# NicoNeureiter/sBayes

Hardware: AMD Instinct MI355X
Metric: log-likelihood evals/sec at 1000 sites x 200 feats x 10 states; 1/2/4/8-GPU chains (higher is better)
Workload: dtype f64; 1 GPU; headline synthetic 1000x200x10, K=5, C=2 (BASELINE.json configs[2]); chains_per_gpu=4096, kernel=packed, log_mode=product, parallelism=1 independent engine(s), one per GPU, no collectives

## Files before the change

sbayes_amd/csrc/sbe_engine_internal.hip.h:

```cpp
#pragma once
#include "sbe_kernels.hip.h"
#include "sbe_unit.hip.h"
#include "../../include/sbe_engine.h"
#include "../../include/sbe_engine_steps.h"
#include "../../include/sbe_engine_diag.h"
#include "sbe_host_helpers.h"
#include "sbe_pool.h"

#include <sched.h>
#include <algorithm>
#include <cstdarg>
#include <cstdio>
#include <cstring>
#include <chrono>
#include <atomic>
#include <condition_variable>
#include <functional>
#include <mutex>
#include <string>
#include <thread>
#include <vector>

using namespace sbe;

inline thread_local std::string g_last_error;

namespace {

struct Slot {
    std::vector<uint16_t> h_gid;
    std::vector<uint8_t> h_pid;
    std::vector<uint32_t> patterns;
    int n_tuples = 0;
    std::vector<uint8_t> h_tid;
    std::vector<uint32_t> h_toff;
    std::vector<uint16_t> h_tuple_g;
    std::vector<uint8_t> h_tuple_p;
    bool share_ok = false;
    bool groups_set = false, weights_set = false, source_set = false;
    std::vector<uint8_t> probs_set, counts_set;
    bool patterns_dirty = true;
    uint32_t gid_pending = 0;
    bool tables_follow = false;
    std::vector<int32_t> pat_cnt;
    std::vector<int32_t> tup_cnt;
    bool inc_ok = false;
    uint64_t group_epoch = 0;
    uint32_t overlap_mask = 0;
    int32_t ov_obj = -1, ov_g1 = 0, ov_g2 = 0, ov_comp = 0;
};

}

static int fuse_tables_default() {
    static const int on = [] { const char* v = getenv("SBE_FUSE_TABLES"); return (v && atoi(v) == 0) ? 0 : 1; }();
    return on;
}

struct sbe_engine : sbe::MixShape {
    int device = 0;
    hipStream_t stream = nullptr;
    hipEvent_t ev0 = nullptr, ev1 = nullptr;
    std::vector<hipEvent_t> ev_pool;
    bool ev_timing = false;  int ev_used = 0;
    int Fp = 0, rs_pitch = 0;
    uint64_t rng_seed = 0, rng_draw = 0;
    std::vector<int> G, goff;
    int64_t n_na = 0;
    int64_t hbm_bytes = 0;
    std::string last_error;
    char device_name[64] = {0};
    char last_kernel[128] = "none";

    sbe::MixTuning tune;
    int opt_log = SBE_LOG_PRODUCT;
    int opt_fuse_tables = fuse_tables_default();
    bool ws_lds_allowed[2] = {false, false};

    uint8_t* d_onehot = nullptr;
    uint8_t* d_state = nullptr;
    uint8_t* d_state_q = nullptr;
    float* d_probs_t = nullptr;
    double* d_wpat_t = nullptr;
    uint16_t* d_gid = nullptr;
    uint8_t* d_pid = nullptr;
    uint8_t* d_src = nullptr;
    int32_t* d_counts = nullptr;
    float* d_probs = nullptr;
    float* d_weights = nullptr;
    float* d_wpat = nullptr;
    uint32_t* d_patbits = nullptr;
    uint16_t* d_state_h = nullptr;
    double2* d_logtab = nullptr;
    uint32_t* d_toff = nullptr;
    uint32_t* d_rowoff = nullptr;
    std::vector<uint64_t> rowoff_epoch;
    uint32_t* d_rowoff_s = nullptr;  int rs_nq_max = 0;
    int32_t* d_rs_nq = nullptr;
    uint8_t* d_state_s = nullptr;
    std::vector<uint64_t> rowsort_epoch;
    std::atomic<uint64_t> epoch_counter{0};
    double2* d_logtab_fine = nullptr;
    unsigned* d_arrive = nullptr;
    uint8_t* d_xt = nullptr;
    int xt_NT = 0, xt_KBp = 0;  size_t xt_bytes = 0;
    uint8_t* d_tid = nullptr;
    uint16_t* d_tuple_g = nullptr;
    uint8_t* d_tuple_p = nullptr;
    double* d_conc = nullptr;
    double* d_unif = nullptr;
    double* d_lg_conc = nullptr; double* d_sum_a = nullptr; double* d_lg_sum_a = nullptr;
    double* d_unif_res = nullptr;  bool unif_set = false;
    int32_t* d_comp_of_group = nullptr;
    std::vector<uint8_t> conc_set;
    double* d_partials = nullptr;
    double* d_results = nullptr;
    double* h_results = nullptr;
    int* d_status = nullptr;
    int* h_status = nullptr;
    int* h_flag = nullptr;  int* d_flag = nullptr;
    unsigned long long* h_done = nullptr;  unsigned long long* d_done = nullptr;
    unsigned* d_ticket = nullptr;  unsigned long long done_seq = 0;
    static constexpr int kMaxChunks = 16;
    unsigned long long* h_chunk_flags = nullptr;  unsigned long long* d_chunk_flags = nullptr;
    unsigned* d_chunk_tickets = nullptr;  unsigned long long chunk_seq = 0;
    uint8_t* h_stream = nullptr;  uint8_t* d_stream = nullptr;  size_t stream_bytes = 0;
    uint8_t* d_changed = nullptr;
    uint32_t* d_step_stamp = nullptr;  uint32_t step_id = 0;
    float* d_step_pf = nullptr;
    double* d_step_pg = nullptr;
    struct StepLayout { size_t ids, pid, tid, toff, tuple_g, tuple_p, patbits, weights, row_of, subset, stale, objects, rows, total; } sl{};
    int step_max_rows = 0;
    uint8_t* h_step_payload = nullptr; uint8_t* d_step_payload = nullptr;
    uint8_t* h_io = nullptr; uint8_t* d_io = nullptr; size_t io_bytes = 0;
    uint8_t* h_step = nullptr;     uint8_t* d_step_host = nullptr;
    struct Lane { uint8_t* h_payload; uint8_t* d_payload; uint8_t* h_step; uint8_t* d_step_host; float* d_pf;
                  uint32_t* d_stamp; uint32_t step_id;
                  int* d_status; };
    std::vector<Lane> lanes;
    uint8_t* d_batch_meta = nullptr; size_t batch_meta_bytes = 0;
    uint8_t* h_batch_payload = nullptr; uint8_t* d_batch_payload = nullptr; size_t batch_payload_bytes = 0;
    std::vector<Slot> batch_cands;
    std::vector<std::vector<int32_t>> batch_moved;
    std::vector<int32_t> step_moved;
    struct Pool;
    Pool* pool = nullptr;
    uint8_t* d_scratch = nullptr;  size_t scratch_bytes = 0;
    uint8_t* h_pinned = nullptr;   size_t pinned_bytes = 0;
    uint8_t* h_arena = nullptr;    uint8_t* d_arena = nullptr;   size_t arena_bytes = 0, arena_off = 0;
    SetterJobs* batch = nullptr;
    int opt_step_form = 0;
    int opt_step_derive = 0;
    int opt_deferred = 0;
    bool status_pending = false;
    const char* pending_origin[2] = {nullptr, nullptr};
    int pending_calls = 0;
    std::vector<Slot> slots;
    struct SrcSync { uint64_t version = 1; int peer = -1; uint64_t peer_version = 0, own_version = 0; std::vector<int32_t> diff; };
    std::vector<SrcSync> src_sync;
    std::vector<SrcSync> ids_sync;

    int64_t probs_t_elems() const { return (int64_t)n_ftiles * tile_tab_elems(); }
    int64_t wpat_tile_elems() const { return (int64_t)Pmax * C * ft; }
    int64_t wpat_t_elems() const { return (int64_t)n_ftiles * wpat_tile_elems(); }
};

namespace {
inline void bump_src(sbe_engine* e, int slot) { ++e->src_sync[slot].version; }
inline void bump_ids(sbe_engine* e, int slot) { ++e->ids_sync[slot].version; }
}

struct sbe_engine::Pool : sbe_host::StepPool { using sbe_host::StepPool::StepPool; };

namespace {

int fail(sbe_engine* e, int code, const char* fmt, ...) {
    char buf[512];
    va_list ap;
    va_start(ap, fmt);
    vsnprintf(buf, sizeof buf, fmt, ap);
    va_end(ap);
    g_last_error = buf;
    if (e) e->last_error = buf;
    return code;
}

#define CHECK_ENGINE(e) \
    if (!(e)) return fail(nullptr, SBE_ERR_ARG, "null engine handle")
#define CHECK_SLOT(e, s) \
    if ((s) < 0 || (s) >= (e)->n_slots) return fail(e, SBE_ERR_ARG, "slot %d out of range [0,%d)", (s), (e)->n_slots)
#define CHECK_COMP(e, c) \
    if ((c) < 0 || (c) >= (e)->C) return fail(e, SBE_ERR_ARG, "component %d out of range [0,%d)", (c), (e)->C)
#define CHECK_PTR(e, p) \
    if (!(p)) return fail(e, SBE_ERR_ARG, "null pointer argument: %s", #p)

inline int round_up(int a, int b) { return (a + b - 1) / b * b; }

template <class T>
int dmalloc(sbe_engine* e, T** p, int64_t n) {
    const size_t bytes = std::max<int64_t>(n, 1) * sizeof(T);
    HIPCHK(e, hipMalloc((void**)p, bytes));
    e->hbm_bytes += (int64_t)bytes;
    return SBE_OK;
}

inline size_t al256(size_t v) { return (v + 255) / 256 * 256; }

int ensure_scratch(sbe_engine* e, size_t bytes) {
    if (bytes <= e->scratch_bytes) return SBE_OK;
    if (e->d_scratch) { HIPCHK(e, hipStreamSynchronize(e->stream)); HIPCHK(e, hipFree(e->d_scratch)); }
    e->scratch_bytes = bytes + bytes / 4 + 4096;
    HIPCHK(e, hipMalloc((void**)&e->d_scratch, e->scratch_bytes));
    return SBE_OK;
}

int ensure_io(sbe_engine* e, size_t bytes) {
    if (bytes <= e->io_bytes) return SBE_OK;
    if (e->h_io) { HIPCHK(e, hipStreamSynchronize(e->stream)); HIPCHK(e, hipHostFree(e->h_io)); e->h_io = nullptr; e->io_bytes = 0; }
    const size_t want = bytes + bytes / 4 + 4096;
    HIPCHK(e, hipHostMalloc((void**)&e->h_io, want, hipHostMallocMapped));
    HIPCHK(e, hipHostGetDevicePointer((void**)&e->d_io, e->h_io, 0));
    e->io_bytes = want;
    return SBE_OK;
}

int ensure_pinned(sbe_engine* e, size_t bytes) {
    if (bytes <= e->pinned_bytes) return SBE_OK;
    if (e->h_pinned) { HIPCHK(e, hipStreamSynchronize(e->stream)); HIPCHK(e, hipHostFree(e->h_pinned)); }
    e->pinned_bytes = bytes + bytes / 4 + 4096;
    HIPCHK(e, hipHostMalloc((void**)&e->h_pinned, e->pinned_bytes, hipHostMallocDefault));
    return SBE_OK;
}

int upload(sbe_engine* e, void* dst_dev, const void* src, size_t bytes);
int synced(sbe_engine* e);

int ensure_step_pool(sbe_engine* e);

int ensure_stream(sbe_engine* e, size_t bytes) {
    if (bytes <= e->stream_bytes) return SBE_OK;
    if (e->h_stream) { HIPCHK(e, hipStreamSynchronize(e->stream)); HIPCHK(e, hipHostFree(e->h_stream)); e->h_stream = nullptr; e->stream_bytes = 0; }
    const size_t want = bytes + bytes / 4 + 4096;
    HIPCHK(e, hipHostMalloc((void**)&e->h_stream, want, hipHostMallocMapped));
    HIPCHK(e, hipHostGetDevicePointer((void**)&e->d_stream, e->h_stream, 0));
    e->stream_bytes = want;
    return SBE_OK;
}

struct StreamPlan { ChunkSig sig; int n_chunks; size_t chunk_bytes; size_t bytes; unsigned grid; };

StreamPlan plan_stream(sbe_engine* e, unsigned n_blocks, size_t bytes_per_block, size_t bytes) {
    static const int max_chunks = [] { const char* v = getenv("SBE_STREAM_CHUNKS"); const int n = v ? atoi(v) : 0;
                                       return n >= 1 && n <= sbe_engine::kMaxChunks ? n : 8; }();
    unsigned per = std::max<unsigned>(1, (unsigned)div_up((int64_t)n_blocks, max_chunks));
    per = std::max<unsigned>(per, (unsigned)div_up((int64_t)128 << 10, (int64_t)bytes_per_block));
    const int n_chunks = (int)div_up((int64_t)n_blocks, (int64_t)per);
    static const bool ordered = [] { const char* v = getenv("SBE_STREAM_ORDERED"); return !(v && atoi(v) == 0); }();
    ChunkSig sig{e->d_chunk_tickets, e->d_chunk_flags, ++e->chunk_seq, per, n_blocks, (unsigned)n_chunks, 0};
    unsigned grid = n_blocks;
    if (ordered && n_chunks > 1) {
        sig.chunk_elems = (long long)per * (long long)(bytes_per_block / sizeof(double));
        grid = per;
    }
    return StreamPlan{sig, n_chunks, (size_t)per * bytes_per_block, bytes, grid};
}

template <class JobBegin, class JobEnd, class Work>
int stream_result(sbe_engine* e, const StreamPlan& plan, int n_jobs, JobBegin job_begin, JobEnd job_end, Work work) {
    static const bool single_thread = [] { const char* v = getenv("SBE_D2H_THREADS"); return v && atoi(v) == 1; }();
    if (!single_thread) { int rc = ensure_step_pool(e); if (rc) return rc; }
    std::atomic<bool> all_landed{false};
    hipError_t sync_err = hipSuccess;
    const volatile unsigned long long* flags = e->h_chunk_flags;
    const unsigned long long seq = plan.sig.seq;
    const size_t chunk_bytes = plan.chunk_bytes;
    const auto t_limit = std::chrono::steady_clock::now() + std::chrono::microseconds(2000 + (int64_t)(plan.bytes / 10000));
    unsigned spins = 0;
    sbe_host::run_as_chunks_land(
        single_thread ? nullptr : e->pool, n_jobs,
        [=](int j) { return (int)(job_begin(j) / chunk_bytes); },
        [=](int j) { return (int)((job_end(j) - 1) / chunk_bytes); },
        [&, flags, seq](int k) { return flags[k] == seq || all_landed.load(std::memory_order_acquire); },
        [&] {
            if ((++spins & 1023u) == 0 && !all_landed.load(std::memory_order_relaxed) && std::chrono::steady_clock::now() > t_limit) {
                sync_err = hipStreamSynchronize(e->stream);
                all_landed.store(true, std::memory_order_release);
            }
        },
        work);
    if (sync_err != hipSuccess) return fail(e, SBE_ERR_HIP, "hipStreamSynchronize (streamed result): %s", hipGetErrorString(sync_err));
    return SBE_OK;
}

int d2h(sbe_engine* e, void* dst, const void* src_dev, size_t bytes) {
    int rc = ensure_pinned(e, bytes);
    if (rc) return rc;
    HIPCHK(e, hipMemcpyAsync(e->h_pinned, src_dev, bytes, hipMemcpyDeviceToHost, e->stream));
    HIPCHK(e, hipStreamSynchronize(e->stream));
    static const bool single_copy = [] { const char* v = getenv("SBE_D2H_THREADS"); return v && atoi(v) == 1; }();
    if (bytes >= ((size_t)1 << 20) && !single_copy) {
        rc = ensure_step_pool(e);
        if (rc) return rc;
        constexpr size_t kJob = (size_t)64 << 10;
        uint8_t* out = (uint8_t*)dst;
        const uint8_t* stage = e->h_pinned;
        e->pool->run((int)((bytes + kJob - 1) / kJob),
                     [=](int j) { const size_t o = (size_t)j * kJob; memcpy(out + o, stage + o, std::min(kJob, bytes - o)); });
        return synced(e);
    }
    memcpy(dst, e->h_pinned, bytes);
    return synced(e);
}

constexpr size_t kMappedOutMax = (size_t)1 << 18;
int out_target(sbe_engine* e, size_t bytes, void* dev_fallback, void** target) {
    *target = dev_fallback;
    if (bytes > kMappedOutMax) return SBE_OK;
    int rc = ensure_io(e, bytes);
    if (rc) return rc;
    *target = e->d_io;
    return SBE_OK;
}
int wait_done(sbe_engine* e, const DoneSig& d);
DoneSig next_done(sbe_engine* e, unsigned n_blocks);
DoneSig out_done(sbe_engine* e, const void* target, unsigned n_blocks) {
    return target == (const void*)e->d_io ? next_done(e, n_blocks) : DoneSig{};
}
int out_fetch(sbe_engine* e, void* host_out, const void* target, size_t bytes, const DoneSig& done = DoneSig{}) {
    if (target != (const void*)e->d_io) return d2h(e, host_out, target, bytes);
    int rc = wait_done(e, done);
    if (rc) return rc;
    memcpy(host_out, e->h_io, bytes);
    return synced(e);
}

int h2d(sbe_engine* e, void* dst_dev, const void* src, size_t bytes) { return upload(e, dst_dev, src, bytes); }

int upload(sbe_engine* e, void* dst_dev, const void* src, size_t bytes) {
    if (bytes == 0) return SBE_OK;
    if (e->h_arena && bytes <= e->arena_bytes / 4) {
        const size_t need = (bytes + 63) / 64 * 64;
        if (e->arena_off + need > e->arena_bytes) {
            HIPCHK(e, hipStreamSynchronize(e->stream));
            e->arena_off = 0;
        }
        uint8_t* stage = e->h_arena + e->arena_off;
        e->arena_off += need;
        memcpy(stage, src, bytes);
        HIPCHK(e, hipMemcpyAsync(dst_dev, stage, bytes, hipMemcpyHostToDevice, e->stream));
        return SBE_OK;
    }
    HIPCHK(e, hipMemcpyAsync(dst_dev, src, bytes, hipMemcpyHostToDevice, e->stream));
    HIPCHK(e, hipStreamSynchronize(e->stream));
    return SBE_OK;
}

int stage(sbe_engine* e, const void* src, size_t bytes, void* dev_fallback, const void** out) {
    constexpr size_t kDirect = (size_t)64 << 10;
    *out = dev_fallback;
    if (bytes == 0) return SBE_OK;
    if (!e->d_arena || bytes > kDirect) return upload(e, dev_fallback, src, bytes);
    const size_t need = (bytes + 63) / 64 * 64;
    if (e->arena_off + need > e->arena_bytes) {
        HIPCHK(e, hipStreamSynchronize(e->stream));
        e->arena_off = 0;
    }
    memcpy(e->h_arena + e->arena_off, src, bytes);
    *out = e->d_arena + e->arena_off;
    e->arena_off += need;
    return SBE_OK;
}

struct UploadSeg { void* dst; const void* src; size_t bytes; };
struct FusedWeightPatterns { WeightPatternArgs args; int bits_seg; const float* new_weights; bool done; };
int upload_segments(sbe_engine* e, const UploadSeg* segs, int n, FusedWeightPatterns* wp = nullptr) {
    size_t total = 0, largest = 0;
    for (int i = 0; i < n; ++i) { total += (segs[i].bytes + 63) / 64 * 64; largest = std::max(largest, segs[i].bytes); }
    if (wp) wp->done = false;
    if (total == 0) return SBE_OK;
    if (!e->d_arena || n > 8 || total > ((size_t)64 << 10)) {
        for (int i = 0; i < n; ++i) { int rc = upload(e, segs[i].dst, segs[i].src, segs[i].bytes); if (rc) return rc; }
        return SBE_OK;
    }
    const size_t w_bytes = wp && wp->new_weights ? (size_t)wp->args.F * wp->args.C * sizeof(float) : 0;
    const bool fuse = wp && segs[wp->bits_seg].bytes > 0 && w_bytes <= ((size_t)64 << 10);
    const size_t reserve = total + (fuse ? (w_bytes + 63) / 64 * 64 : 0);
    if (e->arena_off + reserve > e->arena_bytes) {
        HIPCHK(e, hipStreamSynchronize(e->stream));
        e->arena_off = 0;
    }
    ScatterSegs sg{};
    size_t off = 0;
    for (int i = 0; i < n; ++i) {
        if (segs[i].bytes == 0) continue;
        memcpy(e->h_arena + e->arena_off + off, segs[i].src, segs[i].bytes);
        sg.dst[sg.n] = (uint8_t*)segs[i].dst; sg.off[sg.n] = (uint32_t)off; sg.bytes[sg.n] = (uint32_t)segs[i].bytes;
        ++sg.n;
        if (fuse && i == wp->bits_seg) wp->args.pattern_bits = (const uint32_t*)(e->d_arena + e->arena_off + off);
        off += (segs[i].bytes + 63) / 64 * 64;
    }
    const unsigned sx = (unsigned)std::min<size_t>(div_up((int64_t)largest, 1024), 16);
    unsigned wx = 0;
    if (fuse) {
        if (w_bytes) {
            memcpy(e->h_arena + e->arena_off + off, wp->new_weights, w_bytes);
            wp->args.weights = (const float*)(e->d_arena + e->arena_off + off);
        }
        wx = (unsigned)div_up((int64_t)wp->args.P * wp->args.F, 256);
        wp->done = true;
    }
    if (e->batch && e->batch->n_group_blocks == 0 && (fuse || !wp)) {
        SetterJobs& j = *e->batch;
        j.group_base = e->d_arena + e->arena_off; j.sg = sg; j.has_wp = fuse ? 1 : 0;
        if (fuse) j.wp = wp->args;
        j.group_gx = std::max(sx, wx); j.n_group_blocks = j.group_gx * (unsigned)(sg.n + (fuse ? 1 : 0));
    } else if (fuse) {
        k_scatter_weight_patterns<<<dim3(std::max(sx, wx), sg.n + 1), 256, 0, e->stream>>>(e->d_arena + e->arena_off, sg, wp->args);
    } else {
        k_scatter_bytes<<<dim3(sx, sg.n), 256, 0, e->stream>>>(e->d_arena + e->arena_off, sg);
    }
    HIPCHK(e, hipGetLastError());
    e->arena_off += reserve;
    return SBE_OK;
}

bool poll_done_enabled() {
    static const bool on = [] { const char* v = getenv("SBE_POLL_DONE"); return !(v && atoi(v) == 0); }();
    return on;
}
DoneSig next_done(sbe_engine* e, unsigned n_blocks) {
    if (!poll_done_enabled()) return DoneSig{};
    return DoneSig{e->d_ticket, e->d_done, ++e->done_seq, n_blocks};
}
int wait_done(sbe_engine* e, const DoneSig& d) {
    if (d.flag) {
        const volatile unsigned long long* f = e->h_done;
        const auto t0 = std::chrono::steady_clock::now();
        for (unsigned spins = 1;; ++spins) {
            if (*f == d.seq) { std::atomic_thread_fence(std::memory_order_acquire); return SBE_OK; }
            if ((spins & 127u) == 0u) sched_yield(); else __builtin_ia32_pause();
            if ((spins & 255u) == 0 && std::chrono::steady_clock::now() - t0 > std::chrono::microseconds(300)) break;
        }
    }
    HIPCHK(e, hipStreamSynchronize(e->stream));
    return SBE_OK;
}

bool status_raised(const sbe_engine* e) {
    const volatile int* f = e->h_flag;
    return (f[ST_BAD_NORMALIZE] | f[ST_MULTI_SOURCE]) != 0;
}

int fetch_and_clear_status(sbe_engine* e) {
    HIPCHK(e, hipMemcpyAsync(e->h_status, e->d_status, ST_FLAG_PTR * sizeof(int), hipMemcpyDeviceToHost, e->stream));
    HIPCHK(e, hipMemsetAsync(e->d_status + ST_BAD_NORMALIZE, 0, 2 * sizeof(int), e->stream));
    HIPCHK(e, hipStreamSynchronize(e->stream));
    e->h_flag[ST_BAD_NORMALIZE] = e->h_flag[ST_MULTI_SOURCE] = 0;
    return SBE_OK;
}

int report_status(sbe_engine* e, bool deferred = false) {
    const int n_calls = e->pending_calls;
    const char* origin[2] = {e->pending_origin[0], e->pending_origin[1]};
    e->pending_calls = 0;
    e->pending_origin[0] = e->pending_origin[1] = nullptr;
    if (!status_raised(e)) return SBE_OK;
    int rc = fetch_and_clear_status(e);
    if (rc) return rc;
    const int bad_norm = e->h_status[ST_BAD_NORMALIZE], multi_src = e->h_status[ST_MULTI_SOURCE];
    e->h_status[ST_BAD_NORMALIZE] = e->h_status[ST_MULTI_SOURCE] = 0;
    char where[200] = "";
    const char* who = origin[bad_norm ? 0 : 1];
    if (deferred && who)
        snprintf(where, sizeof where, " [deferred data check: raised by %s (%d state-setting call%s queued since the last report), "
                 "reported by the first call that waited for the device]", who, n_calls, n_calls == 1 ? "" : "s");
    if (bad_norm)
        return fail(e, SBE_ERR_DATA, "normalize: %d rows have a non-positive sum (sbayes/util.py:1006 assert)%s", bad_norm, where);
    return fail(e, SBE_ERR_DATA, "source is not one-hot over components in %d observations%s", multi_src, where);
}

int check_after(sbe_engine* e, int word, const char* who = __builtin_FUNCTION()) {
    if (e->opt_deferred) {
        e->status_pending = true;
        e->pending_origin[word == ST_BAD_NORMALIZE ? 0 : 1] = who;
        ++e->pending_calls;
        return SBE_OK;
    }
    HIPCHK(e, hipStreamSynchronize(e->stream));
    e->status_pending = false;
    return report_status(e);
}

int synced(sbe_engine* e) {
    if (!e->status_pending) return SBE_OK;
    e->status_pending = false;
    return report_status(e, true);
}

int read_status(sbe_engine* e) {
    HIPCHK(e, hipStreamSynchronize(e->stream));
    int rc = synced(e);
    if (rc) return rc;
    e->h_status[ST_BAD_NORMALIZE] = e->h_status[ST_MULTI_SOURCE] = 0;
    if (status_raised(e)) return fetch_and_clear_status(e);
    return SBE_OK;
}

int take_status(sbe_engine* e) {
    e->h_status[ST_BAD_NORMALIZE] = e->h_status[ST_MULTI_SOURCE] = 0;
    if (status_raised(e)) return fetch_and_clear_status(e);
    return SBE_OK;
}

int clear_status_word(sbe_engine* e, int word) {
    if (e->status_pending) return SBE_OK;
    if (!e->h_flag[word]) return SBE_OK;
    HIPCHK(e, hipStreamSynchronize(e->stream));
    HIPCHK(e, hipMemsetAsync(e->d_status + word, 0, sizeof(int), e->stream));
    e->h_flag[word] = 0;
    return SBE_OK;
}

void derive_patterns(sbe_engine* e, Slot& s) {
    const int N = e->N, C = e->C;
    static thread_local std::vector<uint8_t> bits;
    bits.resize(N);
    bool seen[256] = {false};
    s.pat_cnt.assign(256, 0);
    for (int n = 0; n < N; ++n) {
        uint32_t b = 0;
        for (int c = 0; c < C; ++c)
            if (s.h_gid[(size_t)c * N + n] != kNoGroup) b |= 1u << c;
        bits[n] = (uint8_t)b;
        seen[b] = true;
        ++s.pat_cnt[b];
    }
    auto key = [C](uint32_t b) {
        uint32_t k = 0;
        for (int c = 0; c < C; ++c) k |= ((b >> c) & 1u) << (C - 1 - c);
        return k;
    };
    std::vector<uint32_t> uniq;
    for (uint32_t b = 0; b < 256; ++b) if (seen[b]) uniq.push_back(b);
    std::sort(uniq.begin(), uniq.end(), [&](uint32_t a, uint32_t b) { return key(a) < key(b); });
    uint8_t index_of[256] = {0};
    for (size_t i = 0; i < uniq.size(); ++i) index_of[uniq[i]] = (uint8_t)i;
    s.patterns = uniq;
    s.h_pid.resize(N);
    for (int n = 0; n < N; ++n) s.h_pid[n] = index_of[bits[n]];
}

bool tuples_share_operands(const sbe_engine* e, const Slot& s) {
    if (e->C != 2 || s.n_tuples == 0 || (int)s.h_tuple_p.size() != kMaxTuples) return false;
    int first = -1, pb = -1;
    for (int t = 0; t < kMaxTuples; ++t) {
        const int pat = s.h_tuple_p[t];
        if (pat == 0xFF) continue;
        if (first < 0) { first = t; continue; }
        if (s.h_tuple_g[(size_t)t * kMaxComponents + 1] != s.h_tuple_g[(size_t)first * kMaxComponents + 1]) return false;
        const int pa = s.h_tuple_p[first];
        if (pat != pa) {
            if (pb < 0) pb = pat;
            else if (pat != pb) return false;
        }
    }
    return first >= 0;
}

void derive_tuples(sbe_engine* e, Slot& s) {
    const int N = e->N, C = e->C;
    s.h_tid.assign(e->Np, 0);
    s.h_toff.assign(e->Np, 0);
    s.h_tuple_g.assign((size_t)kMaxTuples * kMaxComponents, (uint16_t)e->Gtot);
    s.h_tuple_p.assign(kMaxTuples, 0xFF);
    uint16_t tuples[kMaxTuples][kMaxComponents];
    int n_tup = 0;
    bool ok = true;
    s.tup_cnt.assign(kMaxTuples, 0);
    uint64_t packed[kMaxTuples];
    int last = 0;
    for (int n = 0; n < N && ok; ++n) {
        uint16_t key[kMaxComponents];
        for (int c = 0; c < C; ++c) key[c] = s.h_gid[(size_t)c * N + n];
        int t = 0;
        if (C <= 4) {
            uint64_t k64 = 0;
            for (int c = 0; c < C; ++c) k64 |= (uint64_t)key[c] << (16 * c);
            if (n_tup && packed[last] == k64) t = last;
            else for (; t < n_tup; ++t) if (packed[t] == k64) break;
            if (t == n_tup && n_tup < kMaxTuples) packed[n_tup] = k64;
        } else {
            for (; t < n_tup; ++t) if (memcmp(tuples[t], key, (size_t)C * sizeof(uint16_t)) == 0) break;
        }
        last = t;
        if (t == n_tup) {
            if (n_tup == kMaxTuples) { ok = false; break; }
            memcpy(tuples[n_tup++], key, (size_t)C * sizeof(uint16_t));
            for (int c = 0; c < C; ++c) s.h_tuple_g[(size_t)t * kMaxComponents + c] = key[c] == kNoGroup ? (uint16_t)e->Gtot : key[c];
            s.h_tuple_p[t] = s.h_pid[n];
        }
        s.h_tid[n] = (uint8_t)t;
        s.h_toff[n] = (uint32_t)t * (uint32_t)(e->S + 1) * 512u;
        ++s.tup_cnt[t];
    }
    s.n_tuples = ok ? n_tup : 0;
    s.inc_ok = ok;
    s.share_ok = tuples_share_operands(e, s);
}

bool update_patterns_and_tuples(sbe_engine* e, Slot& s, const int32_t* moved, const uint16_t* old_gid0, int n_moved) {
    const int N = e->N, C = e->C;
    if (!s.inc_ok || s.n_tuples == 0 || (int)s.pat_cnt.size() != 256 || (int)s.tup_cnt.size() != kMaxTuples) return false;
    auto bits_rest = [&](int n) { uint32_t b = 0; for (int c = 1; c < C; ++c) if (s.h_gid[(size_t)c * N + n] != kNoGroup) b |= 1u << c; return b; };
    for (int i = 0; i < n_moved; ++i) {
        const int n = moved[i];
        const uint32_t rest = bits_rest(n);
        const uint32_t b0 = rest | (old_gid0[i] != kNoGroup ? 1u : 0u), b1 = rest | (s.h_gid[n] != kNoGroup ? 1u : 0u);
        if (b0 == b1) continue;
        --s.pat_cnt[b0]; ++s.pat_cnt[b1];
    }
    {
        size_t live = 0;
        for (uint32_t b = 0; b < 256; ++b) if (s.pat_cnt[b] > 0) ++live;
        bool same = live == s.patterns.size();
        for (size_t i = 0; same && i < s.patterns.size(); ++i) same = s.pat_cnt[s.patterns[i]] > 0;
        if (!same) return false;
    }
    uint8_t rank_of[256];
    for (size_t i = 0; i < s.patterns.size(); ++i) rank_of[s.patterns[i]] = (uint8_t)i;
    for (int i = 0; i < n_moved; ++i) {
        const int n = moved[i];
        const uint32_t b1 = bits_rest(n) | (s.h_gid[n] != kNoGroup ? 1u : 0u);
        s.h_pid[n] = rank_of[b1];
        uint16_t key[kMaxComponents];
        for (int c = 0; c < C; ++c) { const uint16_t g = s.h_gid[(size_t)c * N + n]; key[c] = g == kNoGroup ? (uint16_t)e->Gtot : g; }
        const int t0 = s.h_tid[n];
        int t1 = -1, free_t = -1;
        for (int t = 0; t < s.n_tuples; ++t) {
            if (s.tup_cnt[t] == 0) { if (free_t < 0 && t != t0) free_t = t; continue; }
            if (memcmp(&s.h_tuple_g[(size_t)t * kMaxComponents], key, (size_t)C * sizeof(uint16_t)) == 0) { t1 = t; break; }
        }
        if (t1 < 0) {
            if (s.tup_cnt[t0] == 1) t1 = t0;
            else if (free_t >= 0) t1 = free_t;
            else if (s.n_tuples < kMaxTuples) t1 = s.n_tuples++;
            else return false;
            for (int c = 0; c < C; ++c) s.h_tuple_g[(size_t)t1 * kMaxComponents + c] = key[c];
        }
        if (t1 != t0) {
            if (--s.tup_cnt[t0] == 0) s.h_tuple_p[t0] = 0xFF;
            ++s.tup_cnt[t1];
        }
        s.h_tuple_p[t1] = s.h_pid[n];
        s.h_tid[n] = (uint8_t)t1;
        s.h_toff[n] = (uint32_t)t1 * (uint32_t)(e->S + 1) * 512u;
    }
    while (s.n_tuples > 0 && s.tup_cnt[s.n_tuples - 1] == 0) --s.n_tuples;
    s.share_ok = tuples_share_operands(e, s);
    for (int t = 0; t < s.n_tuples; ++t)
        if (s.tup_cnt[t] == 0) return false;
    return s.n_tuples > 0;
}

int upload_patterns_and_weights(sbe_engine* e, int slot, const float* new_weights = nullptr, bool eager = false) {
    Slot& s = e->slots[slot];
    float* d_w = e->d_weights + (int64_t)slot * e->F * e->C;
    auto gid_seg = [&](int c) { return UploadSeg{e->d_gid + ((int64_t)slot * e->C + c) * e->Np, s.h_gid.data() + (size_t)c * e->N, (size_t)e->N * sizeof(uint16_t)}; };
    bool patterns_done = false;
    if (s.patterns_dirty) {
        const bool follow = s.tables_follow;
        s.tables_follow = false;
        if (!follow) derive_patterns(e, s);
        if ((int)s.patterns.size() > e->Pmax) {
            if (eager) {
                for (int c = 0; c < e->C; ++c)
                    if (s.gid_pending >> c & 1u) { const UploadSeg g = gid_seg(c); int rc = upload(e, g.dst, g.src, g.bytes); if (rc) return rc; }
                s.gid_pending = 0;
                return SBE_OK;
            }
            return fail(e, SBE_ERR_ARG, "%zu distinct has_components patterns exceed capacity %d",
                        s.patterns.size(), e->Pmax);
        }
        if (!follow) derive_tuples(e, s);
        UploadSeg segs[6 + kMaxComponents] = {{e->d_pid + (int64_t)slot * e->Np, s.h_pid.data(), (size_t)e->N},
                                              {e->d_patbits + (int64_t)slot * e->Pmax, s.patterns.data(), s.patterns.size() * sizeof(uint32_t)}};
        int n_segs = 2;
        if (s.n_tuples) {
            segs[n_segs++] = {e->d_tid + (int64_t)slot * e->Np, s.h_tid.data(), (size_t)e->Np};
            segs[n_segs++] = {e->d_toff + (int64_t)slot * e->Np, s.h_toff.data(), (size_t)e->Np * sizeof(uint32_t)};
            segs[n_segs++] = {e->d_tuple_g + (int64_t)slot * kMaxTuples * kMaxComponents, s.h_tuple_g.data(), s.h_tuple_g.size() * sizeof(uint16_t)};
            segs[n_segs++] = {e->d_tuple_p + (int64_t)slot * kMaxTuples, s.h_tuple_p.data(), s.h_tuple_p.size()};
        }
        for (int c = 0; c < e->C; ++c) if (s.gid_pending >> c & 1u) segs[n_segs++] = gid_seg(c);
        const int P = (int)s.patterns.size();
        FusedWeightPatterns wp{};
        const bool want_wp = (s.weights_set || new_weights) && P > 0;
        if (want_wp) {
            wp.args = WeightPatternArgs{d_w, nullptr, e->d_wpat + (int64_t)slot * e->Pmax * e->F * e->C, new_weights ? d_w : nullptr,
                                        e->d_wpat_t + (int64_t)slot * e->wpat_t_elems(), P, e->F, e->C, e->Pmax, e->ft};
            wp.bits_seg = 1;
            wp.new_weights = new_weights;
        }
        { int _urc = upload_segments(e, segs, n_segs, want_wp ? &wp : nullptr); if (_urc) return _urc; }
        patterns_done = wp.done;
        s.patterns_dirty = false;
        s.gid_pending = 0;
    }
    const int P = (int)s.patterns.size();
    if (new_weights && P == 0) {
        int rc = upload(e, d_w, new_weights, (size_t)e->F * e->C * sizeof(float));
        if (rc) return rc;
    }
    if ((s.weights_set || new_weights) && P > 0 && !patterns_done) {
        const void* w_in = d_w;
        if (new_weights) { int rc = stage(e, new_weights, (size_t)e->F * e->C * sizeof(float), d_w, &w_in); if (rc) return rc; }
        k_weight_patterns<<<div_up((int64_t)P * e->F, 256), 256, 0, e->stream>>>(
            (const float*)w_in, e->d_patbits + (int64_t)slot * e->Pmax, e->d_wpat + (int64_t)slot * e->Pmax * e->F * e->C, P, e->F, e->C,
            w_in != d_w ? d_w : nullptr, e->d_wpat_t + (int64_t)slot * e->wpat_t_elems(), e->Pmax, e->ft);
        HIPCHK(e, hipGetLastError());
    }
    return SBE_OK;
}

int retile_probs(sbe_engine* e, int slot, int component) {
    const int g_lo = e->goff[component], g_hi = g_lo + e->G[component];
    const int64_t n = (int64_t)(g_hi - g_lo) * e->S * e->ft * e->n_ftiles;
    if (n == 0) return SBE_OK;
    k_tile_probs<<<div_up(n, 256), 256, 0, e->stream>>>(
        e->d_probs + (int64_t)slot * e->table_elems(), e->d_probs_t + (int64_t)slot * e->probs_t_elems(),
        g_lo, g_hi, e->Gtot, e->F, e->S, e->ft, e->n_ftiles);
    HIPCHK(e, hipGetLastError());
    return SBE_OK;
}

int check_slot_ready(sbe_engine* e, int slot, bool need_weights) {
    Slot& s = e->slots[slot];
    if (!s.groups_set) return fail(e, SBE_ERR_STATE, "slot %d: groups not set for every component", slot);
    for (int c = 0; c < e->C; ++c)
        if (!s.probs_set[c]) return fail(e, SBE_ERR_STATE, "slot %d: probability tables of component %d not set", slot, c);
    if (need_weights && !s.weights_set) return fail(e, SBE_ERR_STATE, "slot %d: weights not set", slot);
    return SBE_OK;
}

int check_collapsed_ready(sbe_engine* e, int slot, int c_lo, int c_hi) {
    Slot& s = e->slots[slot];
    for (int c = c_lo; c < c_hi; ++c) {
        if (e->G[c] == 0) continue;
        if (!s.counts_set[c]) return fail(e, SBE_ERR_STATE, "slot %d: counts of component %d not set", slot, c);
        if (!e->conc_set[c]) return fail(e, SBE_ERR_STATE, "concentration of component %d not set", c);
    }
    return SBE_OK;
}

constexpr size_t kCollapsedLdsMax = (size_t)96 << 10;
inline size_t collapsed_lds_bytes(const sbe_engine* e) { return (size_t)e->F * e->S * sizeof(double) + (size_t)e->F * sizeof(float); }

template <class TC>
int enqueue_dcl(sbe_engine* e, const TC* counts, const double* conc, int conc_per_group, int g_lo, int G, float* d_pf, double* d_pg) {
    k_dcl<TC><<<div_up((int64_t)G * e->F, 256), 256, 0, e->stream>>>(counts, conc, d_pf, g_lo, g_lo + G, e->F, e->S, conc_per_group);
    HIPCHK(e, hipGetLastError());
    if (!d_pg) return SBE_OK;
    k_group_sum_f32<<<div_up((int64_t)G * 8, 64), 64, 0, e->stream>>>(d_pf, d_pg, G, e->F);
    HIPCHK(e, hipGetLastError());
    return SBE_OK;
}

int ensure_xt(sbe_engine* e) {
    if (e->d_xt) return SBE_OK;
    const int NT = div_up((int64_t)e->F * e->S, 32), KBp = round_up(div_up(e->N, kTupleMfmaKBlockObjects), 4);
    const size_t bytes = ((size_t)(NT + 1) * KBp + 4) * 1024;
    uint8_t* xt = nullptr;
    double2* logtab = nullptr;
    auto build = [&]() -> int {
        HIPCHK(e, hipMalloc((void**)&xt, bytes));
        HIPCHK(e, hipMemsetAsync(xt, 0, bytes, e->stream));
        std::vector<double> tab(2 * kFineLogEntries);
        fine_log_table(tab.data());
        HIPCHK(e, hipMalloc((void**)&logtab, tab.size() * sizeof(double) + column_tables_bytes(NT)));
        HIPCHK(e, hipMemcpy(logtab, tab.data(), tab.size() * sizeof(double), hipMemcpyHostToDevice));
        launch_column_tables(e->d_state, reinterpret_cast<int32_t*>(logtab + kFineLogEntries), e->N, e->F, e->S, e->Fp, NT, e->stream);
        HIPCHK(e, hipGetLastError());
        launch_xt_frags(e->d_state, xt, e->N, e->F, e->S, e->Fp, NT, KBp, e->stream);
        HIPCHK(e, hipGetLastError());
        return SBE_OK;
    };
    const int rc = build();
    if (rc) {
        (void)hipStreamSynchronize(e->stream);
        if (xt) (void)hipFree(xt);
        if (logtab) (void)hipFree(logtab);
        return rc;
    }
    e->d_xt = xt; e->d_logtab_fine = logtab;
    e->hbm_bytes += (int64_t)bytes;
    e->xt_NT = NT; e->xt_KBp = KBp; e->xt_bytes = bytes;
    return SBE_OK;
}

int next_timing_events(sbe_engine* e, hipEvent_t* ev_a, hipEvent_t* ev_b) {
    *ev_a = *ev_b = nullptr;
    if (!e->ev_timing) return SBE_OK;
    while ((int)e->ev_pool.size() < 2 * (e->ev_used + 1)) {
        hipEvent_t ev;
        HIPCHK(e, hipEventCreate(&ev));
        e->ev_pool.push_back(ev);
    }
    *ev_a = e->ev_pool[2 * e->ev_used]; *ev_b = e->ev_pool[2 * e->ev_used + 1];
    ++e->ev_used;
    return SBE_OK;
}

struct MixCall {
    int first_slot = 0, n = 1;
    const int32_t* slots = nullptr;  const int32_t* d_slots = nullptr;
    const StepFinish* fin = nullptr;
    const StepFinish* d_fins = nullptr;
    DoneSig* done_out = nullptr;
    hipEvent_t ev_a = nullptr, ev_b = nullptr;
    int slot_at(int i) const { return slots ? (int)slots[i] : first_slot + i; }
};

MixFacts mixture_facts(const sbe_engine* e, const MixCall& c) {
    MixFacts f;
    f.n = c.n;
    f.share_ok = true;
    bool tuples = true;
    for (int i = 0; i < c.n; ++i) {
        const Slot& s = e->slots[c.slot_at(i)];
        f.P = std::max<int>(f.P, (int)s.patterns.size());
        f.KT = std::max(f.KT, s.n_tuples);
        tuples &= s.n_tuples != 0;
        f.share_ok &= s.share_ok;
    }
    if (!tuples) f.KT = 0;
    f.epilogue = c.fin || c.d_fins;
    f.waits = c.done_out != nullptr;
    return f;
}

MixTuning launch_tuning(const sbe_engine* e, const MixFacts& f) {
    MixTuning t = e->tune;
    if (considers_tuple_mfma(*e, t, f))
        if (const char* env = getenv("SBE_MFMA_SPLIT")) t.mfma_split = atoi(env);
    t.shared_allowed = tuple_mfma_shared();
    static const bool in_kernel_opt = !(getenv("SBE_REDUCE_IN_KERNEL") && atoi(getenv("SBE_REDUCE_IN_KERNEL")) == 0);
    t.in_kernel_allowed = in_kernel_opt;
    return t;
}

int prepare_mixture(sbe_engine* e, const MixPlan& pl, const MixCall& c) {
    if (pl.form == MixForm::TupleMfma) return ensure_xt(e);
    if (pl.form != MixForm::Rows && pl.form != MixForm::RowsSorted) return SBE_OK;
    const bool sorted = pl.form == MixForm::RowsSorted;
    const int rft = pl.ft;
    if (sorted && !e->d_rowoff_s) {
        e->rs_nq_max = pl.rs_nq_max;
        int rc = dmalloc(e, &e->d_rowoff_s, (int64_t)e->n_slots * e->rs_nq_max * (e->C + 1) * 4); if (rc) return rc;
        rc = dmalloc(e, &e->d_rs_nq, e->n_slots); if (rc) return rc;
        rc = dmalloc(e, &e->d_state_s, (int64_t)(e->N + 1) * e->Fq); if (rc) return rc;
        launch_state_s(e->d_state, e->d_state_s, e->N, e->F, e->Fp, e->Fq, e->S, e->stream);
        HIPCHK(e, hipGetLastError());
        e->rowsort_epoch.assign(e->n_slots, ~0ull);
    }
    std::vector<uint64_t>& built = sorted ? e->rowsort_epoch : e->rowoff_epoch;
    bool stale = false;
    for (int i = 0; i < c.n; ++i) stale |= built[c.slot_at(i)] != e->slots[c.slot_at(i)].group_epoch;
    if (!stale) return SBE_OK;
    if (sorted) {
        launch_rowsort(e->d_gid, e->d_pid, e->d_rowoff_s, e->d_rs_nq, (int64_t)e->C * e->Np, e->Np,
                       (int64_t)e->rs_nq_max * (e->C + 1) * 4, c.first_slot, c.d_slots, c.n, e->N, e->Np, e->C, e->Gtot, e->Pmax,
                       (uint32_t)((e->S + 1) * rft * 4), (uint32_t)e->Fq, 4 * (kWave / rft), e->stream);
    } else {
        const int cells = (e->C + 1) * e->Np;
        k_rowoff<<<dim3(div_up(cells, 256), c.n), 256, 0, e->stream>>>(
            e->d_gid, e->d_pid, e->d_rowoff, (int64_t)e->C * e->Np, e->Np, (int64_t)cells, c.first_slot, c.d_slots, e->N, e->Np,
            e->C, e->Gtot, (uint32_t)((e->S + 1) * rft * 4), (uint32_t)(((e->C + 1) / 2) * rft * 16));
    }
    HIPCHK(e, hipGetLastError());
    for (int i = 0; i < c.n; ++i) built[c.slot_at(i)] = e->slots[c.slot_at(i)].group_epoch;
    return SBE_OK;
}

int launch_mfma_form(sbe_engine* e, const MixCall& c, const MixPlan& pl, const DoneSig& done) {
    MfmaMixParams p{};
    p.F = e->F; p.S = e->S; p.FS = e->F * e->S; p.Gtot = e->Gtot; p.Np = e->Np;
    p.NT = e->xt_NT; p.KBp = e->xt_KBp; p.KT = pl.KT; p.SL = pl.SL; p.shared = pl.shared ? 1 : 0;
    p.n_batch = c.n; p.n_split = pl.n_split; p.nt_per_split = pl.nt_per_split;
    p.first_slot = c.first_slot; p.slot_list = c.d_slots;
    p.xt = e->d_xt; p.xt_bytes = (uint32_t)e->xt_bytes;
    p.tid = e->d_tid; p.tid_stride = e->Np;
    p.tuple_g = e->d_tuple_g; p.tuple_g_stride = (int64_t)kMaxTuples * kMaxComponents;
    p.tuple_p = e->d_tuple_p; p.tuple_p_stride = kMaxTuples;
    p.probs = e->d_probs; p.probs_stride = e->table_elems();
    p.probs_ones_off = (uint32_t)((int64_t)e->n_slots * e->table_elems() * 4);
    p.probs_bytes = p.probs_ones_off + (uint32_t)(e->F * e->S * 4);
    p.wpat = e->d_wpat; p.wpat_stride = (int64_t)e->Pmax * e->F * e->C;
    p.wpat_ones_off = (uint32_t)((int64_t)e->n_slots * e->Pmax * e->F * e->C * 4);
    p.wpat_bytes = p.wpat_ones_off + (uint32_t)(e->F * e->C * 4);
    p.logtab = e->d_logtab_fine;
    p.colcount = reinterpret_cast<const int32_t*>(e->d_logtab_fine + kFineLogEntries);
    p.colfeat = p.colcount + (size_t)(e->xt_NT + 1) * 32;
    p.tile_prefix = p.colcount + (size_t)(e->xt_NT + 1) * 64;
    p.partials = e->d_partials; p.partials_stride = e->partials_stride;
    if (pl.in_kernel) { p.results = e->d_results; p.arrive = e->d_arrive; p.done = done; }
    if (!launch_tuple_mfma(e->C, p, dim3(pl.grid_x), pl.lds_bytes, e->stream))
        return fail(e, SBE_ERR_STATE, "k_mixture_tuple_mfma was built with static LDS: its log table must sit at LDS address 0 "
                                      "(toolchain change; rebuild without static __shared__ in sbe_mixture_mfma.hip)");
    return SBE_OK;
}

void launch_tile_form(sbe_engine* e, const MixCall& c, const MixPlan& pl, const DoneSig& done) {
    Mix2Params p{};
    p.N = e->N; p.NQ = e->NQ; p.Np = e->Np; p.F = e->F; p.Fq = e->Fq; p.S = e->S; p.C = e->C;
    p.Gtot = e->Gtot; p.P = pl.P; p.n_ftiles = pl.n_ftiles; p.quads_per_chunk = pl.quads_per_chunk;
    p.state_q = reinterpret_cast<const uint32_t*>(e->d_state_q);
    p.onehot = e->d_onehot; p.rs_pitch = e->rs_pitch;
    p.gid = e->d_gid; p.gid_stride = (int64_t)e->C * e->Np;
    p.pid = e->d_pid; p.pid_stride = e->Np;
    p.probs_t = e->d_probs_t; p.probs_t_stride = e->probs_t_elems();
    p.wpat_t = e->d_wpat_t; p.wpat_t_stride = e->wpat_t_elems(); p.wpat_tile_stride = (int)e->wpat_tile_elems();
    p.partials = e->d_partials; p.partials_stride = e->partials_stride; p.first_slot = c.first_slot;
    if (pl.in_kernel) { p.results = e->d_results; p.arrive = e->d_arrive; p.done = done; }
    p.slot_list = c.d_slots;
    p.n_work = pl.n_partials; p.n_batch = c.n;
    p.slot_groups = pl.slot_groups; p.slots_per_group = pl.slots_per_group;
    p.tid = e->d_tid; p.tid_stride = e->Np;
    p.state_h = reinterpret_cast<const uint2*>(e->d_state_h);
    p.toff = e->d_toff; p.toff_stride = e->Np;
    p.logtab = e->d_logtab;
    p.ragged_w = pl.ragged_w; p.gen_slots = pl.gen_slots;
    p.tuple_g = e->d_tuple_g; p.tuple_g_stride = (int64_t)kMaxTuples * kMaxComponents;
    p.tuple_p = e->d_tuple_p; p.tuple_p_stride = kMaxTuples;
    p.combo_w_off = pl.combo_w_off; p.combo_tab_off = pl.combo_tab_off;
    p.KT = pl.KT;
    p.eft = e->ft;
    p.wpat = e->d_wpat; p.wpat_stride = (int64_t)e->Pmax * e->F * e->C;
    p.rowoff = e->d_rowoff; p.rowoff_stride = (int64_t)(e->C + 1) * e->Np;
    p.rowoff_s = e->d_rowoff_s; p.rowoff_s_stride = (int64_t)e->rs_nq_max * (e->C + 1) * 4;
    p.rs_nq = e->d_rs_nq; p.state_s = e->d_state_s; p.state_s_pitch = e->Fq;
    {
        constexpr int split[4] = {450, 270, 170, 110};
        p.rows_cum[0] = 0;
        for (int i = 0; i < 4; ++i) p.rows_cum[i + 1] = p.rows_cum[i] + split[i];
    }
    const int mode = e->opt_log == SBE_LOG_PRODUCT ? LOG_PRODUCT : LOG_PER_OBS;
    const dim3 grid(pl.grid_x, 1);
    switch (pl.form) {
        case MixForm::Tuple64: launch_tuple64(e->C, p, grid, pl.lds_bytes, e->stream); break;
        case MixForm::Combo: launch_combo(pl.onehot, pl.ft, e->C, p, grid, pl.lds_bytes, e->stream); break;
        case MixForm::Rows: case MixForm::RowsSorted:
            launch_rows(mode, pl.ft, e->C, p, grid, pl.lds_bytes, e->stream, pl.form == MixForm::RowsSorted); break;
        case MixForm::OnehotV2: launch_oh2(mode, pl.ft, e->C, p, grid, pl.lds_bytes, e->stream, e->direct); break;
        default: launch_v2(mode, pl.ft, e->C, p, grid, pl.lds_bytes, e->stream, e->direct); break;
    }
}

int launch_mixture(sbe_engine* e, const MixCall& c) {
    const MixFacts facts = mixture_facts(e, c);
    const MixPlan pl = plan_mixture(*e, launch_tuning(e, facts), facts);
    if (pl.err) return fail(e, pl.err, "%s", pl.msg);
    int rc = prepare_mixture(e, pl, c);
    if (rc) return rc;
    if (c.ev_a) HIPCHK(e, hipEventRecord(c.ev_a, e->stream));
    DoneSig done_k{};
    if (pl.in_kernel && c.done_out) *c.done_out = done_k = next_done(e, pl.done_blocks);
    plan_name(pl, *e, e->last_kernel, sizeof e->last_kernel);
    if (pl.form == MixForm::TupleMfma) { rc = launch_mfma_form(e, c, pl, done_k); if (rc) return rc; }
    else launch_tile_form(e, c, pl, done_k);
    if (c.ev_b) HIPCHK(e, hipEventRecord(c.ev_b, e->stream));
    HIPCHK(e, hipGetLastError());
    if (pl.in_kernel) return SBE_OK;
    const unsigned n_red = (unsigned)(c.n + (c.d_fins ? c.n : (c.fin ? 1 : 0)));
    const DoneSig done = c.done_out ? next_done(e, n_red) : DoneSig{};
    if (c.done_out) *c.done_out = done;
    k_reduce_partials<<<n_red, kBlock, 0, e->stream>>>(e->d_partials, e->partials_stride, pl.n_partials,
                                                       e->d_results, c.first_slot, c.n, c.fin ? *c.fin : StepFinish{},
                                                       c.d_slots, c.d_fins, done);
    HIPCHK(e, hipGetLastError());
    return SBE_OK;
}

int enqueue_mixture(sbe_engine* e, int first_slot, int n, DoneSig* done_out = nullptr) {
    for (int s = first_slot; s < first_slot + n; ++s) {
        int rc = check_slot_ready(e, s, true);
        if (rc) return rc;
        if (e->slots[s].patterns_dirty) { rc = upload_patterns_and_weights(e, s); if (rc) return rc; }
    }
    MixCall c;
    c.first_slot = first_slot; c.n = n; c.done_out = done_out;
    { int rc = next_timing_events(e, &c.ev_a, &c.ev_b); if (rc) return rc; }
    return launch_mixture(e, c);
}

int counts_launch(sbe_engine* e, int slot_a, int sign_a, int slot_b, int sign_b, const int32_t* d_objects,
                  int n_listed, int dst_slot, bool single_chunk, uint8_t* d_changed) {
    CountSide A{e->d_gid + (int64_t)slot_a * e->C * e->Np, e->d_src + (int64_t)slot_a * e->N * e->Fp, sign_a};
    CountSide B{e->d_gid + (int64_t)slot_b * e->C * e->Np, e->d_src + (int64_t)slot_b * e->N * e->Fp, sign_b};
    int32_t* counts = e->d_counts + (int64_t)dst_slot * e->table_elems();
    int ft = 32;
    auto lds_for = [&](int t) { return (size_t)e->Gtot * t * e->S * sizeof(int32_t); };
    while (ft > 4 && lds_for(ft) > 96 * 1024) ft >>= 1;
    if (lds_for(ft) > 150 * 1024) {
        k_counts_global<<<div_up((int64_t)n_listed * e->F, 256), 256, 0, e->stream>>>(
            e->d_state, A, B, d_objects, n_listed, e->Np, e->F, e->S, e->C, e->Fp, counts, d_changed);
        HIPCHK(e, hipGetLastError());
        return SBE_OK;
    }
    const int n_ftiles = div_up(e->F, ft);
    int chunks = 1;
    if (!single_chunk) chunks = std::max(1, std::min(div_up(n_listed, 32), div_up(2 * e->compute_units, n_ftiles)));
    const int opc = div_up(n_listed, chunks);
    chunks = div_up(n_listed, opc);
    k_counts<<<dim3(n_ftiles, chunks), kBlock, lds_for(ft), e->stream>>>(
        e->d_state, A, B, d_objects, n_listed, opc, e->Np, e->F, e->S, e->C, e->Fp, e->Gtot, ft, counts, d_changed);
    HIPCHK(e, hipGetLastError());
    return SBE_OK;
}

}

namespace {

int set_gid_common(sbe_engine* e, int slot, int component, const std::vector<uint16_t>& ids) {
    Slot& s = e->slots[slot];
    s.tables_follow = false;
    static const bool follow_on = [] { const char* v = getenv("SBE_FOLLOW_TABLES"); return !(v && atoi(v) == 0); }();
    if (follow_on && component == 0 && !s.patterns_dirty && s.inc_ok) {
        static thread_local std::vector<int32_t> moved;
        static thread_local std::vector<uint16_t> old_ids;
        moved.clear(); old_ids.clear();
        const int N = e->N;
        for (int n = 0; n < N; ++n)
            if (ids[n] != s.h_gid[n]) { moved.push_back(n); old_ids.push_back(s.h_gid[n]); }
        std::copy(ids.begin(), ids.end(), s.h_gid.begin());
        s.tables_follow = (int)moved.size() * 8 <= N &&
                          update_patterns_and_tuples(e, s, moved.data(), old_ids.data(), (int)moved.size());
    } else {
        std::copy(ids.begin(), ids.end(), s.h_gid.begin() + (size_t)component * e->N);
    }
    s.gid_pending |= 1u << component;
    s.patterns_dirty = true;
    s.group_epoch = ++e->epoch_counter;
    bump_ids(e, slot);
    s.groups_set = true;
    return upload_patterns_and_weights(e, slot, nullptr, true);
}

void overlap_message(char* buf, size_t len, int n, int g1, int g2, int component) {
    snprintf(buf, len, "object %d is in groups %d and %d of component %d: resident slot state keeps one group id per object "
             "and component (counts.py:28-30 would count it in both); counts of overlapping groups come from the caller or "
             "the stateless sbe_effect_counts", n, g1, g2, component);
}

struct OverlapNote { bool found = false; int obj = -1, g1 = 0, g2 = 0; };

bool matrix_to_ids(const uint8_t* groups, int G, int N, int off, int component, uint16_t* ids, char* msg, size_t msg_len,
                   OverlapNote* note = nullptr) {
    std::fill(ids, ids + N, kNoGroup);
    auto hit = [&](int n, int g) -> bool {
        if (ids[n] != kNoGroup) {
            if (!note) { overlap_message(msg, msg_len, n, (int)ids[n] - off, g, component); return false; }
            if (!note->found) { note->found = true; note->obj = n; note->g1 = (int)ids[n] - off; note->g2 = g; }
        }
        ids[n] = (uint16_t)(off + g);
        return true;
    };
    for (int g = 0; g < G; ++g) {
        const uint8_t* row = groups + (size_t)g * N;
        int n = 0;
        for (; n + 8 <= N; n += 8) {
            uint64_t w8;
            memcpy(&w8, row + n, 8);
            if (!w8) continue;
            for (int k = 0; k < 8; ++k) if (row[n + k] && !hit(n + k, g)) return false;
        }
        for (; n < N; ++n) if (row[n] && !hit(n, g)) return false;
    }
    return true;
}

int reject_overlap(sbe_engine* e, int slot, const char* what) {
    const Slot& s = e->slots[slot];
    if (!s.overlap_mask) return SBE_OK;
    char msg[320];
    overlap_message(msg, sizeof msg, s.ov_obj, s.ov_g1, s.ov_g2, s.ov_comp);
    return fail(e, SBE_ERR_DATA, "%s (slot %d, %s)", msg, slot, what);
}


int enqueue_lh_exact(sbe_engine* e, int slot, const char* who) {
    Slot& s = e->slots[slot];
    if (!s.groups_set || !s.source_set || !s.weights_set) return fail(e, SBE_ERR_STATE, "slot %d: groups / source / weights not set", slot);
    { int orc = reject_overlap(e, slot, who); if (orc) return orc; }
    for (int c = 0; c < e->C; ++c)
        if (!s.counts_set[c] || !e->conc_set[c]) return fail(e, SBE_ERR_STATE, "slot %d: counts / concentration of component %d not set", slot, c);
    HIPCHK(e, hipSetDevice(e->device));
    int rc = SBE_OK;
    if (s.patterns_dirty) { rc = upload_patterns_and_weights(e, slot); if (rc) return rc; }
    const int64_t n = (int64_t)e->N * e->F;
    rc = ensure_scratch(e, n * sizeof(double));
    if (rc) return rc;
    rc = clear_status_word(e, ST_BAD_NORMALIZE);
    if (rc) return rc;
    k_lh_exact<<<div_up(n, 256), 256, 0, e->stream>>>(
        e->d_state, e->d_src + (int64_t)slot * e->N * e->Fp, e->d_gid + (int64_t)slot * e->C * e->Np,
        e->d_counts + (int64_t)slot * e->table_elems(), e->d_conc, (double*)e->d_scratch, e->N, e->Np, e->F, e->S, e->C,
        e->Fp, e->d_status, e->d_wpat + (int64_t)slot * e->Pmax * e->F * e->C, e->d_pid + (int64_t)slot * e->Np);
    HIPCHK(e, hipGetLastError());
    return SBE_OK;
}

int lh_exact_report(sbe_engine* e) {
    int rc = read_status(e);
    if (rc) return rc;
    if (e->h_status[ST_BAD_NORMALIZE]) return fail(e, SBE_ERR_DATA, "normalize: non-positive row sum in leave-one-out tables (sbayes/util.py:1006 assert)");
    return SBE_OK;
}

int sync_and_report(sbe_engine* e, const DoneSig& done = DoneSig{}) {
    { int rc = wait_done(e, done); if (rc) return rc; }
    const bool was_pending = e->status_pending;
    e->status_pending = false;
    return report_status(e, was_pending);
}

int check_objects(sbe_engine* e, const int32_t* objects, int n) {
    for (int i = 0; i < n; ++i)
        if (objects[i] < 0 || objects[i] >= e->N) return fail(e, SBE_ERR_ARG, "object index %d out of range", objects[i]);
    return SBE_OK;
}

SrcPostArgs src_post_args(sbe_engine* e, int slot, const int32_t* d_objects, int n_sub, double temperature, double prior_temperature,
                          int from_prior) {
    const double inv_t = 1.0 / temperature, inv_tp = 1.0 / prior_temperature;
    return SrcPostArgs{e->d_state, e->d_gid + (int64_t)slot * e->C * e->Np, e->d_pid + (int64_t)slot * e->Np,
                       e->d_probs + (int64_t)slot * e->table_elems(), e->d_wpat + (int64_t)slot * e->Pmax * e->F * e->C,
                       d_objects, n_sub, e->Np, e->F, e->S, e->C, e->Fp, inv_t, (float)inv_tp, inv_t != 1.0, inv_tp != 1.0,
                       from_prior != 0};
}

ClusterOpArgs cluster_op_args(sbe_engine* e, int slot, double prior_temperature, const int32_t* d_objects, int n, double* d_out) {
    const double inv = 1.0 / prior_temperature;
    return ClusterOpArgs{e->d_state, e->d_gid + (int64_t)slot * e->C * e->Np, e->d_pid + (int64_t)slot * e->Np,
                         e->d_weights + (int64_t)slot * e->F * e->C, e->d_patbits + (int64_t)slot * e->Pmax, (float)inv,
                         inv != 1.0 ? 1 : 0, d_objects, n, d_out, reinterpret_cast<const f64x2_t*>(e->d_logtab),
                         e->Np, e->F, e->S, e->C, e->Fp};
}

constexpr size_t kGuFusedLdsMax = (size_t)96 << 10;

}

namespace {
int ensure_step_pool(sbe_engine* e) {
    if (!e->pool) {
        int nt = 7;
        if (const char* env = getenv("SBE_STEP_THREADS")) nt = std::max(0, atoi(env) - 1);
        int cpus = (int)std::thread::hardware_concurrency();
        cpu_set_t set;
        if (sched_getaffinity(0, sizeof set, &set) == 0) cpus = std::min(cpus > 0 ? cpus : CPU_COUNT(&set), CPU_COUNT(&set));
        if (FILE* f = fopen("/sys/fs/cgroup/cpu.max", "r")) {
            long long quota = 0, period = 0;
            if (fscanf(f, "%lld %lld", &quota, &period) == 2 && quota > 0 && period > 0)
                cpus = std::min<int>(cpus, (int)std::max<long long>(1, quota / period));
            fclose(f);
        }
        int local_world = 1;
        if (const char* env = getenv("LOCAL_WORLD_SIZE")) local_world = std::max(1, atoi(env));
        nt = std::min<int>(nt, std::max(0, cpus / local_world - 1));
        e->pool = new sbe_engine::Pool(nt);
    }
    return SBE_OK;
}
}
```

sbayes_amd/csrc/sbe_engine_steps.hip:

```cpp
#include "sbe_engine_internal.hip.h"

extern "C" {

namespace {
struct CoreInputs {
    const void* ids_new = nullptr;
    const void* pid = nullptr; const void* tid = nullptr; const void* toff = nullptr;
    const void* tuple_g = nullptr; const void* tuple_p = nullptr; const void* patbits = nullptr;
    const void* weights = nullptr;
    const int16_t* row_of = nullptr;
    const uint8_t* rows = nullptr; const int32_t* objects = nullptr; int n_changed = 0;
    const uint8_t* src_new = nullptr;
    const int32_t* subset = nullptr; int n_subset = 0;
    int P = 1;
    bool full_src_copy = true; const int32_t* stale = nullptr; int n_stale = 0;
    const int32_t* patch_n = nullptr; const uint16_t* patch_gid = nullptr; const uint8_t* patch_pid = nullptr;
    const uint8_t* patch_tid = nullptr; int n_patch = -1;
    const int16_t* sub_row = nullptr; const uint16_t* sub_gid0 = nullptr;
};

sbe_engine::Lane lane0(sbe_engine* e) {
    return sbe_engine::Lane{e->h_step_payload, e->d_step_payload, e->h_step, e->d_step_host, e->d_step_pf, e->d_step_stamp, e->step_id,
                            e->d_status};
}
// ... 275 lines not shown
    ++rc.version;
    if (moved.size() == 1 && moved[0] < 0) {
        rc.peer = cu.peer = -1;
        rc.diff.clear(); cu.diff.clear();
        return;
    }
    rc.peer = cur_slot; rc.peer_version = cu.version; rc.own_version = rc.version; rc.diff = moved;
    cu.peer = cand_slot; cu.peer_version = rc.version; cu.own_version = cu.version; cu.diff = moved;
}

static void commit_src_sync(sbe_engine* e, int cur_slot, int cand_slot, const int32_t* changed_objects, int n_changed) {
    sbe_engine::SrcSync& rc = e->src_sync[cand_slot];
    sbe_engine::SrcSync& cu = e->src_sync[cur_slot];
    ++rc.version;
    rc.peer = cur_slot; rc.peer_version = cu.version; rc.own_version = rc.version;
    rc.diff.assign(changed_objects, changed_objects + n_changed);
    cu.peer = cand_slot; cu.peer_version = rc.version; cu.own_version = cu.version;
    cu.diff = rc.diff;
}

static int step_lean(sbe_engine* e, int cur_slot, int cand_slot, const uint8_t* clusters, const int32_t* changed_objects,
                     int n_changed, const uint8_t* source_rows, const float* weights, double* group_logliks_out,
                     double* mixture_out, uint8_t* changed_groups_out) {
    if (e->status_pending) {
        HIPCHK(e, hipStreamSynchronize(e->stream));
        int rc = synced(e);
        if (rc) return rc;
    }
    static const bool timing = getenv("SBE_STEP_TIMING") && atoi(getenv("SBE_STEP_TIMING")) == 1;
    static double t_acc[3] = {0, 0, 0};
    static int t_n = 0;
    const auto t0 = std::chrono::steady_clock::now();
    Slot cd;
    CoreInputs in;
    {
        std::string err;
        int rc = prepare_step(e, lane0(e), cur_slot, cand_slot, clusters, changed_objects, n_changed, source_rows, weights, cd, in, &err,
                              &e->step_moved);
        if (rc) return fail(e, rc, "%s", err.c_str());
    }
    const auto t1 = std::chrono::steady_clock::now();
    int rc = launch_step_core(e, cur_slot, cand_slot, in);
    if (rc) return rc;
    commit_src_sync(e, cur_slot, cand_slot, changed_objects, n_changed);
    commit_ids_sync(e, cur_slot, cand_slot, e->step_moved);
    e->slots[cand_slot] = cd;
    StepFinish fin = make_step_finish(e);
    DoneSig done;
    MixCall mix;
    mix.first_slot = cand_slot; mix.fin = &fin; mix.done_out = &done;
    rc = launch_mixture(e, mix);
    if (rc) return rc;
    const auto t2 = std::chrono::steady_clock::now();
    rc = wait_done(e, done);
    if (rc) return rc;
    if (timing) {
        const auto t3 = std::chrono::steady_clock::now();
        t_acc[0] += std::chrono::duration<double, std::micro>(t1 - t0).count();
        t_acc[1] += std::chrono::duration<double, std::micro>(t2 - t1).count();
        t_acc[2] += std::chrono::duration<double, std::micro>(t3 - t2).count();
        if (++t_n == 2000) {
            fprintf(stderr, "[sbe_step] host prepare %.1f us, enqueue %.1f us, wait %.1f us per step\n", t_acc[0] / t_n, t_acc[1] / t_n, t_acc[2] / t_n);
            t_acc[0] = t_acc[1] = t_acc[2] = 0; t_n = 0;
        }
    }
    return read_step_results(e, cand_slot, group_logliks_out, mixture_out, changed_groups_out, "rows");
}

namespace {
int ensure_lanes(sbe_engine* e, int n) {
    const size_t hb = step_host_lq_offset(e) + 2 * sizeof(double);
    while ((int)e->lanes.size() < n) {
        sbe_engine::Lane ln{};
        HIPCHK(e, hipHostMalloc((void**)&ln.h_step, hb, hipHostMallocMapped));
        memset(ln.h_step, 0, hb);
        HIPCHK(e, hipHostGetDevicePointer((void**)&ln.d_step_host, ln.h_step, 0));
        HIPCHK(e, hipMalloc((void**)&ln.d_pf, (size_t)e->Gtot * e->F * sizeof(float)));
        HIPCHK(e, hipMalloc((void**)&ln.d_stamp, (size_t)e->Gtot * sizeof(uint32_t)));
        HIPCHK(e, hipMemsetAsync(ln.d_stamp, 0, (size_t)e->Gtot * sizeof(uint32_t), e->stream));
        HIPCHK(e, hipMalloc((void**)&ln.d_status, ST_WORDS * sizeof(int)));
        HIPCHK(e, hipMemsetAsync(ln.d_status, 0, ST_WORDS * sizeof(int), e->stream));
        ln.step_id = 0;
        e->lanes.push_back(ln);
    }
    return SBE_OK;
}
}


int sbe_step_batch(sbe_engine* e, int n_chains, const int32_t* cur_slots, const int32_t* cand_slots,
                   const uint8_t* clusters, const uint8_t* clusters_mask, const int32_t* rows_ptr,
                   const int32_t* changed_objects, const uint8_t* source_rows, const float* weights,
                   const uint8_t* weights_mask, double* group_logliks_out, double* mixture_out,
                   uint8_t* changed_groups_out) {
    CHECK_ENGINE(e); CHECK_PTR(e, cur_slots); CHECK_PTR(e, cand_slots); CHECK_PTR(e, rows_ptr);
    CHECK_PTR(e, group_logliks_out); CHECK_PTR(e, mixture_out);
    if (n_chains < 1 || n_chains > e->n_slots / 2) return fail(e, SBE_ERR_ARG, "n_chains=%d (1..%d: two slots per chain)", n_chains, e->n_slots / 2);
    if ((int64_t)e->Gtot * e->S * 28 > 60 * 1024) return fail(e, SBE_ERR_ARG, "sbe_step_batch: tables too large for the one-launch step (G_total=%d, S=%d)", e->Gtot, e->S);
    const int N = e->N, F = e->F, C = e->C, K = e->G[0];
    if (rows_ptr[0] != 0) return fail(e, SBE_ERR_ARG, "rows_ptr[0] must be 0");
    static const bool timing = getenv("SBE_STEP_TIMING") && atoi(getenv("SBE_STEP_TIMING")) != 0;
    using clk = std::chrono::steady_clock;
    clk::time_point tp[12]; int ntp = 0;
    auto mark = [&] { if (timing && ntp < 12) tp[ntp++] = clk::now(); };
    mark();
    {
        std::vector<uint8_t> used(e->n_slots, 0);
        for (int i = 0; i < n_chains; ++i) {
            const int a = cur_slots[i], b = cand_slots[i];
            if (a < 0 || a >= e->n_slots || b < 0 || b >= e->n_slots || a == b) return fail(e, SBE_ERR_ARG, "chain %d: bad slots (%d, %d)", i, a, b);
            if (used[a] || used[b]) return fail(e, SBE_ERR_ARG, "chain %d: slot used by another chain of the batch", i);
            used[a] = used[b] = 1;
            const int nr = rows_ptr[i + 1] - rows_ptr[i];
            if (nr < 0 || nr > e->step_max_rows) return fail(e, SBE_ERR_ARG, "chain %d: %d changed source rows (0..%d per chain in a batched step)", i, nr, e->step_max_rows);
            if (nr > 0 && (!changed_objects || !source_rows)) return fail(e, SBE_ERR_ARG, "changed_objects / source_rows missing");
            for (int k = rows_ptr[i]; k < rows_ptr[i + 1]; ++k)
                if (changed_objects[k] < 0 || changed_objects[k] >= N) return fail(e, SBE_ERR_ARG, "chain %d: object index %d out of range", i, changed_objects[k]);
            const Slot& cur = e->slots[a];
            if (!cur.groups_set || !cur.source_set || !cur.weights_set) return fail(e, SBE_ERR_STATE, "slot %d: groups / source / weights not set", a);
            { int orc = reject_overlap(e, a, "one-call step"); if (orc) return orc; }
            for (int c = 0; c < C; ++c)
                if (!cur.counts_set[c] || !e->conc_set[c]) return fail(e, SBE_ERR_STATE, "slot %d: counts / concentration of component %d not set", a, c);
        }
    }
    HIPCHK(e, hipSetDevice(e->device));
    if (e->status_pending) {
        HIPCHK(e, hipStreamSynchronize(e->stream));
        int rc = synced(e);
        if (rc) return rc;
    }
    for (int i = 0; i < n_chains; ++i)
        if (e->slots[cur_slots[i]].patterns_dirty) { int rc = upload_patterns_and_weights(e, cur_slots[i]); if (rc) return rc; }
    int rc = ensure_lanes(e, n_chains);
    if (rc) return rc;
    rc = ensure_step_pool(e);
    if (rc) return rc;
    mark();
    if ((int)e->batch_cands.size() < n_chains) e->batch_cands.resize(n_chains);
    if ((int)e->batch_moved.size() < n_chains) e->batch_moved.resize(n_chains);
    std::vector<Slot>& cds = e->batch_cands;
    std::vector<CoreInputs> ins(n_chains);
    std::vector<size_t> pay_off(n_chains + 1, 0);
    for (int i = 0; i < n_chains; ++i)
        pay_off[i + 1] = pay_off[i] + (e->sl.rows + (size_t)(rows_ptr[i + 1] - rows_ptr[i]) * F * C + 255) / 256 * 256;
    if (pay_off[n_chains] > e->batch_payload_bytes) {
        HIPCHK(e, hipStreamSynchronize(e->stream));
        if (e->h_batch_payload) { HIPCHK(e, hipHostFree(e->h_batch_payload)); e->h_batch_payload = nullptr; }
        if (e->d_batch_payload) { HIPCHK(e, hipFree(e->d_batch_payload)); e->d_batch_payload = nullptr; }
        e->batch_payload_bytes = pay_off[n_chains] + pay_off[n_chains] / 2;
        HIPCHK(e, hipHostMalloc((void**)&e->h_batch_payload, e->batch_payload_bytes, hipHostMallocDefault));
        HIPCHK(e, hipMalloc((void**)&e->d_batch_payload, e->batch_payload_bytes));
    }
    int n_parts = n_chains >= 128 ? 2 : 1;
    if (const char* env = getenv("SBE_STEP_PARTS")) n_parts = std::max(1, std::min(atoi(env), n_chains));
    const int per_part = div_up(n_chains, n_parts);
    const size_t part_cores = ((size_t)per_part * sizeof(StepCore) + 255) / 256 * 256;
    const size_t part_fins = ((size_t)per_part * sizeof(StepFinish) + 255) / 256 * 256;
    const size_t part_bytes = part_cores + part_fins + ((size_t)per_part * sizeof(int32_t) + 255) / 256 * 256;
    const size_t meta_bytes = part_bytes * n_parts;
    if (meta_bytes > e->batch_meta_bytes) {
        if (e->d_batch_meta) { HIPCHK(e, hipStreamSynchronize(e->stream)); HIPCHK(e, hipFree(e->d_batch_meta)); }
        e->batch_meta_bytes = meta_bytes + meta_bytes / 2;
        HIPCHK(e, hipMalloc((void**)&e->d_batch_meta, e->batch_meta_bytes));
    }
    std::vector<uint8_t> meta(meta_bytes);
    std::vector<int> rcs(n_chains, SBE_OK);
    std::vector<std::string> errs(n_chains);
    DoneSig batch_done{};
    for (int part = 0; part < n_parts; ++part) {
        const int i0 = part * per_part, i1 = std::min(n_chains, i0 + per_part), np = i1 - i0;
        if (np <= 0) break;
        constexpr int kCopyChunk = 16;
        const int n_copy_chunks = div_up(np, kCopyChunk);
        std::vector<std::atomic<int>> chunk_done(n_copy_chunks);
        for (auto& c : chunk_done) c.store(0, std::memory_order_relaxed);
        int next_copy = 0;
        hipError_t copy_err = hipSuccess;
        auto send_ready = [&]() {
            while (next_copy < n_copy_chunks) {
                const int c0 = i0 + next_copy * kCopyChunk, c1 = std::min(i1, c0 + kCopyChunk);
                if (chunk_done[next_copy].load(std::memory_order_acquire) < c1 - c0) break;
                const hipError_t he = hipMemcpyAsync(e->d_batch_payload + pay_off[c0], e->h_batch_payload + pay_off[c0],
                                                     pay_off[c1] - pay_off[c0], hipMemcpyHostToDevice, e->stream);
                if (he != hipSuccess) copy_err = he;
                ++next_copy;
            }
        };
        const std::function<void()> poll = send_ready;
        e->pool->run(np, [&](int j) {
            const int i = i0 + j;
            const bool regroup = clusters && (!clusters_mask || clusters_mask[i]);
            const bool reweight = weights && (!weights_mask || weights_mask[i]);
            const int r0 = rows_ptr[i], nr = rows_ptr[i + 1] - r0;
            sbe_engine::Lane lane = e->lanes[i];
            lane.h_payload = e->h_batch_payload + pay_off[i];
            lane.d_payload = e->d_batch_payload + pay_off[i];
            rcs[i] = prepare_step(e, lane, cur_slots[i], cand_slots[i], regroup ? clusters + (size_t)i * K * N : nullptr,
                                  nr ? changed_objects + r0 : nullptr, nr, nr ? source_rows + (size_t)r0 * F * C : nullptr,
                                  reweight ? weights + (size_t)i * F * C : nullptr, cds[i], ins[i], &errs[i], &e->batch_moved[i]);
            chunk_done[j / kCopyChunk].fetch_add(1, std::memory_order_release);
        }, &poll);
        send_ready();
        HIPCHK(e, copy_err);
        for (int i = i0; i < i1; ++i)
            if (rcs[i]) { (void)hipStreamSynchronize(e->stream); return fail(e, rcs[i], "chain %d: %s", i, errs[i].c_str()); }
        if (part == 0) mark();
        uint8_t* pm = meta.data() + (size_t)part * part_bytes;
        StepCore* cores = reinterpret_cast<StepCore*>(pm);
        StepFinish* fins = reinterpret_cast<StepFinish*>(pm + part_cores);
        int32_t* slot_list = reinterpret_cast<int32_t*>(pm + part_cores + part_fins);
        size_t lds = 0; int max_blocks = 0;
        for (int i = i0; i < i1; ++i) {
            size_t l = 0; int nb = 0;
            rc = build_step_core(e, e->lanes[i], cur_slots[i], cand_slots[i], ins[i], cores[i - i0], l, nb, n_chains);
            if (rc) return rc;
            lds = std::max(lds, l); max_blocks = std::max(max_blocks, nb);
            fins[i - i0] = make_step_finish_lane(e, e->lanes[i]);
            slot_list[i - i0] = cand_slots[i];
        }
        if (part == 0) mark();
        uint8_t* dm = e->d_batch_meta + (size_t)part * part_bytes;
        rc = upload(e, dm, pm, part_bytes);
        if (rc) return rc;
        if (part == 0) mark();
        k_step_core_batch<<<dim3(max_blocks, np), kBlock, lds, e->stream>>>(reinterpret_cast<const StepCore*>(dm));
        HIPCHK(e, hipGetLastError());
        if (part == 0) mark();
        for (int i = i0; i < i1; ++i) {
            commit_src_sync(e, cur_slots[i], cand_slots[i], changed_objects ? changed_objects + rows_ptr[i] : nullptr,
                            rows_ptr[i + 1] - rows_ptr[i]);
            commit_ids_sync(e, cur_slots[i], cand_slots[i], e->batch_moved[i]);
            std::swap(e->slots[cand_slots[i]], cds[i]);
        }
        if (part == 0) mark();
        MixCall mix;
        mix.n = np; mix.slots = cand_slots + i0; mix.d_slots = reinterpret_cast<const int32_t*>(dm + part_cores + part_fins);
        mix.d_fins = reinterpret_cast<const StepFinish*>(dm + part_cores); mix.done_out = part == n_parts - 1 ? &batch_done : nullptr;
        rc = launch_mixture(e, mix);
        if (rc) return rc;
    }
    mark();
    { int wrc = wait_done(e, batch_done); if (wrc) return wrc; }
    mark();
    int first_bad = SBE_OK;
    std::string first_msg;
    for (int i = 0; i < n_chains; ++i) {
        rc = read_step_results_lane(e, e->lanes[i].h_step, cand_slots[i], group_logliks_out + (size_t)i * e->Gtot, mixture_out + i,
                               changed_groups_out ? changed_groups_out + (size_t)i * e->Gtot : nullptr, "rows", e->lanes[i].d_status, i);
        if (rc && !first_bad) { first_bad = rc; first_msg = e->last_error; }
    }
    if (first_bad) return fail(e, first_bad, "%s", first_msg.c_str());
    mark();
    if (timing && ntp == 10) {
        auto us = [&](int a, int b) { return std::chrono::duration<double, std::micro>(tp[b] - tp[a]).count(); };
        fprintf(stderr, "[sbe_step_batch] %d chains (first part): checks %.1f | prepare (pool) %.1f | step cores %.1f | upload %.1f | launch core %.1f | "
                        "slot moves %.1f | mixture + reduce launches and the other parts %.1f | wait for the device %.1f | read results %.1f us\n", n_chains,
                us(0, 1), us(1, 2), us(2, 3), us(3, 4), us(4, 5), us(5, 6), us(6, 7), us(7, 8), us(8, 9));
    }
    return SBE_OK;
}

namespace {

struct DeltaPlan {
    size_t subset, sub_row, sub_gid0, patch_n, patch_gid, patch_pid, patch_tid, stale, objects, tuple_g, tuple_p, patbits, weights, rows, total;
};

inline size_t al16(size_t v) { return (v + 15) / 16 * 16; }

DeltaPlan plan_delta(const sbe_engine* e, int n_mv, int n_changed, int n_last_ids, int n_last_src, bool reweight) {
    DeltaPlan p{};
    const size_t n_sub = (size_t)n_mv + n_changed, n_patch = (size_t)n_mv + n_last_ids;
    size_t o = 0;
    p.subset = o;    o = al16(o + n_sub * 4);
    p.sub_row = o;   o = al16(o + n_sub * 2);
    p.sub_gid0 = o;  o = al16(o + n_sub * 2);
    p.patch_n = o;   o = al16(o + n_patch * 4);
    p.patch_gid = o; o = al16(o + n_patch * 2);
    p.patch_pid = o; o = al16(o + n_patch);
    p.patch_tid = o; o = al16(o + n_patch);
    p.stale = o;     o = al16(o + (size_t)n_last_src * 4);
    p.objects = o;   o = al16(o + (size_t)n_changed * 4);
    p.tuple_g = o;   o = al16(o + (size_t)kMaxTuples * kMaxComponents * 2);
    p.tuple_p = o;   o = al16(o + (size_t)kMaxTuples);
    p.patbits = o;   o = al16(o + (size_t)e->Pmax * 4);
    p.weights = o;   o = al16(o + (reweight ? (size_t)e->F * e->C * 4 : 0));
    p.rows = o;      o = al16(o + (size_t)n_changed * e->F * e->C);
    p.total = (o + 255) / 256 * 256;
    return p;
}

int prepare_step_delta(sbe_engine* e, uint8_t* h_base, const uint8_t* d_base, const DeltaPlan& L, int cur_slot, int cand_slot,
                       const int32_t* mv_objects, const int32_t* mv_cluster, int n_mv, const int32_t* changed_objects, int n_changed,
                       const uint8_t* source_rows, const float* weights, CoreInputs& in, std::vector<int32_t>& moved_out) {
    const int F = e->F, C = e->C;
    const Slot& cur = e->slots[cur_slot];
    Slot& cd = e->slots[cand_slot];
    const sbe_engine::SrcSync& irec = e->ids_sync[cand_slot];
    for (int32_t n : irec.diff) {
        cd.h_gid[n] = cur.h_gid[n]; cd.h_pid[n] = cur.h_pid[n]; cd.h_tid[n] = cur.h_tid[n]; cd.h_toff[n] = cur.h_toff[n];
    }
    cd.patterns = cur.patterns; cd.n_tuples = cur.n_tuples;
    cd.h_tuple_g = cur.h_tuple_g; cd.h_tuple_p = cur.h_tuple_p; cd.pat_cnt = cur.pat_cnt; cd.tup_cnt = cur.tup_cnt;
    cd.share_ok = cur.share_ok;
    cd.inc_ok = cur.inc_ok; cd.patterns_dirty = false;
    cd.groups_set = cur.groups_set; cd.weights_set = true; cd.source_set = cur.source_set;
    cd.counts_set = cur.counts_set;
    static thread_local std::vector<int32_t> mv;
    static thread_local std::vector<uint16_t> mv_old;
    mv.clear(); mv_old.clear();
    for (int i = 0; i < n_mv; ++i) {
        const int n = mv_objects[i];
        const uint16_t g_new = mv_cluster[i] < 0 ? kNoGroup : (uint16_t)mv_cluster[i];
        if (cd.h_gid[n] == g_new) continue;
        mv.push_back(n); mv_old.push_back(cd.h_gid[n]);
        cd.h_gid[n] = g_new;
    }
    if (!mv.empty()) {
        if (e->opt_step_derive == 1 || !update_patterns_and_tuples(e, cd, mv.data(), mv_old.data(), (int)mv.size())) return 1;
        cd.group_epoch = ++e->epoch_counter;
    } else cd.group_epoch = cur.group_epoch;
    std::fill(cd.probs_set.begin(), cd.probs_set.end(), 1);
    moved_out = mv;
    uint8_t* st = h_base;
    in = CoreInputs{};
    int32_t* sub = reinterpret_cast<int32_t*>(st + L.subset);
    int16_t* sub_row = reinterpret_cast<int16_t*>(st + L.sub_row);
    uint16_t* sub_gid0 = reinterpret_cast<uint16_t*>(st + L.sub_gid0);
    int n_subset = 0;
    {
        static thread_local std::vector<std::pair<int32_t, int32_t>> ch;
        ch.clear();
        for (int i = 0; i < n_changed; ++i) ch.emplace_back(changed_objects[i], i);
        std::sort(ch.begin(), ch.end());
        std::sort(mv.begin(), mv.end());
        size_t a = 0, b = 0;
        while (a < mv.size() || b < ch.size()) {
            int32_t n; int r = -1;
            if (b == ch.size() || (a < mv.size() && mv[a] < ch[b].first)) n = mv[a++];
            else { n = ch[b].first; r = ch[b].second; if (a < mv.size() && mv[a] == n) ++a; ++b; }
            sub[n_subset] = n; sub_row[n_subset] = (int16_t)r; sub_gid0[n_subset] = cd.h_gid[n];
            ++n_subset;
        }
    }
    int n_patch = 0;
    {
        int32_t* pn = reinterpret_cast<int32_t*>(st + L.patch_n);
        uint16_t* pg = reinterpret_cast<uint16_t*>(st + L.patch_gid);
        uint8_t* pp = st + L.patch_pid; uint8_t* pt = st + L.patch_tid;
        auto put = [&](int32_t n) { pn[n_patch] = n; pg[n_patch] = cd.h_gid[n]; pp[n_patch] = cd.h_pid[n]; pt[n_patch] = cd.h_tid[n]; ++n_patch; };
        for (int32_t n : irec.diff) put(n);
        for (int32_t n : mv) put(n);
    }
    const bool tables_changed = cd.patterns != cur.patterns || cd.h_tuple_p != cur.h_tuple_p || cd.h_tuple_g != cur.h_tuple_g;
    if (tables_changed) {
        memcpy(st + L.tuple_g, cd.h_tuple_g.data(), (size_t)kMaxTuples * kMaxComponents * 2);
        memcpy(st + L.tuple_p, cd.h_tuple_p.data(), kMaxTuples);
        memset(st + L.patbits, 0, (size_t)e->Pmax * 4);
        memcpy(st + L.patbits, cd.patterns.data(), cd.patterns.size() * 4);
        in.tuple_g = d_base + L.tuple_g; in.tuple_p = d_base + L.tuple_p; in.patbits = d_base + L.patbits;
    }
    if (weights) { memcpy(st + L.weights, weights, (size_t)F * C * 4); in.weights = d_base + L.weights; }
    if (n_changed > 0) {
        memcpy(st + L.objects, changed_objects, (size_t)n_changed * 4);
        memcpy(st + L.rows, source_rows, (size_t)n_changed * F * C);
        in.rows = d_base + L.rows;
        in.objects = reinterpret_cast<const int32_t*>(d_base + L.objects);
        in.n_changed = n_changed;
    }
    in.subset = reinterpret_cast<const int32_t*>(d_base + L.subset); in.n_subset = n_subset;
    in.sub_row = reinterpret_cast<const int16_t*>(d_base + L.sub_row);
    in.sub_gid0 = reinterpret_cast<const uint16_t*>(d_base + L.sub_gid0);
    in.patch_n = reinterpret_cast<const int32_t*>(d_base + L.patch_n);
    in.patch_gid = reinterpret_cast<const uint16_t*>(d_base + L.patch_gid);
    in.patch_pid = d_base + L.patch_pid; in.patch_tid = d_base + L.patch_tid; in.n_patch = n_patch;
    in.P = (int)cd.patterns.size();
    {
        const sbe_engine::SrcSync& rec = e->src_sync[cand_slot];
        int32_t* stale = reinterpret_cast<int32_t*>(st + L.stale);
        int ns = 0;
        for (int32_t n : rec.diff) {
            bool rewritten = false;
            for (int i = 0; i < n_changed && !rewritten; ++i) rewritten = changed_objects[i] == n;
            if (!rewritten) stale[ns++] = n;
        }
        in.full_src_copy = false;
        in.stale = reinterpret_cast<const int32_t*>(d_base + L.stale);
        in.n_stale = ns;
    }
    return 0;
}

bool sync_valid(const sbe_engine::SrcSync& rec, const sbe_engine::SrcSync& peer, int peer_slot, int cap) {
    return rec.peer == peer_slot && rec.peer_version == peer.version && rec.own_version == rec.version && (int)rec.diff.size() <= cap;
}

}

int sbe_step_batch_delta(sbe_engine* e, int n_chains, const int32_t* cur_slots, const int32_t* cand_slots,
                         const int32_t* moved_ptr, const int32_t* moved_objects, const int32_t* moved_cluster,
                         const int32_t* rows_ptr, const int32_t* changed_objects, const uint8_t* source_rows,
                         const float* weights, const uint8_t* weights_mask, double* group_logliks_out, double* mixture_out,
                         uint8_t* changed_groups_out) {
    CHECK_ENGINE(e); CHECK_PTR(e, cur_slots); CHECK_PTR(e, cand_slots); CHECK_PTR(e, moved_ptr); CHECK_PTR(e, rows_ptr);
    CHECK_PTR(e, group_logliks_out); CHECK_PTR(e, mixture_out);
    const auto t_start = std::chrono::steady_clock::now();
    std::chrono::steady_clock::time_point tq[8]; int nq = 0;
    auto markd = [&] { if (nq < 8) tq[nq++] = std::chrono::steady_clock::now(); };
    if (n_chains < 1 || n_chains > e->n_slots / 2) return fail(e, SBE_ERR_ARG, "n_chains=%d (1..%d: two slots per chain)", n_chains, e->n_slots / 2);
    if ((int64_t)e->Gtot * e->S * 28 > 60 * 1024) return fail(e, SBE_ERR_ARG, "sbe_step_batch_delta: tables too large for the one-launch step (G_total=%d, S=%d)", e->Gtot, e->S);
    const int N = e->N, F = e->F, C = e->C, K = e->G[0];
    if (rows_ptr[0] != 0 || moved_ptr[0] != 0) return fail(e, SBE_ERR_ARG, "rows_ptr[0] / moved_ptr[0] must be 0");
    {
        std::vector<uint8_t> used(e->n_slots, 0);
        std::vector<uint32_t> seen(N, 0), seen_mv(N, 0);
        for (int i = 0; i < n_chains; ++i) {
            const int a = cur_slots[i], b = cand_slots[i];
            if (a < 0 || a >= e->n_slots || b < 0 || b >= e->n_slots || a == b) return fail(e, SBE_ERR_ARG, "chain %d: bad slots (%d, %d)", i, a, b);
            if (used[a] || used[b]) return fail(e, SBE_ERR_ARG, "chain %d: slot used by another chain of the batch", i);
            used[a] = used[b] = 1;
            const int nr = rows_ptr[i + 1] - rows_ptr[i], nm = moved_ptr[i + 1] - moved_ptr[i];
            if (nr < 0 || nr > e->step_max_rows) return fail(e, SBE_ERR_ARG, "chain %d: %d changed source rows (0..%d per chain in a batched step)", i, nr, e->step_max_rows);
            if (nm < 0 || nm > N) return fail(e, SBE_ERR_ARG, "chain %d: %d moved objects", i, nm);
            if ((nr > 0 && (!changed_objects || !source_rows)) || (nm > 0 && (!moved_objects || !moved_cluster))) return fail(e, SBE_ERR_ARG, "chain %d: delta arrays missing", i);
            for (int k = rows_ptr[i]; k < rows_ptr[i + 1]; ++k) {
                const int n = changed_objects[k];
                if (n < 0 || n >= N) return fail(e, SBE_ERR_ARG, "chain %d: object index %d out of range", i, n);
                if (seen[n] == (uint32_t)(2 * i + 1)) return fail(e, SBE_ERR_ARG, "chain %d: object %d listed twice in changed_objects", i, n);
                seen[n] = (uint32_t)(2 * i + 1);
            }
            for (int k = moved_ptr[i]; k < moved_ptr[i + 1]; ++k) {
                const int n = moved_objects[k];
                if (n < 0 || n >= N) return fail(e, SBE_ERR_ARG, "chain %d: moved object index %d out of range", i, n);
                if (moved_cluster[k] < -1 || moved_cluster[k] >= K) return fail(e, SBE_ERR_ARG, "chain %d: cluster %d out of range [-1,%d)", i, moved_cluster[k], K);
                if (seen_mv[n] == (uint32_t)(i + 1)) return fail(e, SBE_ERR_ARG, "chain %d: object %d listed twice in moved_objects", i, n);
                seen_mv[n] = (uint32_t)(i + 1);
            }
            const Slot& cur = e->slots[a];
            if (!cur.groups_set || !cur.source_set || !cur.weights_set) return fail(e, SBE_ERR_STATE, "slot %d: groups / source / weights not set", a);
            { int orc = reject_overlap(e, a, "one-call step"); if (orc) return orc; }
            for (int c = 0; c < C; ++c)
                if (!cur.counts_set[c] || !e->conc_set[c]) return fail(e, SBE_ERR_STATE, "slot %d: counts / concentration of component %d not set", a, c);
        }
    }
    HIPCHK(e, hipSetDevice(e->device));
    if (e->status_pending) {
        HIPCHK(e, hipStreamSynchronize(e->stream));
        int rc = synced(e);
        if (rc) return rc;
    }
    for (int i = 0; i < n_chains; ++i)
        if (e->slots[cur_slots[i]].patterns_dirty) { int rc = upload_patterns_and_weights(e, cur_slots[i]); if (rc) return rc; }
    int rc = ensure_lanes(e, n_chains);
    if (rc) return rc;
    rc = ensure_step_pool(e);
    if (rc) return rc;
    if ((int)e->batch_moved.size() < n_chains) e->batch_moved.resize(n_chains);
    markd();
    std::vector<int> fast, slow;
    std::vector<DeltaPlan> plans(n_chains);
    std::vector<size_t> pay_off(n_chains + 1, 0);
    for (int i = 0; i < n_chains; ++i) {
        const int a = cur_slots[i], b = cand_slots[i];
        const bool ok = sync_valid(e->ids_sync[b], e->ids_sync[a], a, e->step_max_rows) &&
                        sync_valid(e->src_sync[b], e->src_sync[a], a, e->step_max_rows) &&
                        e->slots[a].inc_ok && e->slots[a].n_tuples > 0 && e->slots[b].h_gid.size() == e->slots[a].h_gid.size();
        if (ok) {
            const bool reweight = weights && (!weights_mask || weights_mask[i]);
            plans[i] = plan_delta(e, moved_ptr[i + 1] - moved_ptr[i], rows_ptr[i + 1] - rows_ptr[i], (int)e->ids_sync[b].diff.size(),
                                  (int)e->src_sync[b].diff.size(), reweight);
            pay_off[i + 1] = pay_off[i] + plans[i].total;
            fast.push_back(i);
        } else { pay_off[i + 1] = pay_off[i]; slow.push_back(i); }
    }
    auto run_classic = [&](const std::vector<int>& which, int& rc_out, std::string& msg_out) {
        rc_out = SBE_OK;
        if (which.empty()) return;
        const int ns = (int)which.size();
        std::vector<int32_t> s_cur(ns), s_cand(ns), s_ptr(ns + 1, 0), s_objs;
        std::vector<uint8_t> s_cl((size_t)ns * K * N, 0), s_rows, s_wm(ns, 0);
        std::vector<float> s_w(weights ? (size_t)ns * F * C : 0);
        for (int j = 0; j < ns; ++j) {
            const int i = which[j];
            s_cur[j] = cur_slots[i]; s_cand[j] = cand_slots[i];
            const Slot& cur = e->slots[cur_slots[i]];
            std::vector<uint16_t> ids(cur.h_gid.begin(), cur.h_gid.begin() + N);
            for (int k = moved_ptr[i]; k < moved_ptr[i + 1]; ++k) ids[moved_objects[k]] = moved_cluster[k] < 0 ? kNoGroup : (uint16_t)moved_cluster[k];
            uint8_t* cl = s_cl.data() + (size_t)j * K * N;
            for (int n = 0; n < N; ++n) if (ids[n] != kNoGroup) cl[(size_t)ids[n] * N + n] = 1;
            const int r0 = rows_ptr[i], nr = rows_ptr[i + 1] - r0;
            s_ptr[j + 1] = s_ptr[j] + nr;
            if (nr) {
                s_objs.insert(s_objs.end(), changed_objects + r0, changed_objects + r0 + nr);
                s_rows.insert(s_rows.end(), source_rows + (size_t)r0 * F * C, source_rows + (size_t)(r0 + nr) * F * C);
            }
            if (weights && (!weights_mask || weights_mask[i])) { s_wm[j] = 1; memcpy(&s_w[(size_t)j * F * C], weights + (size_t)i * F * C, (size_t)F * C * 4); }
        }
        std::vector<double> s_glh((size_t)ns * e->Gtot), s_mix(ns);
        std::vector<uint8_t> s_chg((size_t)ns * e->Gtot);
        rc_out = sbe_step_batch(e, ns, s_cur.data(), s_cand.data(), s_cl.data(), nullptr, s_ptr.data(), s_objs.empty() ? nullptr : s_objs.data(),
                                s_rows.empty() ? nullptr : s_rows.data(), weights ? s_w.data() : nullptr, weights ? s_wm.data() : nullptr,
                                s_glh.data(), s_mix.data(), s_chg.data());
        if (rc_out) { msg_out = e->last_error; return; }
        for (int j = 0; j < ns; ++j) {
            const int i = which[j];
            memcpy(group_logliks_out + (size_t)i * e->Gtot, &s_glh[(size_t)j * e->Gtot], (size_t)e->Gtot * sizeof(double));
            mixture_out[i] = s_mix[j];
            if (changed_groups_out) memcpy(changed_groups_out + (size_t)i * e->Gtot, &s_chg[(size_t)j * e->Gtot], (size_t)e->Gtot);
        }
    };
    int slow_rc = SBE_OK; std::string slow_msg;
    run_classic(slow, slow_rc, slow_msg);
    markd();
    std::vector<CoreInputs> ins(n_chains);
    std::vector<int> fb(n_chains, 0);
    const int nf = (int)fast.size();
    const size_t part_cores = ((size_t)std::max(nf, 1) * sizeof(StepCore) + 255) / 256 * 256;
    const size_t part_fins = ((size_t)std::max(nf, 1) * sizeof(StepFinish) + 255) / 256 * 256;
    const size_t meta_bytes = part_cores + part_fins + ((size_t)std::max(nf, 1) * sizeof(int32_t) + 255) / 256 * 256;
    const size_t meta_off = pay_off[n_chains];
    if (meta_off + meta_bytes > e->batch_payload_bytes) {
        HIPCHK(e, hipStreamSynchronize(e->stream));
        if (e->h_batch_payload) { HIPCHK(e, hipHostFree(e->h_batch_payload)); e->h_batch_payload = nullptr; }
        if (e->d_batch_payload) { HIPCHK(e, hipFree(e->d_batch_payload)); e->d_batch_payload = nullptr; }
        e->batch_payload_bytes = (meta_off + meta_bytes) * 3 / 2;
        HIPCHK(e, hipHostMalloc((void**)&e->h_batch_payload, e->batch_payload_bytes, hipHostMallocDefault));
        HIPCHK(e, hipMalloc((void**)&e->d_batch_payload, e->batch_payload_bytes));
    }
    if (nf > 0) {
        e->pool->run(nf, [&](int j) {
            const int i = fast[j];
            const bool reweight = weights && (!weights_mask || weights_mask[i]);
            const int r0 = rows_ptr[i], nr = rows_ptr[i + 1] - r0, m0 = moved_ptr[i], nm = moved_ptr[i + 1] - m0;
            fb[i] = prepare_step_delta(e, e->h_batch_payload + pay_off[i], e->d_batch_payload + pay_off[i], plans[i], cur_slots[i], cand_slots[i],
                                       nm ? moved_objects + m0 : nullptr, nm ? moved_cluster + m0 : nullptr, nm,
                                       nr ? changed_objects + r0 : nullptr, nr, nr ? source_rows + (size_t)r0 * F * C : nullptr,
                                       reweight ? weights + (size_t)i * F * C : nullptr, ins[i], e->batch_moved[i]);
        });
    }
    markd();
    std::vector<int> go, late;
    for (int i : fast) { if (fb[i]) { late.push_back(i); bump_ids(e, cand_slots[i]); } else go.push_back(i); }
    const int ng = (int)go.size();
    DoneSig fast_done{};
    if (ng > 0) {
        uint8_t* pm = e->h_batch_payload + meta_off;
        uint8_t* dm = e->d_batch_payload + meta_off;
        StepCore* cores = reinterpret_cast<StepCore*>(pm);
        StepFinish* fins = reinterpret_cast<StepFinish*>(pm + part_cores);
        int32_t* slot_list = reinterpret_cast<int32_t*>(pm + part_cores + part_fins);
        std::vector<int32_t> cand_go(ng);
        size_t lds = 0; int max_blocks = 0;
        for (int j = 0; j < ng; ++j) {
            const int i = go[j];
            size_t l = 0; int nb = 0;
            rc = build_step_core(e, e->lanes[i], cur_slots[i], cand_slots[i], ins[i], cores[j], l, nb, ng);
            if (rc) return rc;
            lds = std::max(lds, l); max_blocks = std::max(max_blocks, nb);
            fins[j] = make_step_finish_lane(e, e->lanes[i]);
            slot_list[j] = cand_go[j] = cand_slots[i];
        }
        HIPCHK(e, hipMemcpyAsync(e->d_batch_payload, e->h_batch_payload, meta_off + meta_bytes, hipMemcpyHostToDevice, e->stream));
        k_step_core_batch<<<dim3(max_blocks, ng), kBlock, lds, e->stream>>>(reinterpret_cast<const StepCore*>(dm));
        HIPCHK(e, hipGetLastError());
        markd();
        MixCall mix;
        mix.n = ng; mix.slots = cand_go.data(); mix.d_slots = reinterpret_cast<const int32_t*>(dm + part_cores + part_fins);
        mix.d_fins = reinterpret_cast<const StepFinish*>(dm + part_cores); mix.done_out = &fast_done;
        rc = next_timing_events(e, &mix.ev_a, &mix.ev_b);
        if (rc) return rc;
        rc = launch_mixture(e, mix);
        for (int j = 0; j < ng; ++j) {
            const int i = go[j];
            commit_src_sync(e, cur_slots[i], cand_slots[i], changed_objects ? changed_objects + rows_ptr[i] : nullptr, rows_ptr[i + 1] - rows_ptr[i]);
            commit_ids_sync(e, cur_slots[i], cand_slots[i], e->batch_moved[i]);
        }
        if (rc) return rc;
    }
    static const bool timing_d = getenv("SBE_STEP_TIMING") && atoi(getenv("SBE_STEP_TIMING")) != 0;
    const auto t_enq = std::chrono::steady_clock::now();
    { int wrc = wait_done(e, fast_done); if (wrc) return wrc; }
    if (timing_d) {
        const auto t_done = std::chrono::steady_clock::now();
        auto us = [&](std::chrono::steady_clock::time_point a, std::chrono::steady_clock::time_point b) { return std::chrono::duration<double, std::micro>(b - a).count(); };
        fprintf(stderr, "[sbe_step_batch_delta] %d chains: %d patched, %d + %d through sbe_step_batch | checks %.1f | plans %.1f | host halves (pool) %.1f | cores + launch %.1f | "
                        "mixture launches + records %.1f | wait %.1f us\n", n_chains, ng, (int)slow.size(), (int)late.size(), nq > 0 ? us(t_start, tq[0]) : 0.0,
                nq > 1 ? us(tq[0], tq[1]) : 0.0, nq > 2 ? us(tq[1], tq[2]) : 0.0, nq > 3 ? us(tq[2], tq[3]) : 0.0, nq > 3 ? us(tq[3], t_enq) : 0.0, us(t_enq, t_done));
    }
    int first_bad = slow_rc; std::string first_msg = slow_msg;
    for (int i : go) {
        rc = read_step_results_lane(e, e->lanes[i].h_step, cand_slots[i], group_logliks_out + (size_t)i * e->Gtot, mixture_out + i,
                                    changed_groups_out ? changed_groups_out + (size_t)i * e->Gtot : nullptr, "rows", e->lanes[i].d_status, i);
        if (rc && !first_bad) { first_bad = rc; first_msg = e->last_error; }
    }
    if (!late.empty()) {
        int late_rc = SBE_OK; std::string late_msg;
        run_classic(late, late_rc, late_msg);
        if (late_rc && !first_bad) { first_bad = late_rc; first_msg = late_msg; }
    }
    if (first_bad) return fail(e, first_bad, "%s", first_msg.c_str());
    return SBE_OK;
}

int sbe_step_delta(sbe_engine* e, int cur_slot, int cand_slot, const int32_t* moved_objects, const int32_t* moved_cluster, int n_moved,
                   const int32_t* changed_objects, int n_changed, const uint8_t* source_rows, const float* weights,
                   double* group_logliks_out, double* mixture_out, uint8_t* changed_groups_out) {
    CHECK_ENGINE(e); CHECK_SLOT(e, cur_slot); CHECK_SLOT(e, cand_slot);
// ... 400 lines not shown
```

sbayes_amd/csrc/sbe_mixture.hip.h:

```cpp
#pragma once
#include "sbe_device_common.hip.h"

namespace sbe {

enum MixMode : int { LOG_PER_OBS = 0, LOG_PRODUCT = 1, WRITE_OBS = 2 };

struct Mix2Params {
    int N, NQ, Np, F, Fq, S, C, Gtot, P;
    int n_ftiles, quads_per_chunk;
    int n_work, n_batch;
    int slot_groups, slots_per_group;
    const uint8_t* tid;      int64_t tid_stride;
    const uint16_t* tuple_g; int64_t tuple_g_stride;
    const uint8_t* tuple_p;  int64_t tuple_p_stride;
    int KT;
    int combo_w_off;
    int combo_tab_off;
    const uint32_t* state_q;
    const uint2* state_h;
    const uint32_t* toff;  int64_t toff_stride;
    const double2* logtab;
    int gen_slots;
    int rows_cum[5];
    int ragged_w;
    const uint8_t* onehot; int rs_pitch;
    const uint16_t* gid;   int64_t gid_stride;
    const uint8_t* pid;    int64_t pid_stride;
    const float* probs_t;  int64_t probs_t_stride;
    const double* wpat_t;  int64_t wpat_t_stride;
    int wpat_tile_stride;
    double* partials;      int64_t partials_stride;
    double* results;
    unsigned* arrive;
    DoneSig done;
    int first_slot;
    const int32_t* slot_list;
    int eft;
    const float* wpat;     int64_t wpat_stride;
    const uint32_t* rowoff; int64_t rowoff_stride;
    const uint32_t* rowoff_s; int64_t rowoff_s_stride;
    const int32_t* rs_nq;
    const uint8_t* state_s; int state_s_pitch;
};

struct MfmaMixParams {
    int F, S, FS, Gtot, Np;
    int NT, KBp;
    int KT;
    int SL;
    int shared;
    int n_batch, n_split, nt_per_split;
    int first_slot;
    const int32_t* slot_list;
    const uint8_t* xt;  uint32_t xt_bytes;
    const uint8_t* tid;      int64_t tid_stride;
    const uint16_t* tuple_g; int64_t tuple_g_stride;
    const uint8_t* tuple_p;  int64_t tuple_p_stride;
    const float* probs;      int64_t probs_stride;  uint32_t probs_bytes;
    const float* wpat;       int64_t wpat_stride;   uint32_t wpat_bytes;
    uint32_t probs_ones_off, wpat_ones_off;
    const double2* logtab;
    const int32_t* colcount;
    const int32_t* colfeat;
    const int32_t* tile_prefix;
    double* partials;        int64_t partials_stride;
    double* results;
    unsigned* arrive;
    DoneSig done;
};

void launch_v2(int mode, int ft, int C, const Mix2Params& p, dim3 grid, size_t lds, hipStream_t st, bool direct);
void launch_oh2(int mode, int ft, int C, const Mix2Params& p, dim3 grid, size_t lds, hipStream_t st, bool direct);
void launch_combo(bool onehot, int ft, int C, const Mix2Params& p, dim3 grid, size_t lds, hipStream_t st);
void launch_tuple64(int C, const Mix2Params& p, dim3 grid, size_t lds, hipStream_t st);
void launch_rows(int mode, int ft, int C, const Mix2Params& p, dim3 grid, size_t lds, hipStream_t st, bool sorted = false);
void launch_rowsort(const uint16_t* gid, const uint8_t* pid, uint32_t* out, int32_t* nq_out, int64_t gid_stride, int64_t pid_stride,
                    int64_t out_stride, int first_slot, const int32_t* slot_list, int n_slots, int N, int Np, int C, int Gtot, int Pmax,
                    uint32_t row_bytes, uint32_t state_pitch, int step_objects, hipStream_t st);
void launch_state_s(const uint8_t* state, uint8_t* state_s, int N, int F, int Fp, int pitch, int S, hipStream_t st);
void launch_xt_frags(const uint8_t* state, uint8_t* xt, int N, int F, int S, int Fp, int NT, int KBp, hipStream_t st);
size_t column_tables_bytes(int NT);
void launch_column_tables(const uint8_t* state, int32_t* out, int N, int F, int S, int Fp, int NT, hipStream_t st);
void fine_log_table(double* tab);
bool launch_tuple_mfma(int C, const MfmaMixParams& p, dim3 grid, size_t lds, hipStream_t st);
bool tuple_mfma_shared();

}
```

sbayes_amd/csrc/sbe_mixture_mfma.hip:

```cpp
#include <algorithm>
#include <cmath>
#include <cstdio>
#include <cstdlib>
#include <type_traits>
#include "sbe_mixture_mfma.hip.h"

#if defined(__HIP_DEVICE_COMPILE__) && !defined(__gfx950__) && !defined(__gfx942__)
#error "sbe_mixture_mfma.hip: the in-kernel final reduction orders relaxed agent-scope atomics by s_waitcnt (gfx942 / gfx950 cache behaviour); not valid for this target"
#endif

namespace sbe {

constexpr int kMfmaRN = kTupleMfmaColsPerPass;

__global__ void k_xt_frags(const uint8_t* __restrict__ state , uint8_t* __restrict__ xt,
                           int N, int F, int S, int Fp, int NT, int KBp) {
    const int64_t u = (int64_t)blockIdx.x * blockDim.x + threadIdx.x;
    if (u >= (int64_t)NT * KBp * 64) return;
    const int l = (int)(u & 63), kb = (int)((u >> 6) % KBp), nt = (int)((u >> 6) / KBp);
    const int col = nt * 32 + (l & 31), f = col / S, s = col - f * S;
    uint32_t w[4] = {0u, 0u, 0u, 0u};
    if (col < F * S) {
        const int n0 = kb * 64 + 32 * (l >> 5);
#pragma unroll
        for (int j = 0; j < 32; ++j) {
            const int n = n0 + 8 * (j >> 3) + (j & 7);
            const int b = j & 3, hi = (j >> 2) & 1;
            if (n < N && state[(int64_t)n * Fp + f] == (uint8_t)s) w[j >> 3] |= 0x2u << (8 * b + 4 * hi);
        }
    }
    reinterpret_cast<uint4*>(xt)[u] = make_uint4(w[0], w[1], w[2], w[3]);
}

__global__ void k_colcount(const uint8_t* __restrict__ state, int32_t* __restrict__ colcount, int32_t* __restrict__ colfeat,
                           int N, int F, int S, int Fp, int NT) {
    const int col = (int)(blockIdx.x * blockDim.x + threadIdx.x);
    if (col >= (NT + 1) * 32) return;
    int c = 0;
    const int f = min(col / S, F - 1);
    if (col < F * S) {
        const int s = col - f * S;
        for (int n = 0; n < N; ++n) c += state[(int64_t)n * Fp + f] == (uint8_t)s;
    }
    colcount[col] = c;
    colfeat[col] = f;
}

__global__ void k_tile_prefix(const int32_t* __restrict__ colcount, int32_t* __restrict__ tile_prefix, int NT) {
    if (threadIdx.x != 0 || blockIdx.x != 0) return;
    int acc = 0;
    for (int t = 0; t <= NT + 1; ++t) {
        tile_prefix[t] = acc;
        if (t <= NT) for (int i = 0; i < 32; ++i) acc += colcount[t * 32 + i];
    }
}

size_t column_tables_bytes(int NT) { return ((size_t)(NT + 1) * 64 + (size_t)NT + 2) * sizeof(int32_t); }
void launch_column_tables(const uint8_t* state, int32_t* out, int N, int F, int S, int Fp, int NT, hipStream_t st) {
    int32_t* colcount = out;
    int32_t* colfeat = out + (size_t)(NT + 1) * 32;
    int32_t* tile_prefix = out + (size_t)(NT + 1) * 64;
    k_colcount<<<(unsigned)(((NT + 1) * 32 + 255) / 256), 256, 0, st>>>(state, colcount, colfeat, N, F, S, Fp, NT);
    k_tile_prefix<<<1, 64, 0, st>>>(colcount, tile_prefix, NT);
}

void launch_xt_frags(const uint8_t* state, uint8_t* xt, int N, int F, int S, int Fp, int NT, int KBp, hipStream_t st) {
    const int64_t units = (int64_t)NT * KBp * 64;
    k_xt_frags<<<(unsigned)((units + 255) / 256), 256, 0, st>>>(state, xt, N, F, S, Fp, NT, KBp);
}

void fine_log_table(double* tab ) {
    for (int i = 0; i < kFineLogEntries; ++i) {
        const long double c = i == 0 ? 1.0L : i == kFineLogEntries - 1 ? 2.0L : 1.0L + (i + 0.5L) / kFineLogEntries;
        const double inv_c = (double)(1.0L / c);
        const long double lc = -logl((long double)inv_c) - (i >= kFineLogSplit ? logl(2.0L) : 0.0L);
        tab[2 * i] = 0.5 * inv_c;
        tab[2 * i + 1] = (i == 0 || i == kFineLogEntries - 1) ? 0.0 : (double)lc;
    }
}

template <int MT, int CT, int GT = 4, int SLB = 4, bool SHARE = false>
__global__ __launch_bounds__(kMfmaThreads, 1) void k_mixture_tuple_mfma(MfmaMixParams p) {
    typedef v16f_t acc_t;
    constexpr int SL = 1 << SLB, TPT = 32 / SL, TPB = MT * TPT;
    constexpr int NK = SL == 16 ? 8 : SL;
    extern __shared__ __align__(16) unsigned char lds_raw[];
    const int lane = threadIdx.x & (kWave - 1);
    const int w = __builtin_amdgcn_readfirstlane((int)(threadIdx.x >> 6));
    const int split = (int)blockIdx.x % p.n_split, sg = (int)blockIdx.x / p.n_split;
    const int KBp = p.KBp;
    constexpr uint32_t tab_off = 0u;
    constexpr uint32_t a_off = kFineLogEntries * 16u;
    const uint32_t a_bytes = (uint32_t)MT * (uint32_t)KBp * 1024u;
    const uint32_t meta_off = a_off + a_bytes;
    const uint32_t red_off = meta_off + (uint32_t)(SL * TPB * sizeof(TupleMeta<CT>));
    const uint32_t lds_base = (uint32_t)(uintptr_t)(__attribute__((address_space(3))) unsigned char*)lds_raw;
    typedef TupleMeta<CT> Meta;
    Meta* meta = reinterpret_cast<Meta*>(lds_raw + meta_off);
    double* red = reinterpret_cast<double*>(lds_raw + red_off);

    auto slot_of = [&](int sl) -> int {
        const int i = sg * SL + sl;
        if (i >= p.n_batch) return -1;
        return p.slot_list ? p.slot_list[i] : p.first_slot + i;
    };

    const int nt_lo = split * p.nt_per_split, nt_hi = min(p.NT, nt_lo + p.nt_per_split);
    constexpr int PF = 4;
    const __amdgpu_buffer_rsrc_t xt_rsrc = __builtin_amdgcn_make_buffer_rsrc(const_cast<uint8_t*>(p.xt), 0, (int)p.xt_bytes, 0x00020000);
    const int lane16 = lane * 16;
    auto tile_off = [&](int nt) -> int { return (nt < nt_hi ? nt : p.NT) * KBp * 1024; };
    auto load_b = [&](int toff, int kb) -> v4i_t {
        const u32x4_t d = __builtin_amdgcn_raw_buffer_load_b128(xt_rsrc, lane16, toff + kb * 1024, 0);
        v4i_t r; r.x = (int)d.x; r.y = (int)d.y; r.z = (int)d.z; r.w = (int)d.w;
        return r;
    };
    v4i_t bq[PF][kMfmaRN];
    {
        const int nt0 = nt_lo + w * kMfmaRN;
#pragma unroll
        for (int i = 0; i < PF; ++i)
#pragma unroll
            for (int r = 0; r < kMfmaRN; ++r) bq[i][r] = load_b(tile_off(nt0 + r), i);
    }

    if (lds_base != 0u) {
        if ((int)threadIdx.x < SL) {
            const int slot = slot_of((int)threadIdx.x);
            if (slot >= 0) {
                p.partials[(int64_t)slot * p.partials_stride + split] = __longlong_as_double(0x7FF8000000000000ll);
                if (p.results) p.results[slot] = __longlong_as_double(0x7FF8000000000000ll);
            }
        }
        return;
    }
    static_assert(!SHARE || (SL == 16 && CT == 2 && MT <= 3), "the shared-operand epilogue: 16 slots, C = 2, <= 6 tuples");
    const uint4* sdesc = reinterpret_cast<const uint4*>(lds_raw + meta_off);
    const uint4* tdesc = reinterpret_cast<const uint4*>(lds_raw + meta_off + SL * 16);
    const int slot_mine = slot_of((int)threadIdx.x & (SL - 1));
    SharedDescIn<SHARE ? TPB : 1> sd_in;
    if constexpr (SHARE) mfma_shared_desc_load<MT, SL>(p, slot_mine, sd_in);
    mfma_phase0<MT, CT, decltype(slot_of), SL, !SHARE>(lds_raw, p, slot_of, tab_off, a_off, meta, KBp, slot_mine);
    if constexpr (SHARE) mfma_shared_desc<MT, SL>(p, sd_in, const_cast<uint4*>(sdesc), const_cast<uint4*>(tdesc));
    __syncthreads();
    bool bad = false;
    if constexpr (SHARE) bad = __builtin_amdgcn_ballot_w64(sdesc[lane & (SL - 1)].w != 0u) != 0ull;

    const int h = lane >> 5, cl = lane & 31;
    double lsum[NK];
    int ksum[NK];
#pragma unroll
    for (int i = 0; i < NK; ++i) { lsum[i] = 0.0; ksum[i] = 0; }
    auto ent_slot = [&](int e) -> int { return ((e & 3) + 8 * (e >> 2) + 4 * h) & (SL - 1); };
    auto ent_tuple = [&](int m, int e) -> int { return m * TPT + (((e & 3) + 8 * (e >> 2) + 4 * h) >> SLB); };
    auto ent_k = [&](int e) -> int { return SL == 16 ? (e & 3) + 4 * ((e >> 2) & 1) : (e & (SL - 1)); };
    int csum = 0;
    uint32_t one_hi = 0x3FF00000u;
    asm volatile("" : "+v"(one_hi));
    const __amdgpu_buffer_rsrc_t pr_rsrc = __builtin_amdgcn_make_buffer_rsrc(const_cast<float*>(p.probs), 0, (int)p.probs_bytes, 0x00020000);
    const __amdgpu_buffer_rsrc_t w_rsrc = __builtin_amdgcn_make_buffer_rsrc(const_cast<float*>(p.wpat), 0, (int)p.wpat_bytes, 0x00020000);
    const uint32_t a_lane = a_off + (uint32_t)lane * 16u;

    auto counts_pass = [&](acc_t (&acc)[MT][kMfmaRN], const int (&toff)[kMfmaRN]) __attribute__((always_inline)) {
        uint32_t a_at[MT];
        v4i_t a_cur[MT];
#pragma unroll
        for (int m = 0; m < MT; ++m) {
            a_at[m] = a_lane + ((uint32_t)m * (uint32_t)KBp) * 1024u;
            asm volatile("" : "+v"(a_at[m]));
            a_cur[m] = *(lds_cv4i_t*)(uintptr_t)a_at[m];
        }
        auto k_group = [&](int kb0, auto first_c) __attribute__((always_inline)) {
            constexpr bool first = decltype(first_c)::value;
#pragma unroll
            for (int i = 0; i < PF; ++i) {
                v4i_t a_nxt[MT];
#pragma unroll
                for (int m = 0; m < MT; ++m) a_nxt[m] = *(lds_cv4i_t*)(uintptr_t)(a_at[m] + (uint32_t)(i + 1) * 1024u);
                const bool refill = !(first && i == 0);
                if (refill) {
#pragma unroll
                    for (int r = 0; r < kMfmaRN; ++r) bq[(i + PF - 1) % PF][r] = load_b(toff[r], kb0 + i + PF - 1);
                }
#pragma unroll
                for (int m = 0; m < MT; ++m)
#pragma unroll
                    for (int r = 0; r < kMfmaRN; ++r) {
                        const v4i_t bx = bq[i][r];
                        const v8i_t a8 = {a_cur[m].x, a_cur[m].y, a_cur[m].z, a_cur[m].w, 0, 0, 0, 0};
                        const v8i_t b8 = {bx.x, bx.y, bx.z, bx.w, 0, 0, 0, 0};
                        const acc_t zero = {0, 0, 0, 0, 0, 0, 0, 0, 0, 0, 0, 0, 0, 0, 0, 0};
                        if (first && i == 0) acc[m][r] = __builtin_amdgcn_mfma_scale_f32_32x32x64_f8f6f4(a8, b8, zero, 4, 4, 0, 0, 0, 0);
                        else acc[m][r] = __builtin_amdgcn_mfma_scale_f32_32x32x64_f8f6f4(a8, b8, acc[m][r], 4, 4, 0, 0, 0, 0);
                    }
#pragma unroll
                for (int m = 0; m < MT; ++m) a_cur[m] = a_nxt[m];
                __builtin_amdgcn_sched_group_barrier(0x100, MT, 0);
                if (refill) __builtin_amdgcn_sched_group_barrier(0x020, kMfmaRN, 0);
                __builtin_amdgcn_sched_group_barrier(0x008, MT * kMfmaRN, 0);
            }
#pragma unroll
            for (int m = 0; m < MT; ++m) a_at[m] += (uint32_t)PF * 1024u;
        };
        k_group(0, std::true_type{});
        for (int kb0 = PF; kb0 < KBp; kb0 += PF) k_group(kb0, std::false_type{});
    };

    constexpr int G = GT;
    constexpr int HQ = 4 / G;
    constexpr int NST = MT * 4 * HQ * kMfmaRN;
    uint32_t col4[kMfmaRN], fw4[kMfmaRN];
    Meta mdq[G];
    float prq[2][G][CT], wrq[2][G][CT];
    auto st_cols = [&](int nt0) {
#pragma unroll
        for (int r = 0; r < kMfmaRN; ++r) {
            const uint32_t colc = (uint32_t)min((nt0 + r) * 32 + cl, p.FS - 1);
            const uint32_t f = colc / (uint32_t)p.S;
            col4[r] = colc * 4u; fw4[r] = f * (uint32_t)(CT * 4);
        }
    };
    auto st_meta = [&](int u) {
        const int mj = u / HQ, half = u % HQ, m = mj >> 2, j = mj & 3;
#pragma unroll
        for (int i = 0; i < G; ++i) {
            const int e = 4 * j + half * G + i;
            mdq[i] = meta[ent_slot(e) * TPB + ent_tuple(m, e)];
        }
    };
    auto st_load = [&](int q) {
        const int r = q % kMfmaRN;
#pragma unroll
        for (int i = 0; i < G; ++i) {
            const uint32_t wo = mdq[i].woff + fw4[r];
            if constexpr (CT == 2) {
                const u32x2_t v2 = __builtin_amdgcn_raw_buffer_load_b64(w_rsrc, (int)wo, 0, 0);
                const uint32_t e0 = v2.x, e1 = v2.y;
                wrq[q & 1][i][0] = __uint_as_float(e0); wrq[q & 1][i][1] = __uint_as_float(e1);
            } else if constexpr (CT == 4) {
                const u32x4_t v4 = __builtin_amdgcn_raw_buffer_load_b128(w_rsrc, (int)wo, 0, 0);
                const uint32_t e0 = v4.x, e1 = v4.y, e2 = v4.z, e3 = v4.w;
                wrq[q & 1][i][0] = __uint_as_float(e0); wrq[q & 1][i][1] = __uint_as_float(e1);
                wrq[q & 1][i][2] = __uint_as_float(e2); wrq[q & 1][i][3] = __uint_as_float(e3);
            } else {
#pragma unroll
                for (int c = 0; c < CT; ++c)
                    wrq[q & 1][i][c] = __builtin_bit_cast(float, __builtin_amdgcn_raw_buffer_load_b32(w_rsrc, (int)(wo + 4u * c), 0, 0));
            }
#pragma unroll
            for (int c = 0; c < CT; ++c)
                prq[q & 1][i][c] = __builtin_bit_cast(float, __builtin_amdgcn_raw_buffer_load_b32(pr_rsrc, (int)(mdq[i].goff[c] + col4[r]), 0, 0));
        }
    };
    auto st_comp = [&](int q, const acc_t (&acc)[MT][kMfmaRN]) __attribute__((always_inline)) {
        const int r = q % kMfmaRN, u = q / kMfmaRN, mj = u / HQ, half = u % HQ, m = mj >> 2, j = mj & 3;
        double vv[G], lg[G], cntd[G];
        int cnt[G];
        bool special = false;
#pragma unroll
        for (int i = 0; i < G; ++i) {
            const float c = acc[m][r][4 * j + half * G + i];
            cnt[i] = (int)c; cntd[i] = (double)c;
            double v = 0.0;
#pragma unroll
            for (int c = 0; c < CT; ++c) {
                const double wc = (double)wrq[q & 1][i][c], pc = (double)prq[q & 1][i][c];
                v = c == 0 ? wc * pc : fma(wc, pc, v);
            }
            vv[i] = v;
            special |= __builtin_amdgcn_class(v, 0x2FF);
        }
        int kx[G];
        tab_log4_n<G>(vv, lg, kx, tab_off, one_hi);
        if (__builtin_expect(__builtin_amdgcn_ballot_w64(special) != 0ull, 0)) {
#pragma unroll
            for (int i = 0; i < G; ++i)
                if (__builtin_amdgcn_class(vv[i], 0x2FF)) { lg[i] = cnt[i] != 0 ? lib_log(vv[i]) : 0.0; kx[i] = kFineLogBias; }
        }
#pragma unroll
        for (int i = 0; i < G; ++i) {
            const int k = ent_k(4 * j + half * G + i);
            lsum[k] = fma(cntd[i], lg[i], lsum[k]);
            ksum[k] = __mul24(cnt[i], kx[i]) + ksum[k];
            asm volatile("" : "+v"(ksum[k]));
            asm volatile("" : "+v"(lsum[k]));
        }
    };

    constexpr int NSS = 8 * MT;
    uint32_t sh_col4[kMfmaRN], sh_fw4[kMfmaRN], col4u = 0;
    uint4 sdq, tdq[2];
    float p0q[2][4], p1r[kMfmaRN];
    uint32_t wr[kMfmaRN][4];
    uint64_t selm[2][2];
    double w0a[kMfmaRN], ua[kMfmaRN], w0b[kMfmaRN], ub[kMfmaRN];
    auto k_slot = [&](int k) -> int { return (k & 3) + 8 * (k >> 2) + 4 * h; };
    auto sh_desc = [&](int k) { sdq = sdesc[k_slot(k)]; };
    auto sh_load = [&]() {
#pragma unroll
        for (int r = 0; r < kMfmaRN; ++r) {
            p1r[r] = __builtin_bit_cast(float, __builtin_amdgcn_raw_buffer_load_b32(pr_rsrc, (int)(sdq.x + sh_col4[r]), 0, 0));
            const u32x2_t va = __builtin_amdgcn_raw_buffer_load_b64(w_rsrc, (int)(sdq.y + sh_fw4[r]), 0, 0);
            const u32x2_t vb = __builtin_amdgcn_raw_buffer_load_b64(w_rsrc, (int)(sdq.z + sh_fw4[r]), 0, 0);
            const uint32_t a0 = va.x, a1 = va.y, b0 = vb.x, b1 = vb.y;
            wr[r][0] = a0; wr[r][1] = a1; wr[r][2] = b0; wr[r][3] = b1;
        }
    };
    auto sh_conv = [&]() {
#pragma unroll
        for (int r = 0; r < kMfmaRN; ++r) {
            const double p1 = (double)p1r[r];
            w0a[r] = (double)__uint_as_float(wr[r][0]); ua[r] = (double)__uint_as_float(wr[r][1]) * p1;
            w0b[r] = (double)__uint_as_float(wr[r][2]); ub[r] = (double)__uint_as_float(wr[r][3]) * p1;
        }
    };
    auto td_read = [&](int q) { tdq[q & 1] = tdesc[k_slot(q / MT) * MT + q % MT]; };
    auto p0_load = [&](int q) {
        const uint4 d = tdq[q & 1];
        const uint32_t o0 = d.x + col4u, o1 = d.y + col4u;
        p0q[q & 1][0] = __builtin_bit_cast(float, __builtin_amdgcn_raw_buffer_load_b32(pr_rsrc, (int)o0, 0, 0));
        p0q[q & 1][1] = __builtin_bit_cast(float, __builtin_amdgcn_raw_buffer_load_b32(pr_rsrc, (int)(o0 + 128u), 0, 0));
        p0q[q & 1][2] = __builtin_bit_cast(float, __builtin_amdgcn_raw_buffer_load_b32(pr_rsrc, (int)o1, 0, 0));
        p0q[q & 1][3] = __builtin_bit_cast(float, __builtin_amdgcn_raw_buffer_load_b32(pr_rsrc, (int)(o1 + 128u), 0, 0));
        selm[q & 1][0] = __builtin_amdgcn_ballot_w64(d.z != 0u);
        selm[q & 1][1] = __builtin_amdgcn_ballot_w64(d.w != 0u);
    };
    auto sh_comp = [&](int q, const acc_t (&acc)[MT][kMfmaRN]) __attribute__((always_inline)) {
        const int k = q / MT, m = q % MT;
        double vv[4], lg[4], cntd[4];
        int cnt[4];
        bool special = false;
#pragma unroll
        for (int i = 0; i < 4; ++i) {
            const int tt = i >> 1, r = i & 1;
            const float c = acc[m][r][4 * ((k >> 2) + 2 * tt) + (k & 3)];
            cnt[i] = (int)c; cntd[i] = (double)c;
            const double p0 = (double)p0q[q & 1][i];
            double v = fma(w0a[r], p0, ua[r]);
            uint64_t keep;
            asm("s_and_saveexec_b64 %1, %2\n\tv_fma_f64 %0, %3, %4, %5\n\ts_mov_b64 exec, %1"
                : "+v"(v), "=&s"(keep) : "s"(selm[q & 1][tt]), "v"(w0b[r]), "v"(p0), "v"(ub[r]) : "scc");
            vv[i] = v;
            special |= __builtin_amdgcn_class(v, 0x2FF);
        }
        int kx[4];
        tab_log4_n<4>(vv, lg, kx, tab_off, one_hi);
        if (__builtin_expect(__builtin_amdgcn_ballot_w64(special) != 0ull, 0)) {
#pragma unroll
            for (int i = 0; i < 4; ++i)
                if (__builtin_amdgcn_class(vv[i], 0x2FF)) { lg[i] = cnt[i] != 0 ? lib_log(vv[i]) : 0.0; kx[i] = kFineLogBias; }
        }
#pragma unroll
        for (int i = 0; i < 4; ++i) {
            lsum[k] = fma(cntd[i], lg[i], lsum[k]);
            ksum[k] = __mul24(cnt[i], kx[i]) + ksum[k];
            asm volatile("" : "+v"(ksum[k]));
            asm volatile("" : "+v"(lsum[k]));
        }
    };

    const __amdgpu_buffer_rsrc_t cc_rsrc = __builtin_amdgcn_make_buffer_rsrc(const_cast<int32_t*>(p.colcount), 0, (p.NT + 1) * 128, 0x00020000);
    auto load_cc = [&](int nt) -> int { return (int)__builtin_amdgcn_raw_buffer_load_b32(cc_rsrc, cl * 4, (nt < nt_hi ? nt : p.NT) * 128, 0); };
    int ccnt[kMfmaRN];
    for (int nt0 = nt_lo + w * kMfmaRN; nt0 < nt_hi; nt0 += kMfmaWaves * kMfmaRN) {
        int toff[kMfmaRN];
#pragma unroll
        for (int r = 0; r < kMfmaRN; ++r) toff[r] = tile_off(nt0 + r);
        const bool first_pass = nt0 == nt_lo + w * kMfmaRN;
        if (!first_pass) {
#pragma unroll
            for (int i = 0; i < PF; ++i)
#pragma unroll
                for (int r = 0; r < kMfmaRN; ++r) bq[i][r] = load_b(toff[r], i);
        }
        if (first_pass) {
#pragma unroll
            for (int r = 0; r < kMfmaRN; ++r) ccnt[r] = load_cc(nt0 + r);
        }
        acc_t acc[MT][kMfmaRN];
        counts_pass(acc, toff);
#pragma unroll
        for (int r = 0; r < kMfmaRN; ++r) {
            csum += ccnt[r];
            ccnt[r] = load_cc(nt0 + kMfmaWaves * kMfmaRN + r);
        }
        if constexpr (SHARE) {
#pragma unroll
            for (int r = 0; r < kMfmaRN; ++r) {
                const uint32_t colc = (uint32_t)min((nt0 + r) * 32 + cl, p.FS - 1);
                sh_col4[r] = colc * 4u; sh_fw4[r] = colc / (uint32_t)p.S * (uint32_t)(CT * 4);
            }
            col4u = (uint32_t)(nt0 * 32 + cl) * 4u;
            sh_desc(0); td_read(0); td_read(1);
            sh_load();
            p0_load(0);
#pragma unroll
            for (int q = 0; q < NSS; ++q) {
                const int k = q / MT, m = q % MT;
                if (m == 0) {
                    sh_conv();
                    if (k + 1 < 8) sh_desc(k + 1);
                }
                if (m == (MT > 1 ? 1 : 0) && k + 1 < 8) sh_load();
                if (q + 1 < NSS) {
                    p0_load(q + 1);
                    if (q + 2 < NSS) td_read(q + 2);
                }
                sh_comp(q, acc);
                __builtin_amdgcn_sched_barrier(0);
            }
        } else {
        st_cols(nt0);
        st_meta(0);
        st_load(0);
#pragma unroll
        for (int q = 0; q < NST; ++q) {
            if (q + 1 < NST) {
                st_load(q + 1);
                if ((q + 2) % kMfmaRN == 0 && q + 2 < NST) st_meta((q + 2) / kMfmaRN);
            }
            st_comp(q, acc);
            __builtin_amdgcn_sched_barrier(0);
        }
        }
    }

#pragma unroll
    for (int i = 0; i < NK; ++i) {
        double v;
        if constexpr (SL == 16) {
            v = fma((double)(ksum[i] - kFineLogBias * csum), 6.93147180559945286227e-01, lsum[i]);
        } else {
            const int ks = ksum[i] + __shfl_xor(ksum[i], 32, 64);
            v = h == 0 ? fma((double)(ks - kFineLogBias * csum), 6.93147180559945286227e-01, lsum[i]) : lsum[i];
        }
#pragma unroll
        for (int off = 16; off >= 1; off >>= 1) v += __shfl_xor(v, off, 64);
        lsum[i] = v;
    }
    if (cl == 0) {
#pragma unroll
        for (int i = 0; i < NK; ++i) {
            if constexpr (SL == 16) {
                const int sl = 8 * (i >> 2) + 4 * h + (i & 3);
                red[(w * 2 + h) * 16 + sl] = lsum[i];
                red[(w * 2 + h) * 16 + (sl ^ 4)] = 0.0;
            } else {
                red[(w * 2 + h) * 16 + i] = lsum[i];
            }
        }
    }
    __syncthreads();
    if (w != 0) return;
    const int my_slot = lane < SL ? slot_of(lane) : -1;
    double total = 0.0;
    if (my_slot >= 0) {
#pragma unroll
        for (int ww = 0; ww < kMfmaWaves; ++ww) { total += red[(ww * 2 + 0) * 16 + lane]; total += red[(ww * 2 + 1) * 16 + lane]; }
    }
    if (bad) total = __longlong_as_double(0x7FF8000000000000ll);
    double* const my_partials = p.partials + (int64_t)max(my_slot, 0) * p.partials_stride;
    if (!p.results) {
        if (my_slot >= 0) my_partials[split] = total;
        return;
    }
    if (p.n_split > 1) {
        if (my_slot >= 0) __hip_atomic_store(my_partials + split, total, __ATOMIC_RELAXED, __HIP_MEMORY_SCOPE_AGENT);
        asm volatile("s_waitcnt vmcnt(0)" ::: "memory");
        unsigned t = 0;
        if (lane == 0) {
            t = __hip_atomic_fetch_add(p.arrive + sg, 1u, __ATOMIC_RELAXED, __HIP_MEMORY_SCOPE_AGENT);
            if (t == (unsigned)p.n_split - 1u) __hip_atomic_store(p.arrive + sg, 0u, __ATOMIC_RELAXED, __HIP_MEMORY_SCOPE_AGENT);
        }
        t = (unsigned)__builtin_amdgcn_readfirstlane((int)t);
        if (t != (unsigned)p.n_split - 1u) return;
        asm volatile("" ::: "memory");
        if (my_slot >= 0) {
            total = 0.0;
            for (int k = 0; k < p.n_split; ++k) total += __hip_atomic_load(my_partials + k, __ATOMIC_RELAXED, __HIP_MEMORY_SCOPE_AGENT);
        }
    }
    if (my_slot >= 0) p.results[my_slot] = total;
    signal_done(p.done);
}

template <int MT, int CT> constexpr int mfma_gt() { return (MT >= 4 || (MT == 3 && CT >= 3)) ? 2 : 4; }

template <int MT, int SLB>
static void launch_mfma_mt(int C, const MfmaMixParams& p, dim3 grid, size_t lds, hipStream_t st) {
    switch (C) {
        case 1: k_mixture_tuple_mfma<MT, 1, mfma_gt<MT, 1>(), SLB><<<grid, kMfmaThreads, lds, st>>>(p); break;
        case 2:
            if constexpr (SLB == 4 && MT <= 3) {
                if (p.shared) { k_mixture_tuple_mfma<MT, 2, mfma_gt<MT, 2>(), SLB, true><<<grid, kMfmaThreads, lds, st>>>(p); break; }
            }
            k_mixture_tuple_mfma<MT, 2, mfma_gt<MT, 2>(), SLB><<<grid, kMfmaThreads, lds, st>>>(p);
            break;
        case 3: k_mixture_tuple_mfma<MT, 3, mfma_gt<MT, 3>(), SLB><<<grid, kMfmaThreads, lds, st>>>(p); break;
        default: k_mixture_tuple_mfma<MT, 4, mfma_gt<MT, 4>(), SLB><<<grid, kMfmaThreads, lds, st>>>(p); break;
    }
}

template <int MT, int CT, int SLB, bool SHARE = false>
static bool allow_lds() {
    const void* fn = reinterpret_cast<const void*>(&k_mixture_tuple_mfma<MT, CT, mfma_gt<MT, CT>(), SLB, SHARE>);
    (void)hipFuncSetAttribute(fn, hipFuncAttributeMaxDynamicSharedMemorySize, (int)kLdsBytes);
    hipFuncAttributes attr{};
    if (hipFuncGetAttributes(&attr, fn) != hipSuccess) { (void)hipGetLastError(); return true; }
    return attr.sharedSizeBytes == 0;
}

template <int SLB>
static bool allow_lds_all() {
    bool ok = true;
    ok &= allow_lds<1, 1, SLB>(); ok &= allow_lds<1, 2, SLB>(); ok &= allow_lds<1, 3, SLB>(); ok &= allow_lds<1, 4, SLB>();
    ok &= allow_lds<2, 1, SLB>(); ok &= allow_lds<2, 2, SLB>(); ok &= allow_lds<2, 3, SLB>(); ok &= allow_lds<2, 4, SLB>();
    ok &= allow_lds<3, 1, SLB>(); ok &= allow_lds<3, 2, SLB>(); ok &= allow_lds<3, 3, SLB>(); ok &= allow_lds<3, 4, SLB>();
    ok &= allow_lds<4, 1, SLB>(); ok &= allow_lds<4, 2, SLB>(); ok &= allow_lds<4, 3, SLB>(); ok &= allow_lds<4, 4, SLB>();
    if constexpr (SLB == 4) {
        ok &= allow_lds<1, 2, SLB, true>(); ok &= allow_lds<2, 2, SLB, true>(); ok &= allow_lds<3, 2, SLB, true>();
    }
    return ok;
}

bool tuple_mfma_shared() {
    static const bool on = [] { const char* v = getenv("SBE_MFMA_SHARED"); return !(v && atoi(v) == 0); }();
    return on;
}

template <int SLB>
static void launch_mfma_slb(int MT, int C, const MfmaMixParams& p, dim3 grid, size_t lds, hipStream_t st) {
    switch (MT) {
        case 1: launch_mfma_mt<1, SLB>(C, p, grid, lds, st); break;
        case 2: launch_mfma_mt<2, SLB>(C, p, grid, lds, st); break;
        case 3: launch_mfma_mt<3, SLB>(C, p, grid, lds, st); break;
        default: launch_mfma_mt<4, SLB>(C, p, grid, lds, st); break;
    }
}

bool launch_tuple_mfma(int C, const MfmaMixParams& p, dim3 grid, size_t lds, hipStream_t st) {
    static const bool no_static_lds = [] { bool ok = allow_lds_all<4>(); ok &= allow_lds_all<2>(); ok &= allow_lds_all<1>(); return ok; }();
    if (!no_static_lds) return false;
    const int SL = p.SL;
    const int MT = (p.KT + 32 / SL - 1) / (32 / SL);
    if (SL == 16) launch_mfma_slb<4>(MT, C, p, grid, lds, st);
    else if (SL == 4) launch_mfma_slb<2>(MT, C, p, grid, lds, st);
    else launch_mfma_slb<1>(MT, C, p, grid, lds, st);
    return true;
}

}
```

sbayes_amd/csrc/sbe_mixture_mfma.hip.h:

```cpp
#pragma once
#include "sbe_mixture.hip.h"

namespace sbe {

typedef int v4i_t __attribute__((ext_vector_type(4)));
typedef int v8i_t __attribute__((ext_vector_type(8)));
typedef float v16f_t __attribute__((ext_vector_type(16)));
typedef __attribute__((address_space(3))) const v4i_t lds_cv4i_t;

constexpr int kMfmaSlots = 16;
constexpr int kMfmaThreads = kMfmaWaves * kWave;

constexpr int kFineLogSplit = 424;
constexpr uint32_t kFineLogCarry = 0x00100000u - ((uint32_t)kFineLogSplit << 10);
constexpr int kFineLogBias = 1023;
template <int G>
__device__ __forceinline__ void tab_log4_n(const double (&v)[G], double (&out)[G], int (&kexp)[G], uint32_t tab, uint32_t one_hi ) {
    f64x2_t e[G];
    double m[G], r[G], q[G];
    uint32_t mant_mask = 0x000FFFFFu;
    asm volatile("" : "+s"(mant_mask));
#pragma unroll
    for (int g = 0; g < G; ++g) {
        const uint32_t hi = (uint32_t)__double2hiint(v[g]);
        e[g] = *(lds_cf64x2_t*)(uintptr_t)(tab + ((hi >> 6) & 0x3FF0u));
        uint32_t mh;
        asm("v_bfi_b32 %0, %1, %2, %3" : "=v"(mh) : "s"(mant_mask), "v"(hi), "v"(one_hi));
        m[g] = __hiloint2double((int)mh, __double2loint(v[g]));
        kexp[g] = (int)((hi + kFineLogCarry) >> 20);
    }
#pragma unroll
    for (int g = 0; g < G; ++g) r[g] = fma(m[g], e[g].x, -0.5);
#pragma unroll
    for (int g = 0; g < G; ++g) q[g] = fma(r[g], -4.0, 8.0 / 3.0);
#pragma unroll
    for (int g = 0; g < G; ++g) q[g] = fma(r[g], q[g], -2.0);
#pragma unroll
    for (int g = 0; g < G; ++g) q[g] = fma(r[g], q[g], 2.0);
#pragma unroll
    for (int g = 0; g < G; ++g) out[g] = fma(r[g], q[g], e[g].y);
}

template <int CT>
struct __attribute__((aligned(CT <= 1 ? 8 : (CT <= 3 ? 16 : 32)))) TupleMeta {
    uint32_t woff;
    uint32_t goff[CT];
};

template <int MT, int CT, typename SlotOf, int SL = kMfmaSlots, bool META = true>
__device__ __forceinline__ void mfma_phase0(unsigned char* lds_raw, const MfmaMixParams& p, const SlotOf& slot_of, uint32_t tab_off,
                                            uint32_t a_off, TupleMeta<CT>* meta, int KBp, int slot_mine) {
    typedef TupleMeta<CT> Meta;
    constexpr int TPT = 32 / SL, TPB = MT * TPT;
    static_assert(SL == 16 || SL == 4 || SL == 2, "slots per block");
    static_assert(kMfmaThreads % SL == 0, "a thread's id units all belong to one slot");
    auto meta_of = [&](int slot, int t, uint32_t pat, const uint32_t (&g)[CT]) -> Meta {
        Meta md;
        md.woff = p.wpat_ones_off;
#pragma unroll
        for (int c = 0; c < CT; ++c) md.goff[c] = p.probs_ones_off;
        if (slot >= 0 && t < p.KT && pat != 0xFFu) {
            md.woff = (uint32_t)(((int64_t)slot * p.wpat_stride + (int64_t)pat * p.F * CT) * 4);
#pragma unroll
            for (int c = 0; c < CT; ++c)
                if ((int)g[c] < p.Gtot) md.goff[c] = (uint32_t)(((int64_t)slot * p.probs_stride + (int64_t)g[c] * p.FS) * 4);
        }
        return md;
    };
    constexpr bool PERM = TPB <= 8;
    constexpr uint32_t kNoTuple = PERM ? 0x0C0C0C0Cu : 0xFFFFFFFFu;
    const int n_units = SL * KBp * 2;
    constexpr int UB = 2;
    uint32_t d[UB][8];
    auto load_ids = [&](int u0) {
#pragma unroll
        for (int k = 0; k < UB; ++k) {
            const int u = u0 + k * kMfmaThreads;
            const int n0 = (u / SL) * 32;
            const int slot = u < n_units ? slot_mine : -1;
#pragma unroll
            for (int i = 0; i < 8; ++i) {
                d[k][i] = kNoTuple;
                if (slot >= 0 && n0 + 4 * i + 4 <= p.Np)
                    d[k][i] = *reinterpret_cast<const uint32_t*>(p.tid + (int64_t)slot * p.tid_stride + n0 + 4 * i);
            }
        }
    };
    auto emit = [&](int u0) {
#pragma unroll
        for (int k = 0; k < UB; ++k) {
            const int u = u0 + k * kMfmaThreads;
            if (u >= n_units) break;
            const int sl = u % SL, hk = u / SL;
            const int kb = hk >> 1, h = hk & 1;
#pragma unroll 8
            for (int t = 0; t < TPB; ++t) {
                uint4 o;
                uint32_t* ov = reinterpret_cast<uint32_t*>(&o);
#pragma unroll
                for (int wv = 0; wv < 4; ++wv) {
                    if constexpr (PERM) {
                        const uint64_t lut = 0x02ull << (8 * (t & 7));
                        const uint32_t lo = __builtin_amdgcn_perm((uint32_t)(lut >> 32), (uint32_t)lut, d[k][2 * wv]);
                        const uint32_t hi = __builtin_amdgcn_perm((uint32_t)(lut >> 32), (uint32_t)lut, d[k][2 * wv + 1]);
                        ov[wv] = lo | (hi << 4);
                        continue;
                    }
                    uint32_t eq[2];
#pragma unroll
                    for (int q = 0; q < 2; ++q) {
                        const uint32_t x = d[k][2 * wv + q] ^ ((uint32_t)t * 0x01010101u);
                        const uint32_t nz = ((x & 0x7F7F7F7Fu) + 0x7F7F7F7Fu) | x;
                        eq[q] = (~nz >> 7) & 0x01010101u;
                    }
                    ov[wv] = (eq[0] << 1) | (eq[1] << 5);
                }
                const uint32_t fl = (uint32_t)(h * 32 + (t % TPT) * SL + sl);
                *reinterpret_cast<uint4*>(lds_raw + a_off + (((uint32_t)(t / TPT) * (uint32_t)KBp + (uint32_t)kb) * 64u + fl) * 16u) = o;
            }
        }
    };
    const int u_first = (int)threadIdx.x;
    load_ids(u_first);
    constexpr int LT = (2 * kFineLogEntries + kMfmaThreads - 1) / kMfmaThreads;
    double lt[LT];
#pragma unroll
    for (int k = 0; k < LT; ++k) {
        const int i = (int)threadIdx.x + k * kMfmaThreads;
        lt[k] = i < 2 * kFineLogEntries ? reinterpret_cast<const double*>(p.logtab)[i] : 0.0;
    }
    const bool has_meta = META && (int)threadIdx.x < SL * TPB;
    const int m_sl = (int)threadIdx.x / TPB, m_t = (int)threadIdx.x % TPB;
    const int m_slot = has_meta ? slot_of(m_sl) : -1;
    uint32_t m_pat = 0xFFu, m_g[CT];
#pragma unroll
    for (int c = 0; c < CT; ++c) m_g[c] = 0xFFFFFFFFu;
    if (m_slot >= 0) {
        m_pat = p.tuple_p[(int64_t)m_slot * p.tuple_p_stride + m_t];
#pragma unroll
        for (int c = 0; c < CT; ++c) m_g[c] = p.tuple_g[(int64_t)m_slot * p.tuple_g_stride + m_t * kMaxComponents + c];
    }
    if (has_meta) meta[m_sl * TPB + m_t] = meta_of(m_slot, m_t, m_pat, m_g);
    (void)meta;
#pragma unroll
    for (int k = 0; k < LT; ++k) {
        const int i = (int)threadIdx.x + k * kMfmaThreads;
        if (i < 2 * kFineLogEntries) reinterpret_cast<double*>(lds_raw + tab_off)[i] = lt[k];
    }
    for (int u0 = u_first; u0 < n_units; u0 += UB * kMfmaThreads) {
        if (u0 != u_first) load_ids(u0);
        emit(u0);
    }
}

template <int TPB>
struct SharedDescIn {
    int slot;
    uint32_t pat[TPB], g0[TPB], g1[TPB];
};

template <int MT, int SL>
__device__ __forceinline__ void mfma_shared_desc_load(const MfmaMixParams& p, int slot, SharedDescIn<MT * 32 / SL>& in) {
    constexpr int TPB = MT * 32 / SL;
    static_assert(SL == 16 && TPB <= kMaxTuples, "the shared-operand form has 16 slots of <= 8 tuples");
    if ((int)threadIdx.x >= SL) return;
    in.slot = slot;
    const uint8_t* const tp = p.tuple_p + (int64_t)max(slot, 0) * p.tuple_p_stride;
    const uint16_t* const tg = p.tuple_g + (int64_t)max(slot, 0) * p.tuple_g_stride;
#pragma unroll
    for (int t = 0; t < TPB; ++t) {
        in.pat[t] = tp[t];
        in.g0[t] = tg[t * kMaxComponents + 0];
        in.g1[t] = tg[t * kMaxComponents + 1];
    }
}

template <int MT, int SL>
__device__ __forceinline__ void mfma_shared_desc(const MfmaMixParams& p, const SharedDescIn<MT * 32 / SL>& in, uint4* sdesc, uint4* tdesc) {
    constexpr int TPB = MT * 32 / SL;
    if ((int)threadIdx.x >= SL) return;
    const int sl = (int)threadIdx.x, slot = in.slot;
    const uint32_t (&g0)[TPB] = in.g0, (&g1)[TPB] = in.g1;
    uint32_t pat[TPB];
#pragma unroll
    for (int t = 0; t < TPB; ++t) pat[t] = (slot >= 0 && t < p.KT) ? in.pat[t] : 0xFFu;
    auto goff = [&](uint32_t g) -> uint32_t {
        return (int)g < p.Gtot ? (uint32_t)(((int64_t)slot * p.probs_stride + (int64_t)g * p.FS) * 4) : p.probs_ones_off;
    };
    uint32_t goff1 = p.probs_ones_off, wa = p.wpat_ones_off, wb = p.wpat_ones_off, bad = 0u;
    uint32_t go0[TPB], sel[TPB];
    bool any = false;
#pragma unroll
    for (int t = 0; t < TPB; ++t) {
        go0[t] = p.probs_ones_off; sel[t] = 0u;
        if (pat[t] == 0xFFu) continue;
        go0[t] = goff(g0[t]);
        const uint32_t wo = (uint32_t)(((int64_t)slot * p.wpat_stride + (int64_t)pat[t] * p.F * 2) * 4), g1o = goff(g1[t]);
        if (!any) { any = true; goff1 = g1o; wa = wb = wo; }
        if (g1o != goff1) bad = 1u;
        if (wo != wa) {
            if (wb == wa) wb = wo;
            else if (wo != wb) bad = 1u;
            sel[t] = 1u;
        }
    }
    sdesc[sl] = make_uint4(goff1, wa, wb, bad);
#pragma unroll
    for (int m = 0; m < MT; ++m) tdesc[sl * MT + m] = make_uint4(go0[2 * m], go0[2 * m + 1], sel[2 * m], sel[2 * m + 1]);
}

}
```

sbayes_amd/csrc/sbe_mixture_plan.h:

```cpp
#pragma once
#include <algorithm>
#include <cstddef>
#include <cstdint>
#include <cstdio>

#include "../../include/sbe_engine.h"

namespace sbe {

constexpr int kBlock = 256;
constexpr int kWave = 64;
constexpr int kMaxComponents = 8;
constexpr int kMaxTuples = 64;
constexpr int kLogTabEntries = 128;
constexpr int kRowsBlock = 1024;
constexpr int kRowsWaves = kRowsBlock / kWave;
constexpr int tuple64_waves() { return 4; }
constexpr int kTupleMfmaKBlockObjects = 64;
constexpr int kTupleMfmaColsPerPass = 2;
constexpr int kMfmaWaves = 8;
constexpr int kFineLogEntries = 1024;

constexpr size_t kLdsBytes = 160 * 1024;
constexpr size_t kRowsLdsMax = kLdsBytes - 512;
constexpr size_t kLargeImage = 72 * 1024;

inline int plan_div_up(int64_t a, int64_t b) { return (int)((a + b - 1) / b); }
inline int plan_round_up(int a, int b) { return (a + b - 1) / b * b; }

inline int tuple_mfma_slots_per_block(int KT) {
    if (KT < 1 || KT > 64) return 0;
    return KT <= 8 ? 16 : KT <= 32 ? 4 : 2;
}
inline size_t tuple_mfma_lds_bytes(int MT, int C, int KBp) {
    const size_t meta = (size_t)32 * MT * (C <= 1 ? 8 : (C <= 3 ? 16 : 32));
    return (size_t)MT * KBp * 1024 + kFineLogEntries * 16 + meta + (size_t)kMfmaWaves * 2 * 16 * sizeof(double);
}

struct MixShape {
    int N = 0, F = 0, S = 0, C = 0, n_slots = 0;
    int Gtot = 0, Pmax = 0;
    int Np = 0, NQ = 0;
    int Fq = 0;
    int ft = 64, n_ftiles = 0;
    bool direct = false;
    int rows_ft = 0;
    bool has_state_h = false;
    int compute_units = 256;
    int64_t partials_stride = 0;

    int64_t table_elems() const { return (int64_t)Gtot * F * S; }
    int64_t tile_tab_elems() const { return (int64_t)(Gtot + 1) * S * ft; }
};

inline bool derive_mix_shape(MixShape& s, int n_objects, int n_features, int n_states, int n_components, int gtot, int n_slots,
                             int compute_units, const int* forced_ft, bool force_direct, const int* forced_rows_ft) {
    s = MixShape{};
    s.N = n_objects; s.F = n_features; s.S = n_states; s.C = n_components; s.n_slots = n_slots;
    s.Gtot = gtot;
    s.Pmax = std::min(1 << n_components, 64);
    s.Np = plan_round_up(n_objects, 4);
    s.NQ = s.Np / 4;
    s.compute_units = compute_units;
    {
        int ft = 64;
        auto lds_for = [&](int t) { return ((size_t)(gtot + 1) * t * n_states) * sizeof(float) + (size_t)s.Pmax * n_components * t * sizeof(double) + 8 * 1024; };
        while (ft > 16 && lds_for(ft) > 78 * 1024) ft >>= 1;
        if (forced_ft && (*forced_ft == 64 || *forced_ft == 32 || *forced_ft == 16)) ft = *forced_ft;
        if (lds_for(ft) > 156 * 1024) {
            if (forced_ft) return false;
            ft = 16;
            s.direct = true;
        }
        if (force_direct) { ft = 16; s.direct = true; }
        s.ft = ft;
        s.n_ftiles = plan_div_up(n_features, ft);
        s.Fq = plan_round_up(n_features, 64);
    }
    if (n_components <= 4) {
        const int64_t S = n_states, C = n_components;
        const int p_assumed = std::max(1, s.Pmax / 2);
        auto rows_lds = [&](int t) { return (size_t)(gtot + 1) * (S + 1) * t * 4 + (size_t)p_assumed * ((C + 1) / 2) * t * 16 + (size_t)kRowsWaves * (kWave / t) * (C + 1) * 16; };
        s.rows_ft = rows_lds(32) <= kRowsLdsMax ? 32 : rows_lds(16) <= kRowsLdsMax ? 16 : 0;
        if (forced_rows_ft) { const int v = *forced_rows_ft; if (v == 0 || ((v == 16 || v == 32) && rows_lds(v) <= kRowsLdsMax)) s.rows_ft = v; }
    }
    s.has_state_h = s.ft == 64 && n_states <= 127 && (int64_t)s.NQ * s.Fq * 8 < ((int64_t)1 << 31);
    {
        const int64_t min_objs = kBlock / (16 / 4);
        s.partials_stride = std::max<int64_t>(plan_div_up(n_features, 16) * std::max<int64_t>(plan_div_up(n_objects, min_objs), 4 * compute_units), 1024);
    }
    return true;
}

struct MixTuning {
    int opt_kernel = SBE_MIXTURE_PACKED;
    int opt_rows_sorted = 1;
    int mfma_min_batch = 320;
    int64_t mfma_min_obs = 6400000;
    int mfma_wide_min_share = 16;
    int mfma_small_sl4 = 1;
    int mfma_split = 0;
    bool shared_allowed = true;
    bool in_kernel_allowed = true;
};

struct MixFacts {
    int n = 1;
    int P = 1;
    int KT = 0;
    bool share_ok = false;
    bool epilogue = false;
    bool waits = false;
};

enum class MixForm : int { TupleMfma, Tuple64, Combo, Rows, RowsSorted, OnehotV2, V2 };

struct MixPlan {
    int err = SBE_OK;
    char msg[256] = {0};
    MixForm form = MixForm::V2;
    int P = 1, KT = 0;
    int ft = 0, n_ftiles = 0, quads_per_chunk = 0, n_chunks = 0;
    bool onehot = false;
    size_t lds_bytes = 0;
    int combo_w_off = 0, combo_tab_off = 0;
    int rs_nq_max = 0;
    int SL = 0, MT = 0, n_split = 0, nt_per_split = 0;
    bool shared = false;
    int slot_groups = 1, slots_per_group = 1, gen_slots = 0, ragged_w = 0;
    unsigned grid_x = 0;
    int n_partials = 0;
    bool in_kernel = false;
    unsigned done_blocks = 0;
};

inline int64_t tuple_mfma_units(const MixShape& s, int n, int SL, int MT) {
    const int NT = plan_div_up((int64_t)s.F * s.S, 32);
    const int groups = plan_div_up(n, SL);
    const int split = std::max(1, std::min(plan_div_up(NT, 16), s.compute_units / std::max(1, groups)));
    const int passes = plan_div_up(plan_round_up(plan_div_up(NT, split), 2), 16);
    return (int64_t)plan_div_up(groups * split, s.compute_units) * passes * MT;
}

inline bool considers_tuple_mfma(const MixShape& s, const MixTuning& t, const MixFacts& f) {
    if (f.KT == 0) return false;
    if (t.opt_kernel == SBE_MIXTURE_PACKED_TUPLE_MFMA) return true;
    return t.opt_kernel == SBE_MIXTURE_PACKED &&
           (f.n >= t.mfma_min_batch || (t.mfma_small_sl4 && f.n >= 32 && (int64_t)f.n * s.N * s.F >= t.mfma_min_obs));
}

namespace plan_detail {

struct TileGeom { int ft, n_ftiles, quads_per_chunk, n_chunks, n_blocks; size_t lds_bytes; };

inline TileGeom tile_geometry_v2(const MixShape& s, int P, int n_batch, int blocks_per_cu) {
    TileGeom g{};
    g.ft = s.ft;
    g.n_ftiles = s.n_ftiles;
    const size_t image = (size_t)s.tile_tab_elems() * sizeof(float) + (size_t)P * s.C * s.ft * sizeof(double);
    if (!s.direct) blocks_per_cu = (int)std::max<size_t>(1, std::min<size_t>((size_t)blocks_per_cu, kLdsBytes / (image + 4096)));
    const int64_t target_blocks = (int64_t)blocks_per_cu * s.compute_units;
    const int64_t chunks = std::max<int64_t>(1, target_blocks / ((int64_t)g.n_ftiles * std::max(1, n_batch)));
    const int min_quads = 4 * (kWave / s.ft);
    const int max_quads = std::max(min_quads, (8 * 1024) / (8 * s.C + 4));
    g.quads_per_chunk = std::min<int>(max_quads, std::max<int>(min_quads, plan_div_up(s.NQ, chunks)));
    g.n_chunks = plan_div_up(s.NQ, g.quads_per_chunk);
    g.n_blocks = g.n_chunks * g.n_ftiles;
    g.lds_bytes = (size_t)g.quads_per_chunk * (8 * s.C + 4);
    if (!s.direct) g.lds_bytes += image;
    return g;
}

struct MfmaGeom { int n_split, nt_per_split, MT, SL; size_t lds; };
inline MfmaGeom mfma_geometry(const MixShape& s, const MixTuning& t, int n, int KT) {
    MfmaGeom g{};
    g.SL = tuple_mfma_slots_per_block(KT);
    if (g.SL == 0 || s.C > 4) return g;
    const int NT = plan_div_up((int64_t)s.F * s.S, 32), KBp = plan_round_up(plan_div_up(s.N, kTupleMfmaKBlockObjects), 4);
    if (g.SL == 16 && t.mfma_small_sl4 && tuple_mfma_units(s, n, 4, 1) < tuple_mfma_units(s, n, 16, plan_div_up(KT, 2))) g.SL = 4;
    for (;;) {
        g.MT = plan_div_up(KT, 32 / g.SL);
        g.lds = tuple_mfma_lds_bytes(g.MT, s.C, KBp);
        if (g.lds <= kLdsBytes || g.SL == 2) break;
        g.SL = g.SL == 16 ? 4 : 2;
    }
    if (g.lds > kLdsBytes) return g;
    const int64_t probs_bytes = ((int64_t)s.n_slots * s.table_elems() + (int64_t)s.F * s.S) * 4;
    const int64_t wpat_bytes = ((int64_t)s.n_slots * s.Pmax * s.F * s.C + (int64_t)s.F * s.C) * 4;
    if (probs_bytes >= ((int64_t)1 << 32) || wpat_bytes >= ((int64_t)1 << 32) || ((int64_t)(NT + 1) * KBp + 4) * 1024 >= ((int64_t)1 << 31)) return g;
    const int groups = plan_div_up(n, g.SL);
    int n_split = std::max(1, std::min(plan_div_up(NT, 16), s.compute_units / std::max(1, groups)));
    if (t.mfma_split > 0) n_split = std::min(t.mfma_split, NT);
    g.nt_per_split = plan_round_up(plan_div_up(NT, n_split), 2);
    if ((int64_t)plan_div_up(g.nt_per_split, 16) * kTupleMfmaColsPerPass * s.N * 2100 >= ((int64_t)1 << 31)) return g;
    g.n_split = plan_div_up(NT, g.nt_per_split);
    return g;
}

template <class... A>
inline MixPlan& refuse(MixPlan& p, int code, const char* fmt, A... a) {
    p.err = code;
    snprintf(p.msg, sizeof p.msg, fmt, a...);
    return p;
}

inline bool plan_tuple_mfma(MixPlan& p, const MixShape& s, const MixTuning& t, const MixFacts& f, size_t* lds_tried) {
    const int n = f.n, KT = f.KT;
    const bool forced = t.opt_kernel == SBE_MIXTURE_PACKED_TUPLE_MFMA;
    if (!considers_tuple_mfma(s, t, f)) return false;
    const MfmaGeom mg = mfma_geometry(s, t, n, KT);
    *lds_tried = mg.lds;
    if (mg.n_split == 0) return false;
    if (!forced && KT > 8 && s.N < t.mfma_wide_min_share * mg.MT * (32 / mg.SL)) return false;
    p.form = MixForm::TupleMfma;
    p.SL = mg.SL; p.MT = mg.MT; p.n_split = mg.n_split; p.nt_per_split = mg.nt_per_split; p.lds_bytes = mg.lds;
    p.shared = s.C == 2 && mg.SL == 16 && mg.MT <= 3 && t.shared_allowed && f.share_ok;
    p.n_partials = mg.n_split;
    p.grid_x = (unsigned)(plan_div_up(n, mg.SL) * mg.n_split);
    return true;
}

inline bool plan_combo(MixPlan& p, TileGeom& g, const MixShape& s, const MixTuning& t, const MixFacts& f, size_t* lds_tried) {
    const int P = f.P, KT = f.KT;
    const bool forced = t.opt_kernel == SBE_MIXTURE_PACKED_TUPLE || t.opt_kernel == SBE_MIXTURE_PACKED_TUPLE_LDS;
    if (KT == 0 || !(forced || t.opt_kernel == SBE_MIXTURE_PACKED || t.opt_kernel == SBE_MIXTURE_ONEHOT)) return false;
    const TileGeom gc = tile_geometry_v2(s, P, f.n, 2);
    const bool tuple64 = !p.onehot && gc.ft == 64 && s.has_state_h && t.opt_kernel != SBE_MIXTURE_PACKED_TUPLE_LDS;
    const int cu = s.C <= 4 ? s.C : kMaxComponents;
    size_t lds = (size_t)KT * (s.S + 1) * gc.ft * sizeof(double);
    if (!tuple64) {
        lds += (size_t)gc.quads_per_chunk * 4;
        lds += ((size_t)KT * cu + ((KT * cu) & 1)) * sizeof(uint16_t) + (size_t)KT * sizeof(uint32_t);
    }
    lds = (lds + 15) / 16 * 16;
    const int w_off = (int)lds;
    lds += (size_t)P * s.C * gc.ft * sizeof(double);
    if (tuple64) lds += tuple64_waves() * sizeof(double) + kLogTabEntries * 2 * sizeof(double);
    const int tab_off = (int)lds;
    bool fits = true;
    if (p.onehot) {
        const int seg16 = gc.ft * s.S / 16;
        fits = seg16 <= kBlock;
        lds += (size_t)seg16 * 32 * sizeof(uint16_t);
    }
    *lds_tried = lds;
    const int64_t obs_per_block = (int64_t)gc.quads_per_chunk * 4 * gc.ft;
    if (!fits || (forced ? lds > 150 * 1024 : (lds > 40 * 1024 || obs_per_block < (int64_t)3 * KT * s.S * gc.ft))) return false;
    g = gc;
    g.lds_bytes = lds;
    p.form = tuple64 ? MixForm::Tuple64 : MixForm::Combo;
    p.combo_w_off = w_off;
    p.combo_tab_off = p.onehot ? tab_off : 0;
    return true;
}

inline bool plan_rows(MixPlan& p, TileGeom& g, const MixShape& s, const MixTuning& t, const MixFacts& f) {
    const int n = f.n, rft = s.rows_ft;
    if (p.onehot || rft == 0 || t.opt_kernel == SBE_MIXTURE_PACKED_V2) return false;
    const size_t wave_slots = (size_t)kRowsWaves * (kWave / rft) * (s.C + 1) * 16;
    const size_t rows_image = (size_t)(s.Gtot + 1) * (s.S + 1) * rft * 4 + (size_t)f.P * ((s.C + 1) / 2) * rft * 16 + wave_slots;
    if (rows_image > kRowsLdsMax) return false;
    if (t.opt_kernel != SBE_MIXTURE_PACKED_GENERAL) {
        if (n == 1 && rows_image > kLargeImage) return false;
        const int64_t obs = (int64_t)n * s.N * s.F;
        const int64_t min_obs = s.ft >= 64 ? 64000000 : s.ft >= 32 ? 24000000 : 10000000;
        const int min_quads = s.ft >= 64 ? 500 : s.ft >= 32 ? 375 : 250;
        if (obs < min_obs || s.NQ < min_quads) return false;
    }
    const size_t sorted_image = rows_image + wave_slots;
    const bool sorted = (t.opt_rows_sorted == 2 || (t.opt_rows_sorted == 1 && n >= 16)) && rft == 32 && sorted_image <= kRowsLdsMax &&
                        (int64_t)(s.N + 1) * s.Fq < ((int64_t)1 << 24) && s.Pmax <= 64;
    const int gran = kRowsWaves * (kWave / rft);
    const int n_t = plan_div_up(s.F, rft);
    const size_t image = sorted ? sorted_image : rows_image;
    const int step_objs = 4 * (kWave / rft);
    p.rs_nq_max = plan_round_up(s.N + s.Pmax * (step_objs - 1), step_objs) / 4;
    const int NQ_geo = sorted ? p.rs_nq_max : s.NQ;
    const int64_t target = (int64_t)s.compute_units * (image > kLargeImage ? 1 : 2);
    const int min_steps = image > kLargeImage ? 8 : image > 24 * 1024 ? 4 : 1;
    const int64_t chunks = std::max<int64_t>(1, std::min<int64_t>(plan_div_up(NQ_geo, (int64_t)gran * min_steps), plan_div_up(target, (int64_t)n_t * n)));
    const int qpc = plan_round_up(plan_div_up(NQ_geo, chunks), gran);
    g.ft = rft; g.n_ftiles = n_t; g.quads_per_chunk = qpc; g.n_chunks = plan_div_up(NQ_geo, qpc);
    g.n_blocks = g.n_chunks * n_t; g.lds_bytes = image;
    p.form = sorted ? MixForm::RowsSorted : MixForm::Rows;
    return true;
}

inline void plan_tile_grid(MixPlan& p, const TileGeom& g, const MixShape& s, int n) {
    p.ft = g.ft; p.n_ftiles = g.n_ftiles; p.quads_per_chunk = g.quads_per_chunk; p.n_chunks = g.n_chunks;
    p.lds_bytes = g.lds_bytes;
    p.n_partials = g.n_blocks;
    int gcd8 = 8;
    while (g.n_blocks % gcd8) gcd8 >>= 1;
    p.slot_groups = std::max(1, std::min(8 / gcd8, n));
    p.slots_per_group = plan_div_up(n, p.slot_groups);
    p.grid_x = (unsigned)(8 * plan_div_up(g.n_blocks * p.slot_groups, 8) * p.slots_per_group);
    if (p.form != MixForm::Tuple64) return;
    p.gen_slots = std::max(1, (4 * s.compute_units / 8) / g.n_blocks);
    const int gens = plan_div_up(plan_div_up(n, 8), p.gen_slots);
    p.grid_x = n >= 8 ? (unsigned)(8 * gens * p.gen_slots * g.n_blocks) : (unsigned)(n * g.n_blocks);
    p.ragged_w = (s.F % 64 != 0 && s.F % 64 <= 32) ? s.F % 64 : 0;
}

}

inline MixPlan plan_mixture(const MixShape& s, const MixTuning& t, const MixFacts& f) {
    using namespace plan_detail;
    MixPlan p{};
    p.P = f.P; p.KT = f.KT;
    p.onehot = t.opt_kernel == SBE_MIXTURE_ONEHOT || t.opt_kernel == SBE_MIXTURE_ONEHOT_GENERAL;
    size_t lds_tried = 0;
    const bool mfma = plan_tuple_mfma(p, s, t, f, &lds_tried);
    if (!mfma && t.opt_kernel == SBE_MIXTURE_PACKED_TUPLE_MFMA)
        return refuse(p, SBE_ERR_ARG, "matrix-pipe group-tuple kernel forced but not applicable (tuples=%d, C=%d, LDS %zu bytes)", f.KT, s.C, lds_tried);
    if (!mfma) {
        TileGeom g = tile_geometry_v2(s, f.P, f.n, 4);
        const bool combo = plan_combo(p, g, s, t, f, &lds_tried);
        if (!combo && (t.opt_kernel == SBE_MIXTURE_PACKED_TUPLE || t.opt_kernel == SBE_MIXTURE_PACKED_TUPLE_LDS))
            return refuse(p, SBE_ERR_ARG, "group-tuple kernel forced but not applicable (tuples=%d, LDS %zu bytes)", f.KT, lds_tried);
        if (!combo && !plan_rows(p, g, s, t, f)) p.form = p.onehot ? MixForm::OnehotV2 : MixForm::V2;
        plan_tile_grid(p, g, s, f.n);
    }
    if (p.n_partials > s.partials_stride)
        return refuse(p, SBE_ERR_STATE, "internal: partials buffer too small (%d > %lld)", p.n_partials, (long long)s.partials_stride);
    if ((p.form == MixForm::OnehotV2 || p.form == MixForm::V2) && p.lds_bytes > 159 * 1024)
        return refuse(p, SBE_ERR_ARG, "probability / weight tables too large for LDS staging at tile width %d (%zu bytes; G_total=%d, S=%d, P=%d)",
                      p.ft, p.lds_bytes, s.Gtot, s.S, f.P);
    p.in_kernel = !f.epilogue && t.in_kernel_allowed && (mfma || p.n_partials == 1 || (!f.waits && p.n_partials <= 16));
    if (p.in_kernel) p.done_blocks = (unsigned)(mfma ? plan_div_up(f.n, p.SL) : f.n);
    return p;
}

inline void plan_name(const MixPlan& p, const MixShape& s, char* out, size_t cap) {
    if (p.form == MixForm::TupleMfma) {
        snprintf(out, cap, "k_mixture_tuple_mfma<packed stream, group-tuple form, matrix pipe fp4, %d slots x M tiles %d, C=%d%s>", p.SL, p.MT, s.C,
                 p.shared ? ", shared operands" : "");
        return;
    }
    const bool combo = p.form == MixForm::Tuple64 || p.form == MixForm::Combo;
    const char* kernel = p.form == MixForm::Tuple64 ? "k_mixture_tuple64" : p.form == MixForm::Combo ? "k_mixture_combo"
                       : (p.form == MixForm::Rows || p.form == MixForm::RowsSorted) ? "k_mixture_rows"
                       : p.form == MixForm::OnehotV2 ? "k_mixture_onehot_v2" : "k_mixture_v2";
    snprintf(out, cap, "%s<%s%s, tile %d, C=%d>", kernel, p.onehot ? "one-hot stream" : "packed stream",
             combo ? ", group-tuple form" : (p.form == MixForm::RowsSorted ? ", pattern-sorted objects" : (s.direct ? ", direct tables" : "")), p.ft, s.C);
}

}
```

Baseline: 78.09 million evals/s.

## Add clusterless-last variant of shared-operand tuple MFMA epilogue

```diff
diff --git a/sbayes_amd/csrc/sbe_engine_internal.hip.h b/sbayes_amd/csrc/sbe_engine_internal.hip.h
--- a/sbayes_amd/csrc/sbe_engine_internal.hip.h
+++ b/sbayes_amd/csrc/sbe_engine_internal.hip.h
@@ -37,6 +37,7 @@
     std::vector<uint16_t> h_tuple_g;
     std::vector<uint8_t> h_tuple_p;
     bool share_ok = false;
+    int last_need = -1;
     bool groups_set = false, weights_set = false, source_set = false;
     std::vector<uint8_t> probs_set, counts_set;
     bool patterns_dirty = true;
@@ -70,7 +71,7 @@
     int64_t hbm_bytes = 0;
     std::string last_error;
     char device_name[64] = {0};
-    char last_kernel[128] = "none";
+    char last_kernel[160] = "none";
 
     sbe::MixTuning tune;
     int opt_log = SBE_LOG_PRODUCT;
@@ -567,6 +568,11 @@
     return first >= 0;
 }
 
+void flag_tuple_tables(const sbe_engine* e, Slot& s) {
+    s.share_ok = tuples_share_operands(e, s);
+    s.last_need = s.share_ok ? clusterless_last_need(s.h_tuple_p.data(), s.h_tuple_g.data(), s.n_tuples, e->Gtot) : -1;
+}
+
 void derive_tuples(sbe_engine* e, Slot& s) {
     const int N = e->N, C = e->C;
     s.h_tid.assign(e->Np, 0);
@@ -605,7 +611,7 @@
     }
     s.n_tuples = ok ? n_tup : 0;
     s.inc_ok = ok;
-    s.share_ok = tuples_share_operands(e, s);
+    flag_tuple_tables(e, s);
 }
 
 bool update_patterns_and_tuples(sbe_engine* e, Slot& s, const int32_t* moved, const uint16_t* old_gid0, int n_moved) {
@@ -656,7 +662,7 @@
         s.h_toff[n] = (uint32_t)t1 * (uint32_t)(e->S + 1) * 512u;
     }
     while (s.n_tuples > 0 && s.tup_cnt[s.n_tuples - 1] == 0) --s.n_tuples;
-    s.share_ok = tuples_share_operands(e, s);
+    flag_tuple_tables(e, s);
     for (int t = 0; t < s.n_tuples; ++t)
         if (s.tup_cnt[t] == 0) return false;
     return s.n_tuples > 0;
@@ -831,6 +837,7 @@
         f.KT = std::max(f.KT, s.n_tuples);
         tuples &= s.n_tuples != 0;
         f.share_ok &= s.share_ok;
+        if (i == 0 || f.last_need >= 0) f.last_need = s.last_need < 0 ? -1 : std::max(f.last_need, s.last_need);
     }
     if (!tuples) f.KT = 0;
     f.epilogue = c.fin || c.d_fins;
@@ -843,6 +850,7 @@
     if (considers_tuple_mfma(*e, t, f))
         if (const char* env = getenv("SBE_MFMA_SPLIT")) t.mfma_split = atoi(env);
     t.shared_allowed = tuple_mfma_shared();
+    t.clusterless_last_allowed = tuple_mfma_clusterless_last();
     static const bool in_kernel_opt = !(getenv("SBE_REDUCE_IN_KERNEL") && atoi(getenv("SBE_REDUCE_IN_KERNEL")) == 0);
     t.in_kernel_allowed = in_kernel_opt;
     return t;
@@ -884,7 +892,7 @@
 int launch_mfma_form(sbe_engine* e, const MixCall& c, const MixPlan& pl, const DoneSig& done) {
     MfmaMixParams p{};
     p.F = e->F; p.S = e->S; p.FS = e->F * e->S; p.Gtot = e->Gtot; p.Np = e->Np;
-    p.NT = e->xt_NT; p.KBp = e->xt_KBp; p.KT = pl.KT; p.SL = pl.SL; p.shared = pl.shared ? 1 : 0;
+    p.NT = e->xt_NT; p.KBp = e->xt_KBp; p.KT = pl.KT; p.SL = pl.SL; p.shared = pl.shared ? (pl.clusterless_last ? 2 : 1) : 0;
     p.n_batch = c.n; p.n_split = pl.n_split; p.nt_per_split = pl.nt_per_split;
     p.first_slot = c.first_slot; p.slot_list = c.d_slots;
     p.xt = e->d_xt; p.xt_bytes = (uint32_t)e->xt_bytes;
diff --git a/sbayes_amd/csrc/sbe_engine_steps.hip b/sbayes_amd/csrc/sbe_engine_steps.hip
--- a/sbayes_amd/csrc/sbe_engine_steps.hip
+++ b/sbayes_amd/csrc/sbe_engine_steps.hip
@@ -601,7 +601,7 @@
     }
     cd.patterns = cur.patterns; cd.n_tuples = cur.n_tuples;
     cd.h_tuple_g = cur.h_tuple_g; cd.h_tuple_p = cur.h_tuple_p; cd.pat_cnt = cur.pat_cnt; cd.tup_cnt = cur.tup_cnt;
-    cd.share_ok = cur.share_ok;
+    cd.share_ok = cur.share_ok; cd.last_need = cur.last_need;
     cd.inc_ok = cur.inc_ok; cd.patterns_dirty = false;
     cd.groups_set = cur.groups_set; cd.weights_set = true; cd.source_set = cur.source_set;
     cd.counts_set = cur.counts_set;
diff --git a/sbayes_amd/csrc/sbe_mixture.hip.h b/sbayes_amd/csrc/sbe_mixture.hip.h
--- a/sbayes_amd/csrc/sbe_mixture.hip.h
+++ b/sbayes_amd/csrc/sbe_mixture.hip.h
@@ -83,6 +83,7 @@
 void launch_column_tables(const uint8_t* state, int32_t* out, int N, int F, int S, int Fp, int NT, hipStream_t st);
 void fine_log_table(double* tab);
 bool launch_tuple_mfma(int C, const MfmaMixParams& p, dim3 grid, size_t lds, hipStream_t st);
+bool tuple_mfma_clusterless_last();
 bool tuple_mfma_shared();
 
 }
diff --git a/sbayes_amd/csrc/sbe_mixture_mfma.hip b/sbayes_amd/csrc/sbe_mixture_mfma.hip
--- a/sbayes_amd/csrc/sbe_mixture_mfma.hip
+++ b/sbayes_amd/csrc/sbe_mixture_mfma.hip
@@ -79,7 +79,7 @@
     }
 }
 
-template <int MT, int CT, int GT = 4, int SLB = 4, bool SHARE = false>
+template <int MT, int CT, int GT = 4, int SLB = 4, bool SHARE = false, bool CLAST = false>
 __global__ __launch_bounds__(kMfmaThreads, 1) void k_mixture_tuple_mfma(MfmaMixParams p) {
     typedef v16f_t acc_t;
     constexpr int SL = 1 << SLB, TPT = 32 / SL, TPB = MT * TPT;
@@ -135,13 +135,17 @@
         return;
     }
     static_assert(!SHARE || (SL == 16 && CT == 2 && MT <= 3), "the shared-operand epilogue: 16 slots, C = 2, <= 6 tuples");
+    static_assert(!CLAST || SHARE, "clusterless last: a form of the shared-operand epilogue");
     const uint4* sdesc = reinterpret_cast<const uint4*>(lds_raw + meta_off);
     const uint4* tdesc = reinterpret_cast<const uint4*>(lds_raw + meta_off + SL * 16);
     const int slot_mine = slot_of((int)threadIdx.x & (SL - 1));
-    SharedDescIn<SHARE ? TPB : 1> sd_in;
-    if constexpr (SHARE) mfma_shared_desc_load<MT, SL>(p, slot_mine, sd_in);
-    mfma_phase0<MT, CT, decltype(slot_of), SL, !SHARE>(lds_raw, p, slot_of, tab_off, a_off, meta, KBp, slot_mine);
-    if constexpr (SHARE) mfma_shared_desc<MT, SL>(p, sd_in, const_cast<uint4*>(sdesc), const_cast<uint4*>(tdesc));
+    constexpr bool REPOS = mfma_repos<MT, CT, SL>();
+    static_assert(!SHARE || REPOS, "the shared-operand descriptors are built from the rows of the row positions");
+    TupleRows<REPOS ? TPB : 1> rows;
+    int tb_mine = -1;
+    if constexpr (REPOS) mfma_rows_load<TPB>(p, slot_mine, rows);
+    mfma_phase0<MT, CT, decltype(slot_of), SL, !SHARE>(lds_raw, p, slot_of, tab_off, a_off, meta, KBp, slot_mine, rows, tb_mine);
+    if constexpr (SHARE) mfma_shared_desc<MT, SL, CLAST>(p, slot_mine, rows, tb_mine, const_cast<uint4*>(sdesc), const_cast<uint4*>(tdesc));
     __syncthreads();
     bool bad = false;
     if constexpr (SHARE) bad = __builtin_amdgcn_ballot_w64(sdesc[lane & (SL - 1)].w != 0u) != 0ull;
@@ -301,9 +305,16 @@
         for (int r = 0; r < kMfmaRN; ++r) {
             p1r[r] = __builtin_bit_cast(float, __builtin_amdgcn_raw_buffer_load_b32(pr_rsrc, (int)(sdq.x + sh_col4[r]), 0, 0));
             const u32x2_t va = __builtin_amdgcn_raw_buffer_load_b64(w_rsrc, (int)(sdq.y + sh_fw4[r]), 0, 0);
-            const u32x2_t vb = __builtin_amdgcn_raw_buffer_load_b64(w_rsrc, (int)(sdq.z + sh_fw4[r]), 0, 0);
-            const uint32_t a0 = va.x, a1 = va.y, b0 = vb.x, b1 = vb.y;
-            wr[r][0] = a0; wr[r][1] = a1; wr[r][2] = b0; wr[r][3] = b1;
+            const uint32_t a0 = va.x, a1 = va.y;
+            wr[r][0] = a0; wr[r][1] = a1;
+            if constexpr (CLAST) {
+                wr[r][2] = 0u;
+                wr[r][3] = __builtin_amdgcn_raw_buffer_load_b32(w_rsrc, (int)(sdq.z + sh_fw4[r] + 4u), 0, 0);
+            } else {
+                const u32x2_t vb = __builtin_amdgcn_raw_buffer_load_b64(w_rsrc, (int)(sdq.z + sh_fw4[r]), 0, 0);
+                const uint32_t b0 = vb.x, b1 = vb.y;
+                wr[r][2] = b0; wr[r][3] = b1;
+            }
         }
     };
     auto sh_conv = [&]() {
@@ -314,16 +325,26 @@
             w0b[r] = (double)__uint_as_float(wr[r][2]); ub[r] = (double)__uint_as_float(wr[r][3]) * p1;
         }
     };
-    auto td_read = [&](int q) { tdq[q & 1] = tdesc[k_slot(q / MT) * MT + q % MT]; };
+    auto td_read = [&](int q) {
+        if constexpr (CLAST) {
+            const uint2 g = *reinterpret_cast<const uint2*>(tdesc + (k_slot(q / MT) * MT + q % MT));
+            tdq[q & 1].x = g.x; tdq[q & 1].y = g.y;
+        } else tdq[q & 1] = tdesc[k_slot(q / MT) * MT + q % MT];
+    };
     auto p0_load = [&](int q) {
         const uint4 d = tdq[q & 1];
         const uint32_t o0 = d.x + col4u, o1 = d.y + col4u;
         p0q[q & 1][0] = __builtin_bit_cast(float, __builtin_amdgcn_raw_buffer_load_b32(pr_rsrc, (int)o0, 0, 0));
         p0q[q & 1][1] = __builtin_bit_cast(float, __builtin_amdgcn_raw_buffer_load_b32(pr_rsrc, (int)(o0 + 128u), 0, 0));
+        if constexpr (CLAST) {
+            if (q % MT == MT - 1) return;
+        }
         p0q[q & 1][2] = __builtin_bit_cast(float, __builtin_amdgcn_raw_buffer_load_b32(pr_rsrc, (int)o1, 0, 0));
         p0q[q & 1][3] = __builtin_bit_cast(float, __builtin_amdgcn_raw_buffer_load_b32(pr_rsrc, (int)(o1 + 128u), 0, 0));
-        selm[q & 1][0] = __builtin_amdgcn_ballot_w64(d.z != 0u);
-        selm[q & 1][1] = __builtin_amdgcn_ballot_w64(d.w != 0u);
+        if constexpr (!CLAST) {
+            selm[q & 1][0] = __builtin_amdgcn_ballot_w64(d.z != 0u);
+            selm[q & 1][1] = __builtin_amdgcn_ballot_w64(d.w != 0u);
+        }
     };
     auto sh_comp = [&](int q, const acc_t (&acc)[MT][kMfmaRN]) __attribute__((always_inline)) {
         const int k = q / MT, m = q % MT;
@@ -335,11 +356,17 @@
             const int tt = i >> 1, r = i & 1;
             const float c = acc[m][r][4 * ((k >> 2) + 2 * tt) + (k & 3)];
             cnt[i] = (int)c; cntd[i] = (double)c;
-            const double p0 = (double)p0q[q & 1][i];
-            double v = fma(w0a[r], p0, ua[r]);
-            uint64_t keep;
-            asm("s_and_saveexec_b64 %1, %2\n\tv_fma_f64 %0, %3, %4, %5\n\ts_mov_b64 exec, %1"
-                : "+v"(v), "=&s"(keep) : "s"(selm[q & 1][tt]), "v"(w0b[r]), "v"(p0), "v"(ub[r]) : "scc");
+            double v;
+            if constexpr (CLAST) {
+                if (m == MT - 1 && tt == 1) v = ub[r];
+                else v = fma(w0a[r], (double)p0q[q & 1][i], ua[r]);
+            } else {
+                const double p0 = (double)p0q[q & 1][i];
+                v = fma(w0a[r], p0, ua[r]);
+                uint64_t keep;
+                asm("s_and_saveexec_b64 %1, %2\n\tv_fma_f64 %0, %3, %4, %5\n\ts_mov_b64 exec, %1"
+                    : "+v"(v), "=&s"(keep) : "s"(selm[q & 1][tt]), "v"(w0b[r]), "v"(p0), "v"(ub[r]) : "scc");
+            }
             vv[i] = v;
             special |= __builtin_amdgcn_class(v, 0x2FF);
         }
@@ -492,6 +519,7 @@
         case 1: k_mixture_tuple_mfma<MT, 1, mfma_gt<MT, 1>(), SLB><<<grid, kMfmaThreads, lds, st>>>(p); break;
         case 2:
             if constexpr (SLB == 4 && MT <= 3) {
+                if (p.shared == 2) { k_mixture_tuple_mfma<MT, 2, mfma_gt<MT, 2>(), SLB, true, true><<<grid, kMfmaThreads, lds, st>>>(p); break; }
                 if (p.shared) { k_mixture_tuple_mfma<MT, 2, mfma_gt<MT, 2>(), SLB, true><<<grid, kMfmaThreads, lds, st>>>(p); break; }
             }
             k_mixture_tuple_mfma<MT, 2, mfma_gt<MT, 2>(), SLB><<<grid, kMfmaThreads, lds, st>>>(p);
@@ -501,9 +529,9 @@
     }
 }
 
-template <int MT, int CT, int SLB, bool SHARE = false>
+template <int MT, int CT, int SLB, bool SHARE = false, bool CLAST = false>
 static bool allow_lds() {
-    const void* fn = reinterpret_cast<const void*>(&k_mixture_tuple_mfma<MT, CT, mfma_gt<MT, CT>(), SLB, SHARE>);
+    const void* fn = reinterpret_cast<const void*>(&k_mixture_tuple_mfma<MT, CT, mfma_gt<MT, CT>(), SLB, SHARE, CLAST>);
     (void)hipFuncSetAttribute(fn, hipFuncAttributeMaxDynamicSharedMemorySize, (int)kLdsBytes);
     hipFuncAttributes attr{};
     if (hipFuncGetAttributes(&attr, fn) != hipSuccess) { (void)hipGetLastError(); return true; }
@@ -519,12 +547,18 @@
     ok &= allow_lds<4, 1, SLB>(); ok &= allow_lds<4, 2, SLB>(); ok &= allow_lds<4, 3, SLB>(); ok &= allow_lds<4, 4, SLB>();
     if constexpr (SLB == 4) {
         ok &= allow_lds<1, 2, SLB, true>(); ok &= allow_lds<2, 2, SLB, true>(); ok &= allow_lds<3, 2, SLB, true>();
+        ok &= allow_lds<1, 2, SLB, true, true>(); ok &= allow_lds<2, 2, SLB, true, true>(); ok &= allow_lds<3, 2, SLB, true, true>();
     }
     return ok;
 }
 
 bool tuple_mfma_shared() {
     static const bool on = [] { const char* v = getenv("SBE_MFMA_SHARED"); return !(v && atoi(v) == 0); }();
+    return on;
+}
+
+bool tuple_mfma_clusterless_last() {
+    static const bool on = [] { const char* v = getenv("SBE_MFMA_CLUSTERLESS_LAST"); return !(v && atoi(v) == 0); }();
     return on;
 }
 
diff --git a/sbayes_amd/csrc/sbe_mixture_mfma.hip.h b/sbayes_amd/csrc/sbe_mixture_mfma.hip.h
--- a/sbayes_amd/csrc/sbe_mixture_mfma.hip.h
+++ b/sbayes_amd/csrc/sbe_mixture_mfma.hip.h
@@ -47,11 +47,44 @@
     uint32_t goff[CT];
 };
 
-template <int MT, int CT, typename SlotOf, int SL = kMfmaSlots, bool META = true>
+template <int TPB>
+struct TupleRows {
+    uint32_t pw[2];
+    uint32_t gw[TPB];
+    __device__ __forceinline__ uint32_t pat(int t) const { return (pw[t >> 2] >> (8 * (t & 3))) & 0xFFu; }
+    __device__ __forceinline__ uint32_t g0(int t) const { return gw[t] & 0xFFFFu; }
+    __device__ __forceinline__ uint32_t g1(int t) const { return gw[t] >> 16; }
+};
+
+template <int TPB>
+__device__ __forceinline__ void mfma_rows_load(const MfmaMixParams& p, int slot, TupleRows<TPB>& in) {
+    static_assert(TPB <= 8, "one 8-byte word of patterns");
+    const uint2 pw = *reinterpret_cast<const uint2*>(p.tuple_p + (int64_t)max(slot, 0) * p.tuple_p_stride);
+    const uint32_t* const tg = reinterpret_cast<const uint32_t*>(p.tuple_g + (int64_t)max(slot, 0) * p.tuple_g_stride);
+    in.pw[0] = pw.x; in.pw[1] = pw.y;
+#pragma unroll
+    for (int t = 0; t < TPB; ++t) in.gw[t] = tg[t * (kMaxComponents / 2)];
+}
+
+template <int TPB>
+__device__ __forceinline__ int mfma_clusterless_id(const MfmaMixParams& p, int slot, const TupleRows<TPB>& in) {
+    int tb = -1, n = 0;
+#pragma unroll
+    for (int t = 0; t < TPB; ++t)
+        if (slot >= 0 && t < p.KT && in.pat(t) != 0xFFu && (int)in.g0(t) >= p.Gtot) { tb = t; ++n; }
+    return n == 1 ? tb : -1;
+}
+
+template <int TPB>
+__device__ __forceinline__ int mfma_id_at(int pos, int tb) { return tb < 0 ? pos : (pos == TPB - 1 ? tb : pos + (pos >= tb ? 1 : 0)); }
+
+template <int MT, int CT, int SL> constexpr bool mfma_repos() { return SL == 16 && CT == 2 && MT * (32 / SL) <= 8; }
+template <int MT, int CT, typename SlotOf, int SL = kMfmaSlots, bool META = true, typename Rows>
 __device__ __forceinline__ void mfma_phase0(unsigned char* lds_raw, const MfmaMixParams& p, const SlotOf& slot_of, uint32_t tab_off,
-                                            uint32_t a_off, TupleMeta<CT>* meta, int KBp, int slot_mine) {
+                                            uint32_t a_off, TupleMeta<CT>* meta, int KBp, int slot_mine, const Rows& rows, int& tb_out) {
     typedef TupleMeta<CT> Meta;
     constexpr int TPT = 32 / SL, TPB = MT * TPT;
+    constexpr bool REPOS = mfma_repos<MT, CT, SL>();
     static_assert(SL == 16 || SL == 4 || SL == 2, "slots per block");
     static_assert(kMfmaThreads % SL == 0, "a thread's id units all belong to one slot");
     auto meta_of = [&](int slot, int t, uint32_t pat, const uint32_t (&g)[CT]) -> Meta {
@@ -72,6 +105,7 @@
     const int n_units = SL * KBp * 2;
     constexpr int UB = 2;
     uint32_t d[UB][8];
+    uint64_t lut_pos[REPOS ? TPB : 1];
     auto load_ids = [&](int u0) {
 #pragma unroll
         for (int k = 0; k < UB; ++k) {
@@ -100,7 +134,7 @@
 #pragma unroll
                 for (int wv = 0; wv < 4; ++wv) {
                     if constexpr (PERM) {
-                        const uint64_t lut = 0x02ull << (8 * (t & 7));
+                        const uint64_t lut = REPOS ? lut_pos[REPOS ? t : 0] : 0x02ull << (8 * (t & 7));
                         const uint32_t lo = __builtin_amdgcn_perm((uint32_t)(lut >> 32), (uint32_t)lut, d[k][2 * wv]);
                         const uint32_t hi = __builtin_amdgcn_perm((uint32_t)(lut >> 32), (uint32_t)lut, d[k][2 * wv + 1]);
                         ov[wv] = lo | (hi << 4);
@@ -130,18 +164,38 @@
         lt[k] = i < 2 * kFineLogEntries ? reinterpret_cast<const double*>(p.logtab)[i] : 0.0;
     }
     const bool has_meta = META && (int)threadIdx.x < SL * TPB;
-    const int m_sl = (int)threadIdx.x / TPB, m_t = (int)threadIdx.x % TPB;
-    const int m_slot = has_meta ? slot_of(m_sl) : -1;
-    uint32_t m_pat = 0xFFu, m_g[CT];
-#pragma unroll
-    for (int c = 0; c < CT; ++c) m_g[c] = 0xFFFFFFFFu;
-    if (m_slot >= 0) {
-        m_pat = p.tuple_p[(int64_t)m_slot * p.tuple_p_stride + m_t];
-#pragma unroll
-        for (int c = 0; c < CT; ++c) m_g[c] = p.tuple_g[(int64_t)m_slot * p.tuple_g_stride + m_t * kMaxComponents + c];
-    }
-    if (has_meta) meta[m_sl * TPB + m_t] = meta_of(m_slot, m_t, m_pat, m_g);
-    (void)meta;
+    tb_out = -1;
+    if constexpr (REPOS) {
+        const int tb = mfma_clusterless_id<TPB>(p, slot_mine, rows);
+        tb_out = tb;
+#pragma unroll
+        for (int t = 0; t < TPB; ++t) lut_pos[t] = 0x02ull << (8 * mfma_id_at<TPB>(t, tb));
+        if (has_meta) {
+            const int m_sl = (int)threadIdx.x % SL, m_pos = (int)threadIdx.x / SL, id = mfma_id_at<TPB>(m_pos, tb);
+            uint32_t m_pat = 0xFFu, m_gw = 0xFFFFFFFFu;
+#pragma unroll
+            for (int t = 0; t < TPB; ++t) {
+                m_pat = t == id ? rows.pat(t) : m_pat;
+                m_gw = t == id ? rows.gw[t] : m_gw;
+            }
+            uint32_t m_g[CT];
+            m_g[0] = m_gw & 0xFFFFu; m_g[CT - 1] = m_gw >> 16;
+            meta[m_sl * TPB + m_pos] = meta_of(slot_mine, id, m_pat, m_g);
+        }
+    } else {
+        const int m_sl = (int)threadIdx.x / TPB, m_t = (int)threadIdx.x % TPB;
+        const int m_slot = has_meta ? slot_of(m_sl) : -1;
+        uint32_t m_pat = 0xFFu, m_g[CT];
+#pragma unroll
+        for (int c = 0; c < CT; ++c) m_g[c] = 0xFFFFFFFFu;
+        if (m_slot >= 0) {
+            m_pat = p.tuple_p[(int64_t)m_slot * p.tuple_p_stride + m_t];
+#pragma unroll
+            for (int c = 0; c < CT; ++c) m_g[c] = p.tuple_g[(int64_t)m_slot * p.tuple_g_stride + m_t * kMaxComponents + c];
+        }
+        if (has_meta) meta[m_sl * TPB + m_t] = meta_of(m_slot, m_t, m_pat, m_g);
+    }
+    (void)meta; (void)rows;
 #pragma unroll
     for (int k = 0; k < LT; ++k) {
         const int i = (int)threadIdx.x + k * kMfmaThreads;
@@ -153,60 +207,60 @@
     }
 }
 
-template <int TPB>
-struct SharedDescIn {
-    int slot;
+template <int MT, int SL, bool CLAST>
+__device__ __forceinline__ void mfma_shared_desc(const MfmaMixParams& p, int slot, const TupleRows<MT * 32 / SL>& in, int tb, uint4* sdesc, uint4* tdesc) {
+    constexpr int TPB = MT * 32 / SL;
+    static_assert(SL == 16 && TPB <= 8, "the shared-operand form has 16 slots of <= 8 tuples");
+    if ((int)threadIdx.x >= SL) return;
+    const int sl = (int)threadIdx.x;
     uint32_t pat[TPB], g0[TPB], g1[TPB];
-};
-
-template <int MT, int SL>
-__device__ __forceinline__ void mfma_shared_desc_load(const MfmaMixParams& p, int slot, SharedDescIn<MT * 32 / SL>& in) {
-    constexpr int TPB = MT * 32 / SL;
-    static_assert(SL == 16 && TPB <= kMaxTuples, "the shared-operand form has 16 slots of <= 8 tuples");
-    if ((int)threadIdx.x >= SL) return;
-    in.slot = slot;
-    const uint8_t* const tp = p.tuple_p + (int64_t)max(slot, 0) * p.tuple_p_stride;
-    const uint16_t* const tg = p.tuple_g + (int64_t)max(slot, 0) * p.tuple_g_stride;
 #pragma unroll
     for (int t = 0; t < TPB; ++t) {
-        in.pat[t] = tp[t];
-        in.g0[t] = tg[t * kMaxComponents + 0];
-        in.g1[t] = tg[t * kMaxComponents + 1];
-    }
-}
-
-template <int MT, int SL>
-__device__ __forceinline__ void mfma_shared_desc(const MfmaMixParams& p, const SharedDescIn<MT * 32 / SL>& in, uint4* sdesc, uint4* tdesc) {
-    constexpr int TPB = MT * 32 / SL;
-    if ((int)threadIdx.x >= SL) return;
-    const int sl = (int)threadIdx.x, slot = in.slot;
-    const uint32_t (&g0)[TPB] = in.g0, (&g1)[TPB] = in.g1;
-    uint32_t pat[TPB];
-#pragma unroll
-    for (int t = 0; t < TPB; ++t) pat[t] = (slot >= 0 && t < p.KT) ? in.pat[t] : 0xFFu;
+        pat[t] = (slot >= 0 && t < p.KT) ? in.pat(t) : 0xFFu;
+        g0[t] = in.g0(t); g1[t] = in.g1(t);
+    }
     auto goff = [&](uint32_t g) -> uint32_t {
         return (int)g < p.Gtot ? (uint32_t)(((int64_t)slot * p.probs_stride + (int64_t)g * p.FS) * 4) : p.probs_ones_off;
     };
     uint32_t goff1 = p.probs_ones_off, wa = p.wpat_ones_off, wb = p.wpat_ones_off, bad = 0u;
     uint32_t go0[TPB], sel[TPB];
-    bool any = false;
+    bool any = false, any_a = false;
 #pragma unroll
     for (int t = 0; t < TPB; ++t) {
         go0[t] = p.probs_ones_off; sel[t] = 0u;
         if (pat[t] == 0xFFu) continue;
         go0[t] = goff(g0[t]);
         const uint32_t wo = (uint32_t)(((int64_t)slot * p.wpat_stride + (int64_t)pat[t] * p.F * 2) * 4), g1o = goff(g1[t]);
-        if (!any) { any = true; goff1 = g1o; wa = wb = wo; }
-        if (g1o != goff1) bad = 1u;
-        if (wo != wa) {
-            if (wb == wa) wb = wo;
-            else if (wo != wb) bad = 1u;
-            sel[t] = 1u;
-        }
-    }
+        if constexpr (CLAST) {
+            if (!any) { any = true; goff1 = g1o; }
+            if (g1o != goff1) bad = 1u;
+            if (t == tb) { wb = wo; continue; }
+            if (!any_a) { any_a = true; wa = wo; }
+            if (wo != wa || (int)g0[t] >= p.Gtot || (tb < 0 && t == TPB - 1)) bad = 1u;
+        } else {
+            if (!any) { any = true; goff1 = g1o; wa = wb = wo; }
+            if (g1o != goff1) bad = 1u;
+            if (wo != wa) {
+                if (wb == wa) wb = wo;
+                else if (wo != wb) bad = 1u;
+                sel[t] = 1u;
+            }
+        }
+    }
+    if (CLAST && tb < 0) wb = wa;
+    (void)any_a;
     sdesc[sl] = make_uint4(goff1, wa, wb, bad);
-#pragma unroll
-    for (int m = 0; m < MT; ++m) tdesc[sl * MT + m] = make_uint4(go0[2 * m], go0[2 * m + 1], sel[2 * m], sel[2 * m + 1]);
-}
-
-}
+    uint32_t go0p[TPB], selp[TPB];
+#pragma unroll
+    for (int q = 0; q < TPB; ++q) {
+        const int id = mfma_id_at<TPB>(q, tb);
+        go0p[q] = p.probs_ones_off; selp[q] = 0u;
+#pragma unroll
+        for (int t = 0; t < TPB; ++t)
+            if (t == id) { go0p[q] = go0[t]; selp[q] = sel[t]; }
+    }
+#pragma unroll
+    for (int m = 0; m < MT; ++m) tdesc[sl * MT + m] = make_uint4(go0p[2 * m], go0p[2 * m + 1], selp[2 * m], selp[2 * m + 1]);
+}
+
+}
diff --git a/sbayes_amd/csrc/sbe_mixture_plan.h b/sbayes_amd/csrc/sbe_mixture_plan.h
--- a/sbayes_amd/csrc/sbe_mixture_plan.h
+++ b/sbayes_amd/csrc/sbe_mixture_plan.h
@@ -35,6 +35,17 @@
 inline size_t tuple_mfma_lds_bytes(int MT, int C, int KBp) {
     const size_t meta = (size_t)32 * MT * (C <= 1 ? 8 : (C <= 3 ? 16 : 32));
     return (size_t)MT * KBp * 1024 + kFineLogEntries * 16 + meta + (size_t)kMfmaWaves * 2 * 16 * sizeof(double);
+}
+
+inline int clusterless_last_need(const uint8_t* tuple_p, const uint16_t* tuple_g, int n_tuples, int Gtot) {
+    int n_cl = 0, top = 0;
+    for (int t = 0; t < n_tuples && t < kMaxTuples; ++t) {
+        if (tuple_p[t] == 0xFF) continue;
+        top = t + 1;
+        if ((int)tuple_g[(size_t)t * kMaxComponents] >= Gtot) ++n_cl;
+    }
+    if (top == 0 || n_cl > 1) return -1;
+    return n_cl == 1 ? 0 : top;
 }
 
 struct MixShape {
@@ -101,6 +112,7 @@
     int mfma_small_sl4 = 1;
     int mfma_split = 0;
     bool shared_allowed = true;
+    bool clusterless_last_allowed = true;
     bool in_kernel_allowed = true;
 };
 
@@ -109,6 +121,7 @@
     int P = 1;
     int KT = 0;
     bool share_ok = false;
+    int last_need = -1;
     bool epilogue = false;
     bool waits = false;
 };
@@ -127,6 +140,7 @@
     int rs_nq_max = 0;
     int SL = 0, MT = 0, n_split = 0, nt_per_split = 0;
     bool shared = false;
+    bool clusterless_last = false;
     int slot_groups = 1, slots_per_group = 1, gen_slots = 0, ragged_w = 0;
     unsigned grid_x = 0;
     int n_partials = 0;
@@ -215,6 +229,7 @@
     p.form = MixForm::TupleMfma;
     p.SL = mg.SL; p.MT = mg.MT; p.n_split = mg.n_split; p.nt_per_split = mg.nt_per_split; p.lds_bytes = mg.lds;
     p.shared = s.C == 2 && mg.SL == 16 && mg.MT <= 3 && t.shared_allowed && f.share_ok;
+    p.clusterless_last = p.shared && t.clusterless_last_allowed && f.last_need >= 0 && f.last_need <= 2 * mg.MT - 1;
     p.n_partials = mg.n_split;
     p.grid_x = (unsigned)(plan_div_up(n, mg.SL) * mg.n_split);
     return true;
@@ -333,8 +348,8 @@
 
 inline void plan_name(const MixPlan& p, const MixShape& s, char* out, size_t cap) {
     if (p.form == MixForm::TupleMfma) {
-        snprintf(out, cap, "k_mixture_tuple_mfma<packed stream, group-tuple form, matrix pipe fp4, %d slots x M tiles %d, C=%d%s>", p.SL, p.MT, s.C,
-                 p.shared ? ", shared operands" : "");
+        snprintf(out, cap, "k_mixture_tuple_mfma<packed stream, group-tuple form, matrix pipe fp4, %d slots x M tiles %d, C=%d%s%s>", p.SL, p.MT, s.C,
+                 p.shared ? ", shared operands" : "", p.clusterless_last ? ", clusterless last" : "");
         return;
     }
     const bool combo = p.form == MixForm::Tuple64 || p.form == MixForm::Combo;
```

Result: faster. 82.48 million evals/s, median of 5 (+5.6%).
